# domainxz/top-k-rec

Hardware: AMD Instinct MI355X
Metric: BPR training triplets/sec (sampler + plan + step), MovieLens-10M shape (higher is better)
Workload: dtype f32

## Files before the change

include/tkr.h:

```cpp
#ifndef TKR_H
#define TKR_H
#include <stdint.h>

#ifdef __cplusplus
extern "C" {
#endif

#define TKR_VERSION 120
#define TKR_OK 0
#define TKR_E_INVAL (-1)
#define TKR_E_UNSUPPORTED (-2)
#define TKR_E_IO (-3)
#define TKR_E_PARSE (-4)
#define TKR_E_NOMEM (-5)

int tkr_version(void);
int tkr_lab_build(void);

int tkr_plan_team(int32_t batch_size);
int tkr_plan_max_blocks(int32_t batch_size);
int tkr_sample_plan(const int32_t* tr_users, int32_t n_tr, const int32_t* row_ptr, const int32_t* pos_cols,
                    const int32_t* cols_sorted, int32_t n_users, int32_t n_items, uint64_t seed,
                    uint64_t first_triplet, const int64_t* ctl, int32_t n_batches, int32_t batch_size,
                    int32_t* ucnt, int32_t* icnt, uint32_t* touch_u, uint32_t* touch_i, int32_t* out_u,
                    int32_t* out_i, int32_t* out_j, int32_t* task, int32_t* occ, int32_t* rec, int32_t* hdr,
                    int32_t* occt, int32_t* tpar, int32_t* prec, int32_t* pocc, void* workspace, int64_t workspace_bytes,
                    void* stream);
int64_t tkr_plan_workspace_bytes(int32_t batch_size, int32_t n_batches);

int tkr_plan_rollback(const int32_t* task, int32_t batch_size, int32_t first_batch, int32_t n_batches, int32_t* ucnt,
                      int32_t* icnt, void* stream);

typedef struct {
    float* U;
    float* msU;
    float* V;
    float* msV;
    float* b;
    float* msb;
    int32_t n_users, n_items, k;
    int32_t mode;
    float lu, li, lj, lb;
    float lr;
    float rho, eps;
    int32_t opt;
} tkr_bpr_state;

int tkr_bpr_run(const tkr_bpr_state* st, int32_t* rec, const int32_t* occ, const int32_t* hdr,
                int32_t batch_size, int32_t n_batches, float* loss_out, void* stream);

typedef struct {
    void* U;
    void* msU;
    void* tailU;
    uint32_t* rdU;
    void* V;
    void* msV;
    void* tailV;
    uint32_t* rdV;
    int32_t n_users, n_items, k;
    int32_t mode;
    float lu, li, lj, lb;
    float lr, rho, eps;
    int32_t opt;
    int32_t item_bufs;
} tkr_flow_state;
int32_t tkr_flow_row_granules(int32_t k);
int32_t tkr_flow_ctl_words(void);
#define TKR_FLOW_CTL_STATUS 1026
#define TKR_FLOW_CTL_SPINS 1027
int tkr_bpr_flow_run(const tkr_flow_state* st, const int32_t* prec, const int32_t* pocc, int32_t batch_size,
                     int32_t n_batches, uint32_t* ctl, float* loss_out, int32_t waves_per_cu, void* stream);

int32_t tkr_bpr_own_owners(int32_t n_items, int32_t k);
int32_t tkr_bpr_own_owners_shared(int32_t n_items, int32_t k, int32_t share);
int tkr_sample_plan_owned(const int32_t* tr_users, int32_t n_tr, const int32_t* row_ptr, const int32_t* pos_cols,
                          const int32_t* cols_sorted, int32_t n_users, int32_t n_items, uint64_t seed, uint64_t first_triplet,
                          int32_t n_batches, int32_t batch_size, int32_t* ucnt, int32_t* icnt, uint32_t* touch_u,
                          uint32_t* touch_i, int32_t* out_u, int32_t* out_i, int32_t* out_j, int32_t* task, int32_t* occ,
                          int32_t* occt, int32_t* prec, int32_t* pocc, int32_t n_owner, int32_t* ohdr, int32_t ohdr_stride,
                          void* stream);
int tkr_bpr_own_run(const tkr_flow_state* st, const int32_t* prec, const int32_t* pocc, const int32_t* occt, const int32_t* ohdr,
                    int32_t ohdr_stride, int32_t n_owner, int32_t batch_size, int32_t first_batch, int32_t n_batches, uint32_t* ctl, float* loss_out,
                    int32_t owner_waves, void* xch, uint32_t epoch, void* stream);
typedef struct tkr_plan_call {
    const int32_t *tr_users, *row_ptr, *pos_cols, *cols_sorted;
    int32_t *ucnt, *icnt;
    uint32_t *touch_u, *touch_i;
    int32_t *out_u, *out_i, *out_j, *task, *occ, *occt, *prec, *pocc, *ohdr;
    uint64_t seed, first_triplet;
    int32_t n_tr, n_users, n_items, n_batches, batch_size, n_owner, ohdr_stride, reserved;
} tkr_plan_call;
int tkr_bpr_own_plan_run(const tkr_plan_call* plan, const tkr_flow_state* st, int32_t first_batch, int32_t n_batches, uint32_t* ctl,
                         float* loss_out, int32_t owner_waves, void* xch, uint32_t epoch, void* ev_before, void* ev_after, void* stream);
int tkr_bpr_own_run_between(void* ev_before, void* ev_after, const tkr_flow_state* st, const int32_t* prec, const int32_t* pocc,
                            const int32_t* occt, const int32_t* ohdr, int32_t ohdr_stride, int32_t n_owner, int32_t batch_size,
                            int32_t first_batch, int32_t n_batches, uint32_t* ctl, float* loss_out, int32_t owner_waves, void* xch,
                            uint32_t epoch, void* stream);

typedef struct {
    float* U;
    float* msU;
    float* I;
    float* msI;
    float* irb;
    float* msirb;
    float* cem;
    float* mscem;
    float* icb;
    float* msicb;
    const float* feat;
    int32_t n_users, n_items, kh, d;
    int32_t mode;
    float lu, li, lj, lb, le;
    float lr, rho, eps;
    const int32_t* f_ptr;
    const int32_t* f_col;
    const float* f_val;
    const int32_t* c_ptr;
    const int32_t* c_item;
    const float* c_val;
    int64_t* item_tag;
} tkr_vbpr_state;

int64_t tkr_vbpr_workspace_floats(int32_t batch_size, int32_t kh, int32_t d);
int tkr_vbpr_set_pairs(int32_t mode);
int tkr_vbpr_run(const tkr_vbpr_state* st, const int32_t* tri_i, const int32_t* tri_j, const int32_t* rec,
                 const int32_t* occ, const int32_t* hdr, const int32_t* occt, const int32_t* tri_u ,
                 const int32_t* tpar , int32_t batch_size,
                 int32_t n_batches, float* workspace, float* loss_out, void* stream);

int64_t tkr_vbpr_colplan_lds_bytes(int32_t batch_size, int32_t d);
int tkr_vbpr_colplan(const int32_t* f_ptr, const int32_t* f_col, const float* f_val, int32_t d, const int32_t* tri_i,
                     const int32_t* tri_j, int32_t batch_size, int32_t n_batches, int32_t row_cap, int32_t* colh, int32_t* cent,
                     int32_t* tcnt, int32_t* tent, void* stream);
int tkr_vbpr_run_cols(const tkr_vbpr_state* st, const int32_t* tri_i, const int32_t* tri_j, const int32_t* rec, const int32_t* occ,
                      const int32_t* hdr, const int32_t* occt, const int32_t* tri_u, const int32_t* tpar, const int32_t* colh,
                      const int32_t* cent, const int32_t* tcnt, const int32_t* tent, int32_t row_cap, int32_t cols_per_block,
                      int32_t batch_size, int32_t n_batches, float* workspace, float* loss_out, void* stream);

int64_t tkr_topk_workspace_bytes(int32_t n_rows, int32_t K);
int64_t tkr_topk_workspace_bytes_for(int32_t n_rows, int32_t n_cols, int32_t k, int32_t K);
int tkr_topk_set_math(int32_t mode);
int tkr_build_rated_mask(const int64_t* rated_ptr, const int32_t* rated_cols, int32_t n_rows, int32_t n_cols,
                         uint32_t* mask, int32_t mask_pitch, void* stream);
int tkr_score_topk(const float* U, const int32_t* user_idx, int32_t n_rows, const float* Vt, const float* bias,
                   int32_t n_cols, int32_t k, const uint32_t* mask, int32_t mask_pitch, int32_t K,
                   int32_t* out_ids, float* out_scores, void* workspace, int64_t workspace_bytes, void* stream);

int tkr_count_hits(const int32_t* ids, int32_t n_rows, int32_t K, const int64_t* like_ptr, const int32_t* like_cols,
                   int32_t step, int32_t interval, uint64_t* first_bucket, void* stream);

int tkr_raw_ranks(const float* U, const int32_t* user_idx, int32_t n_rows, const float* Vt, const float* bias, int32_t k,
                  const int64_t* rated_ptr, const int32_t* rated_cols, const int32_t* ids, int32_t K, int32_t* raw_rank,
                  void* stream);
int tkr_count_hits_rr(const int32_t* ids, const int32_t* raw_rank, int32_t n_rows, int32_t K, const int64_t* like_ptr,
                      const int32_t* like_cols, int32_t step, int32_t interval, int32_t* hit_first, double* rr_first,
                      void* stream);

int64_t tkr_like_ranks_workspace_bytes(int32_t n_rows, int32_t n_cols, int32_t k, int64_t n_likes);
int tkr_like_ranks(const float* U, const int32_t* user_idx, int32_t n_rows, const float* Vt, const float* bias,
                   int32_t n_cols, int32_t k, const uint32_t* mask, int32_t mask_pitch, const int64_t* like_ptr,
                   const int32_t* like_cols, int32_t* rank_out, void* workspace, int64_t workspace_bytes, void* stream);

#define TKR_CANDIDATES_RESIDENT 2048
int tkr_rank_candidates(const float* U, const int32_t* user_idx, int32_t n_rows, const float* Vt, const float* bias,
                        int32_t n_cols, int32_t k, const int64_t* cand_ptr, const int32_t* cand_cols, const uint32_t* mask,
                        int32_t mask_pitch, float* score_out, int32_t* rank_out, void* stream);

int tkr_bpr_foldin(const float* V, const float* b, int32_t n_items, int32_t k, const int64_t* hist_ptr, const int32_t* hist_cols,
                   int32_t m, const float* U0, float lu, float lr, int32_t mode, int32_t steps, int32_t triplets, uint64_t seed,
                   uint64_t first_row, float* U, float* loss, int32_t* trip, void* stream);

int tkr_bpr_foldin_items(const float* U, const float* V, const float* b, int32_t n_users, int32_t n_items, int32_t k,
                         const int64_t* user_ptr, const int32_t* user_cols, const int64_t* liker_ptr, const int32_t* liker_rows,
                         const uint32_t* role_thresh, int32_t m, const float* V0, const float* b0, float li, float lj, float lb, float lr,
                         int32_t mode, int32_t steps, int32_t triplets, uint64_t seed, uint64_t first_row, float* Vn, float* bn,
                         float* loss, int32_t* trip, void* stream);

int tkr_sync_snapshot(const float* P, const int32_t* cnt, float* start, int64_t n, int32_t w, void* stream);
int tkr_sync_flow_snapshot(const void* V, const void* tailV, const int32_t* icnt, float* start, int32_t n, int32_t k, int32_t item_bufs,
                           void* stream);
int tkr_sync_flow_pack(const void* V, const void* msV, const void* tailV, const int32_t* icnt, const float* start, float* flat_delta,
                       float* flat_ms, int32_t n, int32_t k, float inv_world, int32_t item_bufs, void* stream);
int tkr_sync_flow_unpack(void* V, void* msV, void* tailV, uint32_t* rdV, int32_t* icnt, float* start ,
                         const float* flat_delta, const float* flat_ms, int32_t n, int32_t k, int32_t item_bufs, void* stream);
int tkr_sync_pack(const float* P, const float* ms, const int32_t* cnt, const float* start, float* flat_delta, float* flat_ms,
                  int64_t n, int32_t w, float inv_world, void* stream);
int tkr_sync_unpack(float* P, float* ms, const float* start, const float* flat_delta, const float* flat_ms, int64_t n, int32_t w,
                    void* stream);

int tkr_calib_rowcopy(const float* src, float* dst, const int32_t* rows, int32_t n, int32_t k, void* stream);

int tkr_idmap_create(const char* blob, int64_t blob_len, const int32_t* index, int64_t n, void** out_map);
int tkr_idmap_destroy(void* map);
int tkr_ratings_parse(const char* path, const void* user_map, const void* item_map, void** out_ratings);
int tkr_ratings_sizes(const void* ratings, int64_t* n_lines, int64_t* n_entries);
int tkr_ratings_copy(const void* ratings, int32_t* line_user, int64_t* line_ptr , int32_t* item,
                     int32_t* like);
int tkr_ratings_destroy(void* ratings);
int tkr_matrix_read(const char* path, void** out_matrix);
int tkr_matrix_sizes(const void* matrix, int64_t* rows, int64_t* cols);
int tkr_matrix_copy(const void* matrix, float* dst );
int tkr_matrix_destroy(void* matrix);
int tkr_matrix_write(const char* path, const float* data, int64_t rows, int64_t cols);

int64_t tkr_parse_dev_workspace_bytes(int64_t n_bytes, int64_t chunk_bytes);
int64_t tkr_idtable_slots(int64_t n);
int tkr_idtable_build(const char* blob, int64_t blob_len, const int32_t* index, int64_t n, int32_t* slots, int64_t n_slots);
int tkr_ratings_count_dev(const void* text, int64_t n_bytes, int64_t chunk_bytes, void* workspace, int64_t workspace_bytes,
                          int64_t* totals_out, void* stream);
int tkr_ratings_emit_dev(const void* text, int64_t n_bytes, int64_t chunk_bytes, void* workspace, int64_t workspace_bytes,
                         int64_t n_lines, int64_t n_entries, const int32_t* user_slots, int64_t user_n_slots,
                         const void* user_blob, int64_t user_blob_len, const int32_t* item_slots, int64_t item_n_slots,
                         const void* item_blob, int64_t item_blob_len, int64_t* line_start, int32_t* line_user,
                         int64_t* line_ptr, int32_t* item, int32_t* like, int64_t* status, void* stream);

int tkr_lists_format_sizes_dev(const int32_t* ids, const float* scores, const int32_t* row_user, int64_t n, int32_t K,
                               const void* user_blob, int64_t user_blob_len, const int64_t* user_start, const int32_t* user_len,
                               int64_t n_users, const void* item_blob, int64_t item_blob_len, const int64_t* item_start,
                               const int32_t* item_len, int64_t n_items, int64_t* line_ptr, int64_t* totals, void* stream);
int tkr_lists_format_emit_dev(const int32_t* ids, const float* scores, const int32_t* row_user, int64_t n, int32_t K,
                              const void* user_blob, int64_t user_blob_len, const int64_t* user_start, const int32_t* user_len,
                              int64_t n_users, const void* item_blob, int64_t item_blob_len, const int64_t* item_start,
                              const int32_t* item_len, int64_t n_items, const int64_t* line_ptr, int64_t first_row, int64_t n_rows,
                              void* out, int64_t out_bytes, int64_t* status, void* stream);
int tkr_matrix_format_sizes_dev(const float* data, int64_t rows, int64_t cols, int64_t* line_ptr, int64_t* totals, void* stream);
int tkr_matrix_format_emit_dev(const float* data, int64_t rows, int64_t cols, const int64_t* line_ptr, int64_t first_row,
                               int64_t n_rows, void* out, int64_t out_bytes, int64_t* status, void* stream);

int64_t tkr_scan_dev_workspace_bytes(int64_t n_bytes, int64_t chunk_bytes);
int tkr_matrix_count_dev(const void* text, int64_t n_bytes, int64_t chunk_bytes, void* workspace, int64_t workspace_bytes,
                         int64_t* totals_out, void* stream);
int tkr_matrix_emit_dev(const void* text, int64_t n_bytes, int64_t chunk_bytes, void* workspace, int64_t workspace_bytes,
                        int64_t n_lines, int64_t n_tokens, int64_t cols, int64_t* tok_start, float* data, uint64_t* hard,
                        int64_t* counts, void* stream);
int tkr_matrix_token_host(const char* tok, int64_t len, float* out);
int tkr_matrix_tokens_host(const char* text, int64_t n_bytes, const int64_t* start, int64_t n, float* out);

#ifdef __cplusplus
}
#endif
#endif
```

top-k-rec_amd/csrc/bpr_own.hip:

```cpp
#include "flow_task.h"
#ifndef TKR_TAG_NAP
#define TKR_TAG_NAP 4
#endif
#ifdef TKR_PLAN_STAMP
namespace tkr { __device__ unsigned long long own_k1_prof[32]; }
#define K1_STAMP(i) do { if (blockIdx.x == 0 && threadIdx.x == 0) tkr::own_k1_prof[i] = __builtin_amdgcn_s_memrealtime(); } while (0)
#define K1_STAMP_ITEMS(i) do { if (blockIdx.x == 0 && threadIdx.x == 256) tkr::own_k1_prof[i] = __builtin_amdgcn_s_memrealtime(); } while (0)
#endif
#include "plan_parts.h"

namespace tkr {

struct PlanArgs {
    const int32_t *tr_users, *row_ptr, *pos_cols, *cols_sorted;
    int32_t *ucnt, *icnt;
    uint32_t *touch_u, *touch_i;
    int32_t *out_u, *out_i, *out_j;
    int4* task;
    int2* occ;
    int32_t* occt;
    int4 *prec, *pocc;
    int32_t* ohdr;
    uint64_t seed, first_triplet;
    uint32_t n_tr, n_items;
    int n_plan, npad_items, own_words, reg_sort_ok;
};

template <int NAP>
__device__ __forceinline__ bool plan_rendezvous(uint32_t* counter, uint32_t n, bool arrive, uint32_t* ctl, volatile uint32_t* flag) {
    if (threadIdx.x == 0) {
        if (arrive) __hip_atomic_fetch_add(counter, 1u, __ATOMIC_RELAXED, __HIP_MEMORY_SCOPE_AGENT);
        uint32_t waited = 0, ok = 1u;
        while (ld_u32(counter) < n) {
            __builtin_amdgcn_s_sleep(NAP);
            if (spin_fail(waited, ctl, 0)) { ok = 0u; break; }
        }
        lds_poke(flag, ok);
    }
    __syncthreads();
    const bool ok = lds_peek(flag) != 0u;
    __syncthreads();
    return ok;
}

constexpr uint32_t kOwnInvalid = 0xffffffffu;

__host__ __device__ inline size_t plan_scratch_bytes(int B, int npad_items, int n_owner, int own_words) {
    size_t a = (size_t)npad_items * 8 + (kWideThreads / TKR_WAVE + 1) * 4;
    if (a < (size_t)(256 + 512) * 8 + 64) a = (size_t)(256 + 512) * 8 + 64;
    const size_t pb = (size_t)3 * B * 20 + (size_t)4 * n_owner * (own_words + 1) + (kWideThreads / TKR_WAVE + 1) * 4 + 16 + (size_t)3 * B * 32;
    return ((a > pb ? a : pb) + 15) & ~(size_t)15;
}

template <bool PLAN>
__device__ __forceinline__ int4 plan_ld(const int4* __restrict__ prec, const __amdgpu_buffer_rsrc_t& prec_r, size_t idx16) {
    if constexpr (PLAN) {
        const v4u x = __builtin_amdgcn_raw_buffer_load_b128(prec_r, (int)(idx16 * 16), 0, kAuxLoad);
        return make_int4((int)x.x, (int)x.y, (int)x.z, (int)x.w);
    } else {
        return prec[idx16];
    }
}
constexpr int kDotWin = 1024;

struct OwnQueue {
    uint32_t head;
    uint32_t total;
    uint32_t arrival;
    uint32_t head_batch;
};

struct QueueMap {
    const uint32_t* pre;
    const uint32_t* start;
    uint32_t slots_per_batch;
    __device__ __forceinline__ uint32_t locate(uint32_t pos, uint32_t& cur, int lane) const {
        uint32_t before;
        for (;;) {
            const uint32_t v = pre[cur + 1 + lane];
            const unsigned long long m = __ballot(v > pos);
            if (m) {
                const int f = __ffsll((long long)m) - 1;
                before = f ? (uint32_t)bcast_i((int)v, f - 1) : pre[cur];
                cur += f;
                break;
            }
            cur += TKR_WAVE;
        }
        return cur * slots_per_batch + start[cur] + (pos - before);
    }
};

template <bool PLAN>
struct UserTicketSrc {
    uint32_t ticket;
    int home, queues;
    uint32_t total;
    uint32_t B;
    const int4* __restrict__ prec;
    __amdgpu_buffer_rsrc_t prec_r;
    __device__ __forceinline__ void prefetch(NextTask& nx, int lane) {
        const u64 i64 = (u64)(uint32_t)bcast_i((int)ticket, 0) * (uint32_t)queues + (uint32_t)home;
        const uint32_t idx = i64 < total ? (uint32_t)i64 : 0xffffffffu;
        nx.have = true;
        nx.w = make_int4(0, 0, 0, 0);
        if (idx == 0xffffffffu) { nx.idx = idx; return; }
        nx.idx = idx + 2u * B * (idx / B);
        if (lane < 8) nx.w = plan_ld<PLAN>(prec, prec_r, (size_t)nx.idx * 8 + lane);
    }
};

template <int NP>
__device__ __forceinline__ void lds_row_read(const float* row, int lane, bool sgd, float (&own)[2 * NP], float (&ms)[2 * NP], Own& o) {
    constexpr int KP = NP * 128;
#pragma unroll
    for (int q = 0; q < NP; ++q) {
        const float2 a = *reinterpret_cast<const float2*>(row + q * 128 + 2 * lane);
        own[2 * q] = a.x; own[2 * q + 1] = a.y;
        if (!sgd) {
            const float2 m = *reinterpret_cast<const float2*>(row + KP + q * 128 + 2 * lane);
            ms[2 * q] = m.x; ms[2 * q + 1] = m.y;
        }
    }
    const float4 t = *reinterpret_cast<const float4*>(row + 2 * KP);
    const float2 t2 = *reinterpret_cast<const float2*>(row + 2 * KP + 4);
    o.b = t.x; o.msb = t.y;
    o.exp[0] = __float_as_uint(t.z); o.exp[1] = __float_as_uint(t.w);
    o.exp[2] = __float_as_uint(t2.x); o.exp[3] = __float_as_uint(t2.y);
}

struct ItemRow {
    const u64 *own_p, *own_ms, *own_tail;
    const uint32_t* own_rd;
    uint32_t ver;
    bool from_lds;
    const volatile uint32_t* tag;
    const float* row;
    int halves;
    bool rd_staged;
    uint32_t rd_val;
};

template <int NP>
__device__ __forceinline__ bool item_own_wait(const FlowTables& T, int lane, const ItemRow& r, bool sgd, float (&own)[2 * NP], float (&ms)[2 * NP],
                                              Own& o, uint32_t* ctl, uint32_t& spins) {
    if (r.from_lds) {
        uint32_t waited = 0;
        while (lds_peek(r.tag) != r.ver) {
#if TKR_TAG_NAP > 0
            __builtin_amdgcn_s_sleep(TKR_TAG_NAP);
#endif
            if (spin_fail(waited, ctl, 0)) {
                if (waited >= kSpinLimit && lane == 0 && atomicCAS(ctl + kCtlDebug, 0u, 4u) == 0u) {
                    ctl[kCtlDebug + 1] = lds_peek(r.tag); ctl[kCtlDebug + 3] = r.ver;
                }
                return false;
            }
        }
        spins += waited;
        asm volatile("" ::: "memory");
        lds_row_read<NP>(r.row, lane, sgd, own, ms, o);
        o.ok = true;
        if (r.rd_staged) {
            o.rd = r.rd_val;
            return true;
        }
    }
    return flow_own<NP>(T, lane, r.own_p, r.own_ms, r.own_tail, r.own_rd, r.ver, own, ms, o, sgd, ctl, spins, r.halves);
}

template <int NP>
struct LdsOwnStep {
    const FlowTables& T;
    int lane;
    const ItemRow& r;
    bool sgd;
    uint32_t* ctl;
    uint32_t& spins;
    __device__ __forceinline__ bool operator()(float (&own)[2 * NP], float (&ms)[2 * NP], Own& o) {
#ifdef TKR_OWN_PROF
        o.t_own0 = __builtin_amdgcn_s_memtime();
        const bool ok = item_own_wait<NP>(T, lane, r, sgd, own, ms, o, ctl, spins);
        o.t_own1 = __builtin_amdgcn_s_memtime();
        return ok;
#else
        return item_own_wait<NP>(T, lane, r, sgd, own, ms, o, ctl, spins);
#endif
    }
};
struct NoFeed {
    __device__ __forceinline__ void prefetch(NextTask& nx, int) { nx.have = true; }
};

template <int NP>
__device__ __forceinline__ void own_update(const tkr_flow_state& st, bool sgd, const float (&own)[2 * NP], const float (&ms)[2 * NP],
                                           const Own& o, const float (&g)[2 * NP], float gb, float (&pn)[2 * NP], float (&mn)[2 * NP],
                                           float& bn, float& mbn) {
    constexpr int NE = 2 * NP;
    if (sgd) {
#pragma unroll
        for (int e = 0; e < NE; ++e) { pn[e] = own[e] - st.lr * g[e]; mn[e] = 0.f; }
        bn = o.b - st.lr * gb;
        mbn = o.msb;
    } else {
#pragma unroll
        for (int e = 0; e < NE; ++e) {
            mn[e] = st.rho * ms[e] + (1.f - st.rho) * g[e] * g[e];
            pn[e] = own[e] - st.lr * g[e] * __builtin_amdgcn_rsqf(mn[e] + st.eps);
        }
        mbn = st.rho * o.msb + (1.f - st.rho) * gb * gb;
        bn = o.b - st.lr * gb * __builtin_amdgcn_rsqf(mbn + st.eps);
    }
}

template <int NP>
__device__ __forceinline__ bool own_publish(int lane, bool is_item, uint32_t bmask, bool sgd, u64* tabP, u64* tabM, u64* tabT, size_t woff,
                                            size_t n_rows, int row, int rowk, uint32_t ver, int n_occ, Own& o, const uint32_t* own_rd,
                                            const float (&pn)[2 * NP], const float (&mn)[2 * NP], float bn, float mbn, uint32_t* ctl,
                                            uint32_t& spins, uint32_t readers_per_occ) {
    const uint32_t nv = ver + 1u;
    const uint32_t expect = pick_exp(o, (ver + 1u) & bmask);
    uint32_t waited = 0;
    while ((int32_t)(o.rd - expect) < 0) {
        if (spin_fail(waited, ctl)) {
            if (waited >= kSpinLimit && lane == 0 && atomicCAS(ctl + kCtlDebug, 0u, 2u) == 0u) {
                ctl[kCtlDebug + 1] = o.rd; ctl[kCtlDebug + 2] = expect; ctl[kCtlDebug + 3] = ver; ctl[kCtlDebug + 4] = (uint32_t)rowk;
            }
            return false;
        }
        o.rd = ld_u32(own_rd);
    }
    spins += waited;
#ifdef TKR_OWN_PROF
    o.t_ack = __builtin_amdgcn_s_memtime();
#endif
    store_row<NP>(tabP + woff, lane, pn, nv);
    if (!sgd) store_row<NP>(tabM + woff, lane, mn, nv);
    store_tail(tabT, n_rows, row, bmask, lane, is_item, bn, mbn, o, ver, n_occ, readers_per_occ);
    return true;
}

constexpr int own_threads(int np) { return np == 1 ? 768 : 512; }

template <int NP, bool PLAN = false>
__global__ __launch_bounds__(own_threads(NP), own_threads(NP) / 256) void bpr_own_kernel(
    tkr_flow_state st, const int4* __restrict__ prec , const int4* __restrict__ pocc,
    const int32_t* __restrict__ occt, const int32_t* __restrict__ ohdr , int ohdr_stride,
    int first_batch, int nb, int B, int n_owner, int owner_waves, uint32_t tune, uint32_t* __restrict__ ctl, float* __restrict__ loss_out,
    u64* __restrict__ xch , uint32_t epoch, PlanArgs pa) {
    constexpr int TPB = own_threads(NP);
    constexpr int NE = 2 * NP;
    constexpr int KP = NP * 128;
    constexpr int ROWF = 2 * KP + 8;
    const int lane = threadIdx.x & (TKR_WAVE - 1), wave = threadIdx.x / TKR_WAVE;
    FlowTables T;
    T.tune = 0u;
    T.kp = KP;
    T.ustride = (size_t)st.n_users * T.kp;
    T.istride = (size_t)st.n_items * T.kp;
    T.imask = st.item_bufs == 4 ? 3u : 1u;
    const int item_halves = tail_halves(T.imask);
    T.U = reinterpret_cast<u64*>(st.U); T.msU = reinterpret_cast<u64*>(st.msU); T.tailU = reinterpret_cast<u64*>(st.tailU);
    T.V = reinterpret_cast<u64*>(st.V); T.msV = reinterpret_cast<u64*>(st.msV); T.tailV = reinterpret_cast<u64*>(st.tailV);
    T.rdU = st.rdU; T.rdV = st.rdV;
    const bool sgd = st.opt == 1;
    const bool want_loss = loss_out != nullptr;

    extern __shared__ __attribute__((aligned(16))) unsigned char smem[];
    OwnQueue* q = reinterpret_cast<OwnQueue*>(smem);
    uint32_t* pre = reinterpret_cast<uint32_t*>(smem + sizeof(OwnQueue));
    uint32_t* start = pre + nb + 1 + TKR_WAVE;
    const int rows_here = (st.n_items + n_owner - 1) / n_owner;
    uint32_t* tags = start + nb;
    uint32_t* dotmark = tags + rows_here;
    float* rows = reinterpret_cast<float*>(smem + ((sizeof(OwnQueue) + (size_t)4 * (2 * nb + 1 + TKR_WAVE + rows_here + kDotWin) + 15) & ~(size_t)15));

    const uint32_t me = blockIdx.x;
    bool alive = true;
    int commit_key = -1, commit_total = 0;
#ifdef TKR_PLAN_STAMP
#define PLAN_STAMP(i) do { if ((me == 0 || me == gridDim.x - 1) && threadIdx.x == 0) reinterpret_cast<u64*>(ctl + kCtlProf)[(me ? 16 : 0) + (i)] = __builtin_amdgcn_s_memrealtime(); } while (0)
#else
#define PLAN_STAMP(i) do { } while (0)
#endif
    PLAN_STAMP(0);
    for (int b = threadIdx.x; b < TKR_WAVE; b += TPB) pre[nb + 1 + b] = 0xffffffffu;
    for (int s = threadIdx.x; s < rows_here; s += TPB) tags[s] = kOwnInvalid;
    for (int s = threadIdx.x; s < kDotWin; s += TPB) dotmark[s] = 0u;
    if constexpr (PLAN) {
        static_assert(TPB == kWideThreads, "phase B of the planner is one thread per task slot");
        unsigned char* scratch = reinterpret_cast<unsigned char*>(rows);
        volatile uint32_t* flag = &q->arrival;
        const uint32_t n_plan = (uint32_t)pa.n_plan;
        int4 ct = make_int4(-1, 0, 0, 0);
        int cprev = 0, ctotal = 0;
        if (me < n_plan) {
            const int b = (int)me, n3 = 3 * B;
            int4* task_b = pa.task + (size_t)b * n3;
            int2* occ_b = pa.occ + (size_t)b * n3;
            int32_t* occt_b = pa.occt + (size_t)b * n3;
            const bool split = pa.reg_sort_ok != 0 && pa.npad_items == 512 && B > 128;
            const PlanMirror mir = plan_mirror(scratch + plan_scratch_bytes(B, pa.npad_items, n_owner, pa.own_words), B);
            if (split)
                plan_phase_a_split<TPB>(scratch, b, pa.tr_users, pa.n_tr, pa.row_ptr, pa.pos_cols, pa.cols_sorted, pa.n_items, pa.seed,
                                        pa.first_triplet + (uint64_t)b * (uint64_t)B, B, pa.out_u + (size_t)b * B, pa.out_i + (size_t)b * B,
                                        pa.out_j + (size_t)b * B, task_b, occ_b, occt_b, pa.touch_u, pa.touch_i, mir);
            else
                plan_phase_a<TPB, 256>(scratch, b, pa.tr_users, pa.n_tr, pa.row_ptr, pa.pos_cols, pa.cols_sorted, pa.n_items, pa.seed,
                                       pa.first_triplet + (uint64_t)b * (uint64_t)B, B, pa.npad_items, pa.out_u + (size_t)b * B, pa.out_i + (size_t)b * B,
                                       pa.out_j + (size_t)b * B, task_b, occ_b, occt_b, pa.touch_u, pa.touch_i, pa.reg_sort_ok != 0);
            PLAN_STAMP(1);
            asm volatile("s_waitcnt vmcnt(0)" ::: "memory");
            __syncthreads();
            PLAN_STAMP(2);
            alive = plan_rendezvous<4>(ctl + kCtlPlanA, n_plan, true, ctl, flag);
            PLAN_STAMP(3);
            if (alive) {
                if (split)
                    plan_phase_b_wide<true, true>(scratch, b, B, task_b, occ_b, occt_b, pa.ucnt, pa.icnt, pa.touch_u, pa.touch_i, pa.pocc + (size_t)b * n3,
                                                  pa.prec + (size_t)b * n3 * 8, n_owner, pa.ohdr, ohdr_stride, pa.own_words, ct, cprev, ctotal, mir);
                else
                    plan_phase_b_wide<true, false>(scratch, b, B, task_b, occ_b, occt_b, pa.ucnt, pa.icnt, pa.touch_u, pa.touch_i, pa.pocc + (size_t)b * n3,
                                                   pa.prec + (size_t)b * n3 * 8, n_owner, pa.ohdr, ohdr_stride, pa.own_words, ct, cprev, ctotal);
                PLAN_STAMP(4);
            }
            asm volatile("s_waitcnt vmcnt(0)" ::: "memory");
            __syncthreads();
            PLAN_STAMP(5);
        }
        alive = plan_rendezvous<12>(ctl + kCtlPlanC, n_plan, me < n_plan, ctl, flag) && alive;
        PLAN_STAMP(8);
        commit_key = (alive && me < n_plan && (int)threadIdx.x < 3 * B && ct.x != -1 && cprev == -1) ? ct.x : -1;
        commit_total = ctotal;
        PLAN_STAMP(9);
    }
    const bool ticket_wave = wave > owner_waves;
    const int tw = wave - owner_waves - 1, n_tw = TPB / TKR_WAVE - owner_waves - 1;
    const int queues = min(kQueues, max(n_tw, 1) * (int)gridDim.x);
    const int home = ticket_wave ? (int)((me * (uint32_t)n_tw + (uint32_t)tw) % (uint32_t)queues) : 0;
    uint32_t ticket = 0;
    if (ticket_wave) ticket = grab_issue(ctl, lane, home);
    for (int b = threadIdx.x; b < nb; b += TPB) {
        uint32_t h = 0u;
        if (me < (uint32_t)n_owner) {
            if constexpr (PLAN) h = (uint32_t)__hip_atomic_load(ohdr + (size_t)me * ohdr_stride + b, __ATOMIC_RELAXED, __HIP_MEMORY_SCOPE_AGENT);
            else h = (uint32_t)ohdr[(size_t)me * ohdr_stride + b];
        }
        start[b] = h & 0xffffu;
        pre[b + 1] = h >> 16;
    }
    __syncthreads();
    if (wave == 0) {
        const int per = (nb + TKR_WAVE - 1) / TKR_WAVE;
        const int b0 = min(lane * per, nb), b1 = min(b0 + per, nb);
        uint32_t mine = 0;
        for (int b = b0; b < b1; ++b) mine += pre[b + 1];
        uint32_t incl = mine;
#pragma unroll
        for (int d = 1; d < TKR_WAVE; d <<= 1) {
            const uint32_t up = (uint32_t)__shfl_up((int)incl, d);
            if (lane >= d) incl += up;
        }
        uint32_t run = incl - mine;
        for (int b = b0; b < b1; ++b) { run += pre[b + 1]; pre[b + 1] = run; }
        if (lane == TKR_WAVE - 1) { q->total = incl; q->head = 0u; q->head_batch = 0u; }
        if (lane == 0) pre[0] = 0u;
    }
    __syncthreads();

    PLAN_STAMP(10);
    uint32_t spins = 0;
#ifdef TKR_OWN_PROF
    u64 prof[16] = {0, 0, 0, 0, 0, 0, 0, 0, 0, 0, 0, 0, 0, 0, 0, 0};
    u64 tprev = __builtin_amdgcn_s_memtime();
#endif
    const QueueMap qm{pre, start, 3u * (uint32_t)B};
    const __amdgpu_buffer_rsrc_t prec_r = row_rsrc(prec, PLAN ? nb * 3 * B * 128 : 16);
    const uint32_t q_total = q->total;

    auto item_row = [&](const int4 w, ItemRow& r, int& row, int& slot) {
        const int rowk = bcast_i(w.x, 0);
        const uint32_t ver = (uint32_t)bcast_i(w.y, 0);
        const int prev = bcast_i(w.y, 1);
        row = rowk & 0x7fffffff;
        slot = row / n_owner;
        const size_t roff = (size_t)(ver & T.imask) * T.istride + (size_t)row * T.kp;
        r.own_p = T.V + roff; r.own_ms = T.msV + roff;
        r.own_tail = T.tailV + ((size_t)(ver & T.imask) * st.n_items + row) * (2 * item_halves);
        r.own_rd = T.rdV + (T.imask + 1u) * (size_t)row + ((ver + 1u) & T.imask);
        r.ver = ver;
        r.from_lds = prev >= first_batch;
        r.tag = tags + slot;
        r.row = rows + (size_t)slot * ROWF;
        r.halves = item_halves;
        r.rd_staged = false;
        r.rd_val = 0u;
    };

    constexpr uint32_t kItemReaders = 2u;
    if (wave <= owner_waves) {
        uint32_t cur = 0;
        while (alive) {
            uint32_t pos = 0;
            if (lane == 0) pos = atomicAdd(&q->head, 1u);
            pos = (uint32_t)bcast_i((int)pos, 0);
            if (pos >= q_total) break;
            const uint32_t idx = qm.locate(pos, cur, lane);
            if (lane == 0) atomicMax(&q->head_batch, cur);
            int4 w = make_int4(0, 0, 0, 0);
            if (lane < 8) w = plan_ld<PLAN>(prec, prec_r, (size_t)idx * 8 + lane);
#ifdef TKR_OWN_PROF
            asm volatile("" : "+v"(w.x) :: "memory");
            const u64 t0 = __builtin_amdgcn_s_memtime();
            prof[5] += t0 - tprev;
#endif
            ItemRow r;
            int row, slot;
            item_row(w, r, row, slot);
            const int rowk = bcast_i(w.x, 0);
            const uint32_t ver = r.ver;
            const int n_occ = bcast_i(w.z, 0), first = bcast_i(w.w, 0);
            const size_t woff = (size_t)((ver + 1u) & T.imask) * T.istride + (size_t)row * T.kp;
            float* lrow = rows + (size_t)slot * ROWF;

            float own[NE], ms[NE], g[NE];
#pragma unroll
            for (int e = 0; e < NE; ++e) { g[e] = 0.f; ms[e] = 0.f; }
            Own o = {};
            float gb = 0.f;
            o.ok = r.from_lds;
            NextTask nx;
            nx.idx = 0u; nx.w = make_int4(0, 0, 0, 0); nx.have = true;
            NoFeed feed;
            LdsOwnStep<NP> own_step{T, lane, r, sgd, ctl, spins};
            float loss_lane = 0.f;
            alive = run_task<NP, true, NoFeed, LdsOwnStep<NP>, 4>(st, T, lane, n_occ, first, w, pocc, r.own_p, r.own_ms, r.own_tail, ver, own, ms, o, g,
                                                                  gb, loss_lane, false, sgd, ctl, spins, nx, feed, own_step);
            if (!alive) break;
            if (lane == 0) dotmark[pos & (kDotWin - 1)] = pos + 1u;
#ifdef TKR_OWN_PROF
            const u64 t1 = __builtin_amdgcn_s_memtime();
#endif
            float pn[NE], mn[NE], bn, mbn;
            own_update<NP>(st, sgd, own, ms, o, g, gb, pn, mn, bn, mbn);

#pragma unroll
            for (int qq = 0; qq < NP; ++qq) {
                *reinterpret_cast<float2*>(lrow + qq * 128 + 2 * lane) = make_float2(pn[2 * qq], pn[2 * qq + 1]);
                if (!sgd) *reinterpret_cast<float2*>(lrow + KP + qq * 128 + 2 * lane) = make_float2(mn[2 * qq], mn[2 * qq + 1]);
            }
            if (lane == 0) {
                const uint32_t rb = ver & T.imask, add = kItemReaders * (uint32_t)n_occ;
                *reinterpret_cast<float4*>(lrow + 2 * KP) = make_float4(bn, mbn, __uint_as_float(o.exp[0] + (rb == 0u ? add : 0u)),
                                                                        __uint_as_float(o.exp[1] + (rb == 1u ? add : 0u)));
                *reinterpret_cast<float2*>(lrow + 2 * KP + 4) =
                    make_float2(__uint_as_float(o.exp[2] + (rb == 2u ? add : 0u)), __uint_as_float(o.exp[3] + (rb == 3u ? add : 0u)));
            }
            asm volatile("s_waitcnt lgkmcnt(0)" ::: "memory");
            if (lane == 0) lds_poke(tags + slot, ver + 1u);

            alive = own_publish<NP>(lane, true, T.imask, sgd, T.V, T.msV, T.tailV, woff, (size_t)st.n_items, row, rowk, ver, n_occ, o, r.own_rd, pn,
                                    mn, bn, mbn, ctl, spins, kItemReaders);
#ifdef TKR_OWN_PROF
            tprev = __builtin_amdgcn_s_memtime();
            prof[0] += o.t_own0 - t0; prof[1] += o.t_own1 - o.t_own0; prof[2] += t1 - o.t_own1;
            prof[3] += o.t_ack - t1; prof[4] += tprev - o.t_ack; prof[6] += 1; prof[7] += r.from_lds ? 1 : 0;
#endif
        }
    } else {
        const uint32_t total = (uint32_t)nb * (uint32_t)B;
        NextTask nx;
        nx.idx = 0u; nx.w = make_int4(0, 0, 0, 0); nx.have = false;
        while (alive) {
            if (!nx.have) {
                UserTicketSrc<PLAN> first_feed{ticket, home, queues, total, (uint32_t)B, prec, prec_r};
                first_feed.prefetch(nx, lane);
                asm volatile("" : "+v"(nx.w.x), "+v"(nx.w.y), "+v"(nx.w.z), "+v"(nx.w.w) :: "memory");
            }
            const uint32_t idx = nx.idx;
            const int4 w = nx.w;
            if (idx == 0xffffffffu) break;
            nx.have = false;
            ticket = grab_issue(ctl, lane, home);
            const int rowk = bcast_i(w.x, 0);
#ifdef TKR_OWN_PROF
            const u64 t0 = __builtin_amdgcn_s_memtime();
            prof[8] += t0 - tprev;
#endif
            if (rowk < 0) {
#ifdef TKR_OWN_PROF
                tprev = t0;
#endif
                continue;
            }
            const uint32_t ver = (uint32_t)bcast_i(w.y, 0);
            const int n_occ = bcast_i(w.z, 0);
            const int first = bcast_i(w.w, 0);
            const int batch = bcast_i(w.x, 1);
            const int row = rowk;

            const size_t roff = (size_t)(ver & 1u) * T.ustride + (size_t)row * T.kp;
            const size_t woff = (size_t)((ver + 1u) & 1u) * T.ustride + (size_t)row * T.kp;
            const uint32_t* own_rd = T.rdU + 2 * (size_t)row + ((ver + 1u) & 1u);
            const u64* own_tail = T.tailU + ((size_t)(ver & 1u) * st.n_users + row) * 4;

            float own[NE], ms[NE], g[NE];
#pragma unroll
            for (int e = 0; e < NE; ++e) { g[e] = 0.f; ms[e] = 0.f; }
            Own o = {};
            float gb = 0.f, loss_lane = 0.f;
            UserTicketSrc<PLAN> feed{ticket, home, queues, total, (uint32_t)B, prec, prec_r};
            GlobalOwn<NP> own_step{T, lane, T.U + roff, T.msU + roff, own_tail, own_rd, ver, sgd, ctl, spins, 2};
            alive = run_task<NP, false, UserTicketSrc<PLAN>, GlobalOwn<NP>, 4>(st, T, lane, n_occ, first, w, pocc, T.U + roff, T.msU + roff, own_tail, ver,
                                                                         own, ms, o, g, gb, loss_lane, want_loss, sgd, ctl, spins, nx, feed, own_step);
            if (!alive) break;
#ifdef TKR_OWN_PROF
            const u64 t1 = __builtin_amdgcn_s_memtime();
#endif
            if (want_loss) {
                const float tot = wave_sum(loss_lane);
                if (lane == 0) {
                    const uint32_t slot = idx - (uint32_t)(batch - first_batch) * 3u * (uint32_t)B;
                    __hip_atomic_store(xch + ((size_t)batch * B + slot) * 2, ((u64)epoch << 32) | (u64)__float_as_uint(tot), __ATOMIC_RELAXED,
                                       __HIP_MEMORY_SCOPE_AGENT);
                }
            }
            float pn[NE], mn[NE], bn, mbn;
            own_update<NP>(st, sgd, own, ms, o, g, gb, pn, mn, bn, mbn);
            asm volatile("" : "+v"(nx.w.x), "+v"(nx.w.y), "+v"(nx.w.z), "+v"(nx.w.w));
            alive = own_publish<NP>(lane, false, 1u, sgd, T.U, T.msU, T.tailU, woff, (size_t)st.n_users, row, rowk, ver, n_occ, o, own_rd, pn, mn,
                                    bn, mbn, ctl, spins, 2u);
#ifdef TKR_OWN_PROF
            tprev = __builtin_amdgcn_s_memtime();
            prof[9] += t1 - t0; prof[11] += o.t_ack - t1; prof[12] += tprev - o.t_ack; prof[13] += 1;
#endif
        }
    }

    if (lane == 0 && spins) atomicAdd(ctl + kCtlSpins, spins);
#ifdef TKR_OWN_PROF
    if (lane == 0)
        for (int qq = 0; qq < 16; ++qq) atomicAdd(reinterpret_cast<u64*>(ctl + kCtlProf) + qq, prof[qq]);
#endif
    asm volatile("s_waitcnt vmcnt(0)" ::: "memory");
    __syncthreads();
    PLAN_STAMP(11);
    if constexpr (PLAN) {
        if (commit_key != -1) plan_commit_first_touch(make_int4(commit_key, 0, 0, 0), -1, commit_total, pa.ucnt, pa.icnt, pa.touch_u, pa.touch_i);
    }
    const bool fold_loss = want_loss && (tune & 8u) != 0u;
    if (threadIdx.x == 0) {
        const bool last = __hip_atomic_fetch_add(ctl + kCtlLeave, 1u, __ATOMIC_RELAXED, __HIP_MEMORY_SCOPE_AGENT) == gridDim.x - 1u;
        if (last) {
            for (int qq = 0; qq < kQueues; ++qq) ctl[qq * kQueueStride] = 0u;
            ctl[kCtlArrive] = 0u;
            ctl[kCtlLeave] = 0u;
            if constexpr (PLAN) { ctl[kCtlPlanA] = 0u; ctl[kCtlPlanB] = 0u; ctl[kCtlPlanC] = 0u; }
        }
        q->arrival = last ? 1u : 0u;
    }
    if (!fold_loss) return;
    __syncthreads();
    if (q->arrival == 0u) return;
    for (int b = wave; b < nb; b += TPB / TKR_WAVE) {
        const int batch = first_batch + b;
        float part[4];
#pragma unroll
        for (int w = 0; w < 4; ++w) {
            float acc = 0.f;
            for (int t = w * TKR_WAVE + lane; t < B; t += 256) {
                const u64 g = __hip_atomic_load(xch + ((size_t)batch * B + t) * 2, __ATOMIC_RELAXED, __HIP_MEMORY_SCOPE_AGENT);
                if ((uint32_t)(g >> 32) == epoch) acc += __uint_as_float((uint32_t)g);
            }
            part[w] = wave_sum(acc);
        }
        if (lane == 0) loss_out[batch] = (part[0] + part[1]) + (part[2] + part[3]);
    }
}

__global__ __launch_bounds__(256) void own_loss_kernel(const u64* __restrict__ xch, int first_batch, int B, uint32_t epoch, float* __restrict__ loss_out) {
    __shared__ float part[4];
    const int b = first_batch + (int)blockIdx.x, lane = threadIdx.x & (TKR_WAVE - 1), wave = threadIdx.x / TKR_WAVE;
    float acc = 0.f;
    for (int s = threadIdx.x; s < B; s += 256) {
        const u64 g = xch[((size_t)b * B + s) * 2];
        if ((uint32_t)(g >> 32) == epoch) acc += __uint_as_float((uint32_t)g);
    }
    acc = wave_sum(acc);
    if (lane == TKR_WAVE - 1) part[wave] = acc;
    __syncthreads();
    if (threadIdx.x == 0) loss_out[b] = (part[0] + part[1]) + (part[2] + part[3]);
}

static size_t own_lds_bytes(int np, int nb, int n_items, int n_owner) {
    const int rows_here = (n_items + n_owner - 1) / n_owner;
    const size_t head = (sizeof(OwnQueue) + (size_t)4 * (2 * nb + 1 + TKR_WAVE + rows_here + kDotWin) + 15) & ~(size_t)15;
    return head + (size_t)rows_here * (2 * np * 128 + 8) * 4;
}

static size_t own_lds_bytes_planned(int np, int nb, int n_items, int n_owner, int B, int npad_items, int own_words) {
    const int rows_here = (n_items + n_owner - 1) / n_owner;
    const size_t head = (sizeof(OwnQueue) + (size_t)4 * (2 * nb + 1 + TKR_WAVE + rows_here + kDotWin) + 15) & ~(size_t)15;
    const size_t rows = (size_t)rows_here * (2 * np * 128 + 8) * 4;
    const size_t scratch = plan_scratch_bytes(B, npad_items, n_owner, own_words) + plan_mirror_lds(B);
    return head + (rows > scratch ? rows : scratch);
}

}

extern "C" int32_t tkr_bpr_own_owners_shared(int32_t n_items, int32_t k, int32_t share) {
    if (n_items <= 0 || k <= 0 || k > 256 || share <= 0) return 0;
    int dev = 0, cus = 0;
    if (hipGetDevice(&dev) != hipSuccess) return 0;
    if (hipDeviceGetAttribute(&cus, hipDeviceAttributeMultiprocessorCount, dev) != hipSuccess || cus <= 0) return 0;
    const int owners = cus / share;
    if (owners <= 0) return 0;
    const int np = (k + 127) / 128;
    if (tkr::own_lds_bytes(np, 512, n_items, owners) > 160 * 1024) return 0;
    return owners;
}
extern "C" int32_t tkr_bpr_own_owners(int32_t n_items, int32_t k) { return tkr_bpr_own_owners_shared(n_items, k, 1); }

static int own_launch(const tkr_flow_state* st, const int32_t* prec, const int32_t* pocc, const int32_t* occt, const int32_t* ohdr,
                      int32_t ohdr_stride, int32_t n_owner, int32_t batch_size, int32_t first_batch, int32_t n_batches, uint32_t* ctl,
                      float* loss_out, int32_t owner_waves, void* xch, uint32_t epoch, const tkr::PlanArgs* pa, void* stream) {
    if (!st || !st->U || !st->V || !st->tailU || !st->tailV || !st->rdU || !st->rdV) return TKR_EINVAL;
    if (st->opt != 0 && st->opt != 1) return TKR_EINVAL;
    if (st->opt == 0 && (!st->msU || !st->msV)) return TKR_EINVAL;
    if (st->n_users <= 0 || st->n_items <= 0 || st->k <= 0) return TKR_EINVAL;
    if (st->k > 256) return TKR_EUNSUPPORTED;
    if (st->item_bufs != 0 && st->item_bufs != 2 && st->item_bufs != 4) return TKR_EINVAL;
    if (!xch || epoch == 0u) return TKR_EINVAL;
    if (!prec || !pocc || !occt || !ohdr || !ctl || batch_size <= 0 || n_batches < 0 || first_batch < 0 || n_owner <= 0) return TKR_EINVAL;
    if (ohdr_stride < first_batch + n_batches || n_batches > 512) return TKR_EINVAL;
    if (n_batches == 0) return TKR_OK;
    if ((uint64_t)(first_batch + n_batches) * 3u * (uint64_t)batch_size >= 0xffffffffull / 8) return TKR_EUNSUPPORTED;
    const int np = (st->k + 127) / 128;
    int dev = 0;
    TKR_CHECK(hipGetDevice(&dev));
    static int cached_cus[64];
    static bool attr_set[64][3];
    int cus;
    if (dev >= 0 && dev < 64 && cached_cus[dev] > 0) cus = cached_cus[dev];
    else {
        TKR_CHECK(hipDeviceGetAttribute(&cus, hipDeviceAttributeMultiprocessorCount, dev));
        if (dev >= 0 && dev < 64) cached_cus[dev] = cus;
    }
    if (n_owner > cus) return TKR_EUNSUPPORTED;
    size_t lds = tkr::own_lds_bytes(np, n_batches, st->n_items, n_owner);
    if (pa) lds = tkr::own_lds_bytes_planned(np, n_batches, st->n_items, n_owner, batch_size, pa->npad_items, pa->own_words);
    if (lds > 160 * 1024) return TKR_EUNSUPPORTED;
    const uint32_t tune = ((uint32_t)owner_waves >> 8) & 0xffu;
    owner_waves &= 0xff;
    if ((tune & (1u | 128u)) || (np == 1 && (tune & (32u | 64u)))) return TKR_EUNSUPPORTED;
    if (pa && np != 1) return TKR_EINVAL;
    const int tpb = tkr::own_threads(np);
    const int waves = tpb / TKR_WAVE;
    int ow = owner_waves > 0 ? owner_waves : (waves == 12 ? 9 : 6);
    if (ow < 1) ow = 1;
    if (ow > waves - 2) ow = waves - 2;
    const bool fold = loss_out && n_batches <= 64 && !(tune & 2u);
    const uint32_t ktune = (tune & ~8u) | (fold ? 8u : 0u);
    const void* fn = pa ? (const void*)tkr::bpr_own_kernel<1, true>
                   : np == 1 ? (const void*)tkr::bpr_own_kernel<1, false> : (const void*)tkr::bpr_own_kernel<2, false>;
    const int form = pa ? 2 : np - 1;
    if (lds > 64 * 1024 && !(dev >= 0 && dev < 64 && attr_set[dev][form])) {
        TKR_CHECK(hipFuncSetAttribute(fn, hipFuncAttributeMaxDynamicSharedMemorySize, 160 * 1024));
        if (dev >= 0 && dev < 64) attr_set[dev][form] = true;
    }
    static signed char fits[64][3];
    if (dev >= 0 && dev < 64 && fits[dev][form] == 0) {
        int per_cu = 0;
        TKR_CHECK(hipOccupancyMaxActiveBlocksPerMultiprocessor(&per_cu, fn, tpb, 160 * 1024));
        fits[dev][form] = per_cu >= 1 ? 1 : -1;
    }
    if (dev >= 0 && dev < 64 && fits[dev][form] < 0) return TKR_EUNSUPPORTED;
    hipStream_t s = (hipStream_t)stream;
    const int4* r4 = reinterpret_cast<const int4*>(prec) + (size_t)first_batch * 3 * batch_size * 8;
    const int4* o4 = reinterpret_cast<const int4*>(pocc);
    ohdr += first_batch;
    const tkr::PlanArgs no_plan = {};
#define TKR_OWN_LAUNCH(NPV, PL)                                                                                                           \
    hipLaunchKernelGGL((tkr::bpr_own_kernel<NPV, PL>), dim3(n_owner), dim3(tkr::own_threads(NPV)), lds, s, *st, r4, o4, occt, ohdr, ohdr_stride,   \
                       first_batch, n_batches, batch_size, n_owner, ow, ktune, ctl, loss_out, static_cast<tkr::u64*>(xch), epoch, PL ? *pa : no_plan)
    if (pa) TKR_OWN_LAUNCH(1, true);
    else if (np == 1) TKR_OWN_LAUNCH(1, false);
    else TKR_OWN_LAUNCH(2, false);
#undef TKR_OWN_LAUNCH
    TKR_LAUNCH_CHECK();
    if (loss_out && !fold) {
        hipLaunchKernelGGL(tkr::own_loss_kernel, dim3(n_batches), dim3(256), 0, s, static_cast<const tkr::u64*>(xch), first_batch, batch_size, epoch,
                           loss_out);
        TKR_LAUNCH_CHECK();
    }
    return TKR_OK;
}

extern "C" int tkr_bpr_own_run(const tkr_flow_state* st, const int32_t* prec, const int32_t* pocc, const int32_t* occt, const int32_t* ohdr,
                               int32_t ohdr_stride, int32_t n_owner, int32_t batch_size, int32_t first_batch, int32_t n_batches,
                               uint32_t* ctl, float* loss_out, int32_t owner_waves, void* xch, uint32_t epoch, void* stream) {
    return own_launch(st, prec, pocc, occt, ohdr, ohdr_stride, n_owner, batch_size, first_batch, n_batches, ctl, loss_out, owner_waves, xch, epoch,
                      nullptr, stream);
}

extern "C" int tkr_bpr_own_run_between(void* ev_before, void* ev_after, const tkr_flow_state* st, const int32_t* prec, const int32_t* pocc,
                                       const int32_t* occt, const int32_t* ohdr, int32_t ohdr_stride, int32_t n_owner, int32_t batch_size,
                                       int32_t first_batch, int32_t n_batches, uint32_t* ctl, float* loss_out, int32_t owner_waves, void* xch,
                                       uint32_t epoch, void* stream) {
    if (ev_before) TKR_CHECK(hipEventRecord((hipEvent_t)ev_before, (hipStream_t)stream));
    const int rc = tkr_bpr_own_run(st, prec, pocc, occt, ohdr, ohdr_stride, n_owner, batch_size, first_batch, n_batches, ctl, loss_out, owner_waves,
                                   xch, epoch, stream);
    if (ev_after) TKR_CHECK(hipEventRecord((hipEvent_t)ev_after, (hipStream_t)stream));
    return rc;
}

extern "C" int tkr_bpr_own_plan_run(const tkr_plan_call* plan, const tkr_flow_state* st, int32_t first_batch, int32_t n_batches, uint32_t* ctl,
                                    float* loss_out, int32_t owner_waves, void* xch, uint32_t epoch, void* ev_before, void* ev_after,
                                    void* stream) {
    if (!plan || !st || first_batch < 0 || n_batches < 0 || first_batch + n_batches > plan->n_batches) return TKR_EINVAL;
    const uint32_t tune = ((uint32_t)owner_waves >> 8) & 0xffu;
    const int B = plan->batch_size, n_owner = plan->n_owner;
    const int np = (st->k + 127) / 128;
    int npad = 1, npad_bits = 0;
    while (npad < 2 * B) { npad <<= 1; ++npad_bits; }
    const int own_words = n_owner > 0 ? ((plan->n_items + n_owner - 1) / n_owner + 31) / 32 : 0;
    const bool fusable = !(tune & 16u) && np == 1 && !(tune & (32u | 64u | 128u)) && first_batch == 0 && n_batches == plan->n_batches && n_batches > 0 &&
                         n_batches <= 64 && n_batches <= n_owner && B > 0 && 3 * B <= tkr::kWideThreads && plan->n_tr > 0 && plan->n_users > 0 &&
                         plan->n_items > 0 && plan->n_users < (1 << 25) && plan->n_items < (1 << 25)  && plan->ohdr_stride >= n_batches &&
                         plan->n_users == st->n_users && plan->n_items == st->n_items &&
                         tkr::own_lds_bytes_planned(np, n_batches, st->n_items, n_owner, B, npad, own_words) <= 160 * 1024;
    if (fusable) {
        if (!plan->tr_users || !plan->row_ptr || !plan->pos_cols || !plan->cols_sorted || !plan->ucnt || !plan->icnt || !plan->touch_u ||
            !plan->touch_i || !plan->out_u || !plan->out_i || !plan->out_j || !plan->task || !plan->occ || !plan->occt || !plan->prec ||
            !plan->pocc || !plan->ohdr)
            return TKR_EINVAL;
        tkr::PlanArgs pa;
        pa.tr_users = plan->tr_users; pa.row_ptr = plan->row_ptr; pa.pos_cols = plan->pos_cols; pa.cols_sorted = plan->cols_sorted;
        pa.ucnt = plan->ucnt; pa.icnt = plan->icnt; pa.touch_u = plan->touch_u; pa.touch_i = plan->touch_i;
        pa.out_u = plan->out_u; pa.out_i = plan->out_i; pa.out_j = plan->out_j;
        pa.task = reinterpret_cast<int4*>(plan->task); pa.occ = reinterpret_cast<int2*>(plan->occ); pa.occt = plan->occt;
        pa.prec = reinterpret_cast<int4*>(plan->prec); pa.pocc = reinterpret_cast<int4*>(plan->pocc); pa.ohdr = plan->ohdr;
        pa.seed = plan->seed; pa.first_triplet = plan->first_triplet;
        pa.n_tr = (uint32_t)plan->n_tr; pa.n_items = (uint32_t)plan->n_items;
        pa.n_plan = n_batches; pa.npad_items = npad; pa.own_words = own_words;
        pa.reg_sort_ok = (npad_bits < 31 && (uint64_t)(plan->n_users > plan->n_items ? plan->n_users : plan->n_items) < (1ull << (32 - npad_bits)) - 1ull) ? 1 : 0;
        if (ev_before) TKR_CHECK(hipEventRecord((hipEvent_t)ev_before, (hipStream_t)stream));
        const int rc = own_launch(st, plan->prec, plan->pocc, plan->occt, plan->ohdr, plan->ohdr_stride, n_owner, B, 0, n_batches, ctl, loss_out,
                                  owner_waves, xch, epoch, &pa, stream);
        if (ev_after) TKR_CHECK(hipEventRecord((hipEvent_t)ev_after, (hipStream_t)stream));
        return rc;
    }
    const int rc = tkr_sample_plan_owned(plan->tr_users, plan->n_tr, plan->row_ptr, plan->pos_cols, plan->cols_sorted, plan->n_users,
                                         plan->n_items, plan->seed, plan->first_triplet, plan->n_batches, plan->batch_size, plan->ucnt,
                                         plan->icnt, plan->touch_u, plan->touch_i, plan->out_u, plan->out_i, plan->out_j, plan->task,
                                         plan->occ, plan->occt, plan->prec, plan->pocc, plan->n_owner, plan->ohdr, plan->ohdr_stride, stream);
    if (rc != TKR_OK) return rc;
    return tkr_bpr_own_run_between(ev_before, ev_after, st, plan->prec, plan->pocc, plan->occt, plan->ohdr, plan->ohdr_stride, plan->n_owner,
                                   plan->batch_size, first_batch, n_batches, ctl, loss_out, owner_waves, xch, epoch, stream);
}

#ifdef TKR_PLAN_STAMP
extern "C" int tkr_debug_own_k1_prof(unsigned long long* out ) {
    return hipMemcpyFromSymbol(out, HIP_SYMBOL(tkr::own_k1_prof), sizeof(unsigned long long) * 32) == hipSuccess ? 0 : -100;
}
#endif
```

top-k-rec_amd/csrc/sampler.hip:

```cpp
#include <stdlib.h>

#include "tkr_common.h"

#ifdef TKR_K1_PROF
namespace tkr { __device__ unsigned long long k1_prof[32]; }
#define K1_STAMP(i) do { if (blockIdx.x == 0 && threadIdx.x == 0) tkr::k1_prof[i] = __builtin_amdgcn_s_memrealtime(); } while (0)
#endif
#include "plan_parts.h"

namespace tkr {

template <int T>
__global__ __launch_bounds__(T) void sample_plan_kernel(
    const int32_t* __restrict__ tr_users, uint32_t n_tr, const int32_t* __restrict__ row_ptr,
    const int32_t* __restrict__ pos_cols, const int32_t* __restrict__ cols_sorted, uint32_t n_items,
    uint64_t seed, uint64_t first_triplet, const int64_t* __restrict__ ctl, int B, int npad_items,
    int32_t* __restrict__ out_u, int32_t* __restrict__ out_i, int32_t* __restrict__ out_j,
    int4* __restrict__ task_all, int2* __restrict__ occ_all, int32_t* __restrict__ occt_all,
    uint32_t* __restrict__ touch_u, uint32_t* __restrict__ touch_i, bool reg_sort_ok ) {
    extern __shared__ __attribute__((aligned(16))) unsigned char smem[];
    const int b = blockIdx.x;
    const uint64_t batch0 = ctl ? (uint64_t)ctl[0] : 0ull;
    const uint64_t g0 = first_triplet + (batch0 + (uint64_t)b) * (uint64_t)B;
    plan_phase_a<T, T>(smem, b, tr_users, n_tr, row_ptr, pos_cols, cols_sorted, n_items, seed, g0, B, npad_items, out_u + (size_t)b * B,
                       out_i + (size_t)b * B, out_j + (size_t)b * B, task_all + (size_t)b * 3 * B, occ_all + (size_t)b * 3 * B,
                       occt_all + (size_t)b * 3 * B, touch_u, touch_i, reg_sort_ok);
}

__device__ __forceinline__ int block_exclusive_scan2(int a, int b, int* scan , int& tot_a,
                                                      int& tot_b, int& ex_b) {
    const int lane = threadIdx.x & (TKR_WAVE - 1), wave = threadIdx.x / TKR_WAVE;
    int ia = a, ib = b;
#pragma unroll
    for (int d = 1; d < TKR_WAVE; d <<= 1) {
        const int ua = __shfl_up(ia, d), ub = __shfl_up(ib, d);
        if (lane >= d) { ia += ua; ib += ub; }
    }
    __syncthreads();
    if (lane == TKR_WAVE - 1) { scan[wave] = ia; scan[kPlanThreads / TKR_WAVE + wave] = ib; }
    __syncthreads();
    int ea = ia - a;
    ex_b = ib - b;
    tot_a = 0;
    tot_b = 0;
#pragma unroll
    for (int w = 0; w < kPlanThreads / TKR_WAVE; ++w) {
        const int ta = scan[w], tb = scan[kPlanThreads / TKR_WAVE + w];
        if (w < wave) { ea += ta; ex_b += tb; }
        tot_a += ta;
        tot_b += tb;
    }
    return ea;
}

__global__ __launch_bounds__(kPlanThreads) void resolve_kernel(
    int B, int rec_stride , int4* __restrict__ task_all, int2* __restrict__ occ_all,
    const int32_t* __restrict__ occt_all,
    const int32_t* __restrict__ ucnt, const int32_t* __restrict__ icnt, const uint32_t* __restrict__ touch_u,
    const uint32_t* __restrict__ touch_i, int32_t* __restrict__ rec_all, int4* __restrict__ hdr_all,
    const int32_t* __restrict__ out_u_all, int32_t* __restrict__ tpar_all ) {
    __shared__ int scan[2 * (kPlanThreads + 1)];
    const int kTeam = team_for(B);
    const int lmax = light_max(B);
    const int b = blockIdx.x;
    int4* task = task_all + (size_t)b * 3 * B;
    int2* occ = occ_all + (size_t)b * 3 * B;
    const int32_t* occt = occt_all + (size_t)b * 3 * B;
    int32_t* rec = rec_all + (size_t)b * rec_stride * 16;

    for (int s = threadIdx.x; s < 3 * B; s += kPlanThreads) {
        int4 t = task[s];
        if (t.x != -1) {
            const int row = t.x & 0x7fffffff;
            t.w = (t.x < 0) ? parity_of(icnt, touch_i, row, b) : parity_of(ucnt, touch_u, row, b);
            task[s] = t;
        }
    }
    for (int p = threadIdx.x; p < B; p += kPlanThreads) {
        int2 o = occ[p];
        const int pi = parity_of(icnt, touch_i, o.x, b), pj = parity_of(icnt, touch_i, o.y, b);
        o.x |= pi << 30;
        o.y |= pj << 30;
        occ[p] = o;
        if (tpar_all) {
            const int t = occt[p];
            const int u = out_u_all[(size_t)b * B + t];
            tpar_all[(size_t)b * B + t] = parity_of(ucnt, touch_u, u, b) | (pi << 1) | (pj << 2);
        }
    }
    for (int p = threadIdx.x; p < 2 * B; p += kPlanThreads) {
        int2 o = occ[B + p];
        o.x |= parity_of(ucnt, touch_u, o.x, b) << 30;
        o.y |= parity_of(icnt, touch_i, o.y & 0x3fffffff, b) << 30;
        occ[B + p] = o;
    }
    __threadfence_block();
    __syncthreads();

    const int per = (3 * B + kPlanThreads - 1) / kPlanThreads;
    const int beg = min((int)threadIdx.x * per, 3 * B), end = min(beg + per, 3 * B);
    int nl = 0, nh = 0;
    for (int s = beg; s < end; ++s) {
        const int4 t = task[s];
        if (t.x != -1) { if (t.z <= lmax) ++nl; else ++nh; }
    }
    int tot_l, tot_h, hi;
    int li = block_exclusive_scan2(nl, nh, scan, tot_l, tot_h, hi);
    const int lpb = light_per_block(B);
    const int nlb = (tot_l + lpb - 1) / lpb;
    for (int s = beg; s < end; ++s) {
        const int4 t = task[s];
        if (t.x == -1) continue;
        if (t.z <= lmax) {
            int32_t* r = rec + ((size_t)(li / lpb) * kTeam + li % lpb) * 16;
            r[0] = t.x; r[1] = t.w | (1 << 8); r[2] = t.z; r[3] = t.y;
            int tt[4];
            for (int q = 0; q < 4; ++q) {
                const int2 o = (q < t.z) ? occ[t.y + q] : make_int2(0, 0);
                r[4 + 2 * q] = o.x; r[5 + 2 * q] = o.y;
                tt[q] = (q < t.z) ? occt[t.y + q] : 0;
            }
            r[12] = t.z; r[13] = tt[0] | (tt[1] << 16); r[14] = tt[2] | (tt[3] << 16); r[15] = 0;
            ++li;
        } else {
            for (int w = 0; w < kTeam; ++w) {
                int32_t* r = rec + ((size_t)(nlb + hi) * kTeam + w) * 16;
                const int mine = (t.z > w) ? (t.z - w + kTeam - 1) / kTeam : 0;
                r[0] = t.x; r[1] = t.w | (kTeam << 8) | (w << 16); r[2] = mine; r[3] = t.y + w;
                int tt[4];
                for (int q = 0; q < 4; ++q) {
                    const int2 o = (q < mine) ? occ[t.y + w + q * kTeam] : make_int2(0, 0);
                    r[4 + 2 * q] = o.x; r[5 + 2 * q] = o.y;
                    tt[q] = (q < mine) ? occt[t.y + w + q * kTeam] : 0;
                }
                r[12] = t.z; r[13] = tt[0] | (tt[1] << 16); r[14] = tt[2] | (tt[3] << 16); r[15] = 0;
            }
            ++hi;
        }
    }
    for (int s = threadIdx.x; s < nlb * kTeam; s += kPlanThreads) {
        const int li_of = (s / kTeam) * lpb + (s % kTeam);
        if ((s % kTeam) >= lpb || li_of >= tot_l) {
            int32_t* r = rec + (size_t)s * 16;
            r[0] = -1;
            for (int q = 1; q < 16; ++q) r[q] = 0;
        }
    }
    if (threadIdx.x == 0) hdr_all[b] = make_int4(nlb + tot_h, nlb, tot_h, tot_l + tot_h);
}

template <int T>
__global__ __launch_bounds__(T) void resolve_flow_kernel(
    int B, const int4* __restrict__ task_all, const int2* __restrict__ occ_all, const int32_t* __restrict__ ucnt,
    const int32_t* __restrict__ icnt, const uint32_t* __restrict__ touch_u, const uint32_t* __restrict__ touch_i,
    int4* __restrict__ pocc_all, int4* __restrict__ prec_all, int n_owner, int32_t* __restrict__ ohdr, int ohdr_stride,
    const int32_t* __restrict__ occt_all, int own_words ) {
    extern __shared__ __attribute__((aligned(16))) unsigned char smem[];
    __shared__ int s_first_item, s_wave[T / TKR_WAVE];
    const int b = blockIdx.x;
    const int4* task = task_all + (size_t)b * 3 * B;
    const int2* occ = occ_all + (size_t)b * 3 * B;
    int4* pocc = pocc_all + (size_t)b * 3 * B;
    int4* prec = prec_all + (size_t)b * 3 * B * 8;
    K1_STAMP(8);

    for (int p = threadIdx.x; p < B; p += T) {
        const int2 o = occ[p];
        pocc[p] = make_int4(o.x, version_of(icnt, touch_i, o.x, b), o.y, version_of(icnt, touch_i, o.y, b));
    }
    for (int p = threadIdx.x; p < 2 * B; p += T) {
        const int2 o = occ[B + p];
        pocc[B + p] = make_int4(o.x, version_of(ucnt, touch_u, o.x, b), o.y,
                                version_of(icnt, touch_i, o.y & 0x3fffffff, b));
    }
    uint32_t* own_mask = reinterpret_cast<uint32_t*>(smem);
    uint32_t* own_start = own_mask + (size_t)n_owner * own_words;
    int first_item = 0;
#ifdef TKR_K1_PROF
    __syncthreads();
    K1_STAMP(9);
#endif
    if (n_owner > 0) {
        if (threadIdx.x == 0) s_first_item = 3 * B;
        for (int w = threadIdx.x; w < n_owner * own_words; w += T) own_mask[w] = 0u;
        __syncthreads();
        for (int s = threadIdx.x; s < 3 * B; s += T) {
            const int x = task[s].x;
            if (x < 0 && x != -1) {
                if (s == 0 || task[s - 1].x >= 0) s_first_item = s;
                const int row = x & 0x7fffffff, bit = row / n_owner;
                atomicOr(&own_mask[(size_t)(row % n_owner) * own_words + (bit >> 5)], 1u << (bit & 31));
            }
        }
        __syncthreads();
        first_item = s_first_item;
        const int per = (n_owner + T - 1) / T;
        const int w0 = min((int)threadIdx.x * per, n_owner), w1 = min(w0 + per, n_owner);
        int mine = 0;
        for (int w = w0; w < w1; ++w)
            for (int j = 0; j < own_words; ++j) mine += __popc(own_mask[(size_t)w * own_words + j]);
        const int lane = threadIdx.x & (TKR_WAVE - 1), wave = threadIdx.x / TKR_WAVE;
        int incl = mine;
#pragma unroll
        for (int d = 1; d < TKR_WAVE; d <<= 1) {
            const int up = __shfl_up(incl, d);
            if (lane >= d) incl += up;
        }
        if (lane == TKR_WAVE - 1) s_wave[wave] = incl;
        __syncthreads();
        int run = incl - mine;
        for (int w = 0; w < wave; ++w) run += s_wave[w];
        for (int w = w0; w < w1; ++w) {
            int c = 0;
            for (int j = 0; j < own_words; ++j) c += __popc(own_mask[(size_t)w * own_words + j]);
            ohdr[(size_t)w * ohdr_stride + b] = (first_item + run) | (c << 16);
            own_start[w] = (uint32_t)run;
            run += c;
        }
    }
    __threadfence_block();
    __syncthreads();
    K1_STAMP(10);
    for (int s = threadIdx.x; s < 3 * B; s += T) {
        const int4 t = task[s];
        int dst = s;
        if (n_owner > 0 && t.x < 0 && t.x != -1) {
            const int row = t.x & 0x7fffffff, w = row % n_owner, bit = row / n_owner;
            const uint32_t* m = own_mask + (size_t)w * own_words;
            int before = __popc(m[bit >> 5] & ((1u << (bit & 31)) - 1u));
            for (int j = 0; j < (bit >> 5); ++j) before += __popc(m[j]);
            dst = first_item + (int)own_start[w] + before;
        }
        int4* r = prec + (size_t)dst * 8;
        if (t.x == -1) {
            r[0] = make_int4(-1, 0, 0, 0);
#pragma unroll
            for (int q = 1; q < 8; ++q) r[q] = make_int4(0, 0, 0, 0);
            continue;
        }
        const int row = t.x & 0x7fffffff;
        int ver, prev;
        if (t.x < 0) row_history(icnt, touch_i, row, b, ver, prev);
        else row_history(ucnt, touch_u, row, b, ver, prev);
        r[0] = make_int4(t.x, ver, t.z, b * 3 * B + t.y);
        r[1] = make_int4(b, prev, 0, 0);
#pragma unroll
        for (int q = 0; q < 4; ++q) r[2 + q] = (q < t.z) ? pocc[t.y + q] : make_int4(0, 0, 0, 0);
        const int32_t* tt = occt_all + (size_t)b * 3 * B + t.y;
        r[6] = make_int4(tt[0], t.z > 1 ? tt[1] : 0, t.z > 2 ? tt[2] : 0, t.z > 3 ? tt[3] : 0);
        r[7] = make_int4(0, 0, 0, 0);
    }
#ifdef TKR_K1_PROF
    __syncthreads();
    K1_STAMP(11);
#endif
}

__global__ __launch_bounds__(kWideThreads) void resolve_flow_wide_kernel(
    int B, const int4* __restrict__ task_all, const int2* __restrict__ occ_all, const int32_t* __restrict__ ucnt,
    const int32_t* __restrict__ icnt, const uint32_t* __restrict__ touch_u, const uint32_t* __restrict__ touch_i,
    int4* __restrict__ pocc_all, int4* __restrict__ prec_all, int n_owner, int32_t* __restrict__ ohdr, int ohdr_stride,
    const int32_t* __restrict__ occt_all, int own_words) {
    extern __shared__ __attribute__((aligned(16))) unsigned char smem[];
    const int b = blockIdx.x, n = 3 * B;
    int4 t;
    int prev, total;
    plan_phase_b_wide<false>(smem, b, B, task_all + (size_t)b * n, occ_all + (size_t)b * n, occt_all + (size_t)b * n, ucnt, icnt, touch_u, touch_i,
                             pocc_all + (size_t)b * n, prec_all + (size_t)b * n * 8, n_owner, ohdr, ohdr_stride, own_words, t, prev, total);
#ifdef TKR_K1_PROF
    __syncthreads();
    K1_STAMP(11);
#endif
}

__global__ void commit_kernel(int n_users, int n_items, int32_t* __restrict__ ucnt, int32_t* __restrict__ icnt,
                              uint32_t* __restrict__ touch_u, uint32_t* __restrict__ touch_i) {
    const int r = blockIdx.x * blockDim.x + threadIdx.x;
    if (r >= n_users + n_items) return;
    int32_t* cnt = (r < n_users) ? ucnt + r : icnt + (r - n_users);
    uint4* w = reinterpret_cast<uint4*>((r < n_users) ? touch_u + (size_t)r * kTouchWords
                                                       : touch_i + (size_t)(r - n_users) * kTouchWords);
    int c = 0;
#pragma unroll
    for (int q = 0; q < kTouchWords / 4; ++q) {
        const uint4 v = w[q];
        c += __popc(v.x) + __popc(v.y) + __popc(v.z) + __popc(v.w);
    }
    if (c) {
        *cnt += c;
#pragma unroll
        for (int q = 0; q < kTouchWords / 4; ++q) w[q] = make_uint4(0, 0, 0, 0);
    }
}

__global__ void rollback_kernel(const int4* __restrict__ task, size_t n_slots, int32_t* __restrict__ ucnt,
                                int32_t* __restrict__ icnt) {
    const size_t s = (size_t)blockIdx.x * blockDim.x + threadIdx.x;
    if (s >= n_slots) return;
    const int rowk = task[s].x;
    if (rowk == -1) return;
    atomicSub((rowk < 0) ? icnt + (rowk & 0x7fffffff) : ucnt + rowk, 1);
}

}

extern "C" int tkr_plan_team(int32_t batch_size) { return tkr::team_for(batch_size); }

extern "C" __attribute__((visibility("hidden"))) int tkr_plan_commit(int32_t n_users, int32_t n_items, int32_t* ucnt, int32_t* icnt, uint32_t* touch_u,
                                                                     uint32_t* touch_i, void* stream) {
    const int rows = n_users + n_items;
    hipLaunchKernelGGL(tkr::commit_kernel, dim3((rows + 255) / 256), dim3(256), 0, (hipStream_t)stream, n_users, n_items, ucnt, icnt, touch_u, touch_i);
    TKR_LAUNCH_CHECK();
    return TKR_OK;
}

extern "C" int tkr_plan_max_blocks(int32_t batch_size) {
    const int lpb = tkr::light_per_block(batch_size);
    return (3 * batch_size + lpb - 1) / lpb + (3 * batch_size) / (tkr::light_max(batch_size) + 1);
}

extern "C" __attribute__((visibility("hidden"))) int64_t tkr_plan_workspace_bytes_for(int32_t batch_size, int32_t n_batches);
extern "C" __attribute__((visibility("hidden"))) int tkr_plan_mid_ok(int32_t n_users, int32_t n_items, int32_t B);
extern "C" __attribute__((visibility("hidden"))) int64_t tkr_plan_mid_workspace_bytes(int32_t batch_size, int32_t n_batches);
extern "C" __attribute__((visibility("hidden"))) int tkr_sample_plan_mid(
    const int32_t* tr_users, int32_t n_tr, const int32_t* row_ptr, const int32_t* pos_cols, const int32_t* cols_sorted, int32_t n_users,
    int32_t n_items, uint64_t seed, uint64_t first_triplet, const int64_t* ctl, int32_t n_batches, int32_t B, int32_t* ucnt, int32_t* icnt,
    uint32_t* touch_u, uint32_t* touch_i, int32_t* out_u, int32_t* out_i, int32_t* out_j, int32_t* task, int32_t* occ, int32_t* rec,
    int32_t* hdr, int32_t* occt, int32_t* tpar, void* workspace, int64_t workspace_bytes, void* stream);
extern "C" __attribute__((visibility("hidden"))) int tkr_sample_plan_big(const int32_t* tr_users, int32_t n_tr, const int32_t* row_ptr, const int32_t* pos_cols,
                                   const int32_t* cols_sorted, int32_t n_users, int32_t n_items, uint64_t seed,
                                   uint64_t first_triplet, const int64_t* ctl, int32_t n_batches, int32_t B, int32_t* ucnt,
                                   int32_t* icnt, uint32_t* touch_u, uint32_t* touch_i, int32_t* out_u, int32_t* out_i,
                                   int32_t* out_j, int32_t* task, int32_t* occ, int32_t* rec, int32_t* hdr, int32_t* occt,
                                   int32_t* tpar, void* workspace, int64_t workspace_bytes, void* stream);

static int sample_plan_impl(const int32_t* tr_users, int32_t n_tr, const int32_t* row_ptr,
                               const int32_t* pos_cols, const int32_t* cols_sorted, int32_t n_users,
                               int32_t n_items, uint64_t seed, uint64_t first_triplet, const int64_t* ctl,
                               int32_t n_batches, int32_t batch_size, int32_t* ucnt, int32_t* icnt,
                               uint32_t* touch_u, uint32_t* touch_i, int32_t* out_u, int32_t* out_i,
                               int32_t* out_j, int32_t* task, int32_t* occ, int32_t* rec, int32_t* hdr,
                               int32_t* occt, int32_t* tpar, int32_t* prec, int32_t* pocc, void* workspace,
                               int64_t workspace_bytes, int32_t n_owner, int32_t* ohdr, int32_t ohdr_stride, void* stream) {
    if (n_owner < 0 || n_owner > 65535 || (n_owner > 0 && (!prec || !ohdr || ohdr_stride < n_batches))) return TKR_EINVAL;
    const int own_words = n_owner > 0 ? ((n_items + n_owner - 1) / n_owner + 31) / 32 : 0;
    if (n_owner > 0 && (size_t)4 * n_owner * (own_words + 1) > 60 * 1024) return TKR_EUNSUPPORTED;
    if (n_tr <= 0 || n_items <= 0 || n_users <= 0 || batch_size <= 0 || n_batches < 0) return TKR_EINVAL;
    if (n_users >= (1 << 30) || n_items >= (1 << 30)) return TKR_EUNSUPPORTED;
    if (n_batches > 32 * tkr::kTouchWords) return TKR_EUNSUPPORTED;
    if (n_batches == 0) return TKR_OK;
    if (!ucnt || !icnt || !touch_u || !touch_i || !occt) return TKR_EINVAL;
    const bool flow = prec != nullptr;
    if (flow ? !pocc : (!rec || !hdr)) return TKR_EINVAL;
    if (!flow && tkr_plan_mid_ok(n_users, n_items, batch_size) && workspace &&
        workspace_bytes >= tkr_plan_mid_workspace_bytes(batch_size, n_batches)) {
        const int rc = tkr_sample_plan_mid(tr_users, n_tr, row_ptr, pos_cols, cols_sorted, n_users, n_items, seed, first_triplet, ctl,
                                           n_batches, batch_size, ucnt, icnt, touch_u, touch_i, out_u, out_i, out_j, task, occ, rec,
                                           hdr, occt, tpar, workspace, workspace_bytes, stream);
        return rc;
    }
    static const int big_from = [] { const char* e = getenv("TKR_PLAN_BIG_FROM"); const int v = e ? atoi(e) : 0; return v > 0 ? v : 4096; }();
    if (batch_size > 8192 || (batch_size >= big_from && !flow && workspace &&
                              workspace_bytes >= tkr_plan_workspace_bytes_for(batch_size, n_batches))) {
        if (flow) return TKR_EUNSUPPORTED;
        const int rc = tkr_sample_plan_big(tr_users, n_tr, row_ptr, pos_cols, cols_sorted, n_users, n_items, seed, first_triplet, ctl,
                                           n_batches, batch_size, ucnt, icnt, touch_u, touch_i, out_u, out_i, out_j, task, occ, rec,
                                           hdr, occt, tpar, workspace, workspace_bytes, stream);
        if (rc != TKR_OK) return rc;
        const int rows_ = n_users + n_items;
        hipLaunchKernelGGL(tkr::commit_kernel, dim3((rows_ + 255) / 256), dim3(256), 0, (hipStream_t)stream, n_users, n_items, ucnt,
                           icnt, touch_u, touch_i);
        TKR_LAUNCH_CHECK();
        return TKR_OK;
    }
    int npad = 1, npad_bits = 0;
    while (npad < 2 * batch_size) { npad <<= 1; ++npad_bits; }
    static const bool lds_sort = [] { const char* e = getenv("TKR_PLAN_LDS_SORT"); return e && atoi(e) != 0; }();
    const bool reg_sort_ok = !lds_sort && npad_bits < 31 && (uint64_t)(n_users > n_items ? n_users : n_items) < (1ull << (32 - npad_bits)) - 1ull;
    hipStream_t s = (hipStream_t)stream;
    if (batch_size <= 1024) {
        const size_t lds = (size_t)npad * 8 + (tkr::kPlanThreads + 1) * sizeof(int);
        hipLaunchKernelGGL(tkr::sample_plan_kernel<tkr::kPlanThreads>, dim3(n_batches), dim3(tkr::kPlanThreads), lds, s,
                           tr_users, (uint32_t)n_tr, row_ptr, pos_cols, cols_sorted, (uint32_t)n_items, seed,
                           first_triplet, ctl, batch_size, npad, out_u, out_i, out_j, reinterpret_cast<int4*>(task),
                           reinterpret_cast<int2*>(occ), occt, touch_u, touch_i, reg_sort_ok);
    } else {
        const size_t lds = (size_t)npad * 8 + (tkr::kPlanThreadsBig + 1) * sizeof(int);
        static bool attr_set[64] = {};
        int dev = 0;
        TKR_CHECK(hipGetDevice(&dev));
        if (lds > 64 * 1024 && !(dev >= 0 && dev < 64 && attr_set[dev])) {
            TKR_CHECK(hipFuncSetAttribute(reinterpret_cast<const void*>(tkr::sample_plan_kernel<tkr::kPlanThreadsBig>),
                                          hipFuncAttributeMaxDynamicSharedMemorySize, 160 * 1024));
            if (dev >= 0 && dev < 64) attr_set[dev] = true;
        }
        hipLaunchKernelGGL(tkr::sample_plan_kernel<tkr::kPlanThreadsBig>, dim3(n_batches), dim3(tkr::kPlanThreadsBig), lds,
                           s, tr_users, (uint32_t)n_tr, row_ptr, pos_cols, cols_sorted, (uint32_t)n_items, seed,
                           first_triplet, ctl, batch_size, npad, out_u, out_i, out_j, reinterpret_cast<int4*>(task),
                           reinterpret_cast<int2*>(occ), occt, touch_u, touch_i, reg_sort_ok);
    }
    TKR_LAUNCH_CHECK();
    if (flow) {
        static const int wide_upto = [] { const char* e = getenv("TKR_PLAN_WIDE_UPTO"); return e ? atoi(e) : 64; }();
        const size_t lds_r = n_owner > 0 ? (size_t)4 * n_owner * (own_words + 1) : 0;
        const size_t lds_w = tkr::plan_phase_b_wide_lds(batch_size, n_owner, own_words);
        if (n_batches <= wide_upto && 3 * batch_size <= tkr::kWideThreads && lds_w <= 64 * 1024)
            hipLaunchKernelGGL(tkr::resolve_flow_wide_kernel, dim3(n_batches), dim3(tkr::kWideThreads), lds_w, s,
                               batch_size, reinterpret_cast<const int4*>(task), reinterpret_cast<const int2*>(occ), ucnt, icnt, touch_u,
                               touch_i, reinterpret_cast<int4*>(pocc), reinterpret_cast<int4*>(prec), n_owner, ohdr, ohdr_stride, occt, own_words);
        else
            hipLaunchKernelGGL(tkr::resolve_flow_kernel<tkr::kPlanThreads>, dim3(n_batches), dim3(tkr::kPlanThreads), lds_r, s, batch_size,
                               reinterpret_cast<const int4*>(task), reinterpret_cast<const int2*>(occ), ucnt, icnt, touch_u,
                               touch_i, reinterpret_cast<int4*>(pocc), reinterpret_cast<int4*>(prec), n_owner, ohdr, ohdr_stride, occt, own_words);
    }
    else
        hipLaunchKernelGGL(tkr::resolve_kernel, dim3(n_batches), dim3(tkr::kPlanThreads), 0, s, batch_size,
                           tkr_plan_max_blocks(batch_size) * tkr::team_for(batch_size), reinterpret_cast<int4*>(task),
                           reinterpret_cast<int2*>(occ), occt, ucnt, icnt, touch_u, touch_i, rec,
                           reinterpret_cast<int4*>(hdr), out_u, tpar);
    TKR_LAUNCH_CHECK();
    const int rows = n_users + n_items;
    hipLaunchKernelGGL(tkr::commit_kernel, dim3((rows + 255) / 256), dim3(256), 0, s, n_users, n_items, ucnt, icnt,
                       touch_u, touch_i);
    TKR_LAUNCH_CHECK();
    return TKR_OK;
}

extern "C" int tkr_sample_plan(const int32_t* tr_users, int32_t n_tr, const int32_t* row_ptr,
                               const int32_t* pos_cols, const int32_t* cols_sorted, int32_t n_users,
                               int32_t n_items, uint64_t seed, uint64_t first_triplet, const int64_t* ctl,
                               int32_t n_batches, int32_t batch_size, int32_t* ucnt, int32_t* icnt,
                               uint32_t* touch_u, uint32_t* touch_i, int32_t* out_u, int32_t* out_i,
                               int32_t* out_j, int32_t* task, int32_t* occ, int32_t* rec, int32_t* hdr,
                               int32_t* occt, int32_t* tpar, int32_t* prec, int32_t* pocc, void* workspace,
                               int64_t workspace_bytes, void* stream) {
    return sample_plan_impl(tr_users, n_tr, row_ptr, pos_cols, cols_sorted, n_users, n_items, seed, first_triplet, ctl, n_batches,
                            batch_size, ucnt, icnt, touch_u, touch_i, out_u, out_i, out_j, task, occ, rec, hdr, occt, tpar, prec, pocc,
                            workspace, workspace_bytes, 0, nullptr, 0, stream);
}

extern "C" int tkr_sample_plan_owned(const int32_t* tr_users, int32_t n_tr, const int32_t* row_ptr,
                                     const int32_t* pos_cols, const int32_t* cols_sorted, int32_t n_users,
                                     int32_t n_items, uint64_t seed, uint64_t first_triplet, int32_t n_batches,
                                     int32_t batch_size, int32_t* ucnt, int32_t* icnt, uint32_t* touch_u, uint32_t* touch_i,
                                     int32_t* out_u, int32_t* out_i, int32_t* out_j, int32_t* task, int32_t* occ, int32_t* occt,
                                     int32_t* prec, int32_t* pocc, int32_t n_owner, int32_t* ohdr, int32_t ohdr_stride, void* stream) {
    if (n_owner <= 0) return TKR_EINVAL;
    return sample_plan_impl(tr_users, n_tr, row_ptr, pos_cols, cols_sorted, n_users, n_items, seed, first_triplet, nullptr, n_batches,
                            batch_size, ucnt, icnt, touch_u, touch_i, out_u, out_i, out_j, task, occ, nullptr, nullptr, occt, nullptr, prec,
                            pocc, nullptr, 0, n_owner, ohdr, ohdr_stride, stream);
}

extern "C" int tkr_plan_rollback(const int32_t* task, int32_t batch_size, int32_t first_batch, int32_t n_batches,
                                 int32_t* ucnt, int32_t* icnt, void* stream) {
    if (!task || !ucnt || !icnt || batch_size <= 0 || first_batch < 0 || n_batches < 0) return TKR_EINVAL;
    if (n_batches == 0) return TKR_OK;
    const size_t per = (size_t)3 * batch_size, n_slots = per * n_batches;
    hipLaunchKernelGGL(tkr::rollback_kernel, dim3((unsigned)((n_slots + 255) / 256)), dim3(256), 0, (hipStream_t)stream,
                       reinterpret_cast<const int4*>(task) + per * first_batch, n_slots, ucnt, icnt);
    TKR_LAUNCH_CHECK();
    return TKR_OK;
}

#ifdef TKR_K1_PROF
extern "C" int tkr_debug_k1_prof(unsigned long long* out ) {
    return hipMemcpyFromSymbol(out, HIP_SYMBOL(tkr::k1_prof), sizeof(unsigned long long) * 32) == hipSuccess ? 0 : -100;
}
#endif
```

top-k-rec_amd/single/_config.py:

```python
from __future__ import annotations

import os
from dataclasses import dataclass, fields


def _flag(name, raw):
    if raw in ('0', '1'):
        return raw == '1'
    raise ValueError('%s=%r: expected 0 or 1' % (name, raw))


def _int_in(lo, hi):
    def parse(name, raw):
        try:
            v = int(raw, 0)
        except ValueError:
            raise ValueError('%s=%r: expected an integer in [%d, %d]' % (name, raw, lo, hi)) from None
        if not lo <= v <= hi:
            raise ValueError('%s=%d: expected an integer in [%d, %d]' % (name, v, lo, hi))
        return v
    return parse


def _choice(*allowed):
    def parse(name, raw):
        if raw not in allowed:
            raise ValueError('%s=%r: expected one of %s' % (name, raw, ', '.join(allowed)))
        return raw
    return parse


@dataclass
class Tuning:
    flow: bool = True
    flow_max_batch: int = 512
    flow_waves_per_cu: int = 0
    flow_item_bufs: int = 4
    own: str = '1'
    own_max_batch: int = 256
    own_waves: int = 0
    fuse_short: bool = True
    fuse_plan: bool = True
    overlap_min_batch: int = 2048
    epoch_ahead: bool = True
    call_ahead: bool = False
    restart: bool = True
    vbpr_cols: bool = True
    vbpr_overlap: bool = True


    @classmethod
    def from_env(cls, environ=None):
        env = os.environ if environ is None else environ
        parsers = {
            'flow': _flag, 'flow_max_batch': _int_in(0, 1 << 20), 'flow_waves_per_cu': _int_in(0, 32),
            'flow_item_bufs': lambda n, r: int(_choice('2', '4')(n, r)), 'own': _choice('0', '1', '2'),
            'own_max_batch': _int_in(0, 1024), 'own_waves': _int_in(0, 0xffff), 'fuse_short': _flag, 'fuse_plan': _flag,
            'overlap_min_batch': _int_in(1, 1 << 30), 'epoch_ahead': _flag, 'call_ahead': _flag, 'restart': _flag, 'vbpr_cols': _flag, 'vbpr_overlap': _flag,
        }
        out = cls()
        for f in fields(cls):
            if f.name.startswith('_'):
                continue
            var = 'TKR_' + f.name.upper()
            raw = env.get(var)
            if raw is not None and raw != '':
                setattr(out, f.name, parsers[f.name](var, raw))
        return out
```

top-k-rec_amd/single/_engine.py:

```python
from __future__ import annotations

import numpy as np
import torch

import tkr_hip
from ._config import Tuning

RHO, EPS = 0.9, 1e-10
MAX_PLAN_BATCHES = tkr_hip.PLAN_MAX_BATCHES


def default_device():
    if not torch.cuda.is_available():
        raise tkr_hip.TkrError('no MI355X visible to PyTorch-ROCm: BPR/VBPR training runs only on the '
                               'HIP path (there is no CPU fallback)')
    return torch.device('cuda', torch.cuda.current_device())


class TrainingCSR:

    def __init__(self, tr_data: dict, tr_users, n_users: int, device):
        deg = np.zeros(n_users, dtype=np.int64)
        for u, items in tr_data.items():
            deg[u] = len(items)
        row_ptr = np.zeros(n_users + 1, dtype=np.int64)
        np.cumsum(deg, out=row_ptr[1:])
        order = sorted(tr_data.keys())
        pos = np.fromiter((it for u in order for it in tr_data[u]), dtype=np.int32, count=int(row_ptr[-1])) \
            if len(order) else np.zeros(0, np.int32)
        self._finish(row_ptr, pos, np.asarray(list(tr_users), dtype=np.int32), device)

    @classmethod
    def from_arrays(cls, row_ptr, pos_cols, tr_users, device):
        self = cls.__new__(cls)
        self._finish(np.asarray(row_ptr, dtype=np.int64), np.asarray(pos_cols, dtype=np.int32),
                     np.asarray(tr_users, dtype=np.int32), device)
        return self

    @classmethod
    def shard(cls, row_ptr, pos_cols, owned, device):
        row_ptr = np.asarray(row_ptr, dtype=np.int64)
        owned = np.asarray(owned, dtype=np.int64)
        deg = row_ptr[owned + 1] - row_ptr[owned]
        local_ptr = np.zeros(len(owned) + 1, dtype=np.int64)
        np.cumsum(deg, out=local_ptr[1:])
        take = np.repeat(row_ptr[owned] - local_ptr[:-1], deg) + np.arange(int(local_ptr[-1]), dtype=np.int64)
        self = cls.from_arrays(local_ptr, np.asarray(pos_cols)[take], np.flatnonzero(deg > 0).astype(np.int32), device)
        self.local = True
        return self

    def _finish(self, row_ptr, pos, tr_users, device):
        assert row_ptr[-1] < 2 ** 31
        owner = np.repeat(np.arange(len(row_ptr) - 1, dtype=np.int64), np.diff(row_ptr))
        big = int(pos.max()) + 1 if len(pos) else 1
        srt = (np.sort(owner * big + pos) % big).astype(np.int32)
        self.row_ptr = torch.from_numpy(row_ptr.astype(np.int32)).to(device)
        self.pos_cols = torch.from_numpy(pos).to(device)
        self.cols_sorted = torch.from_numpy(srt).to(device)
        self.tr_users = torch.from_numpy(tr_users).to(device)
        self.nnz = int(row_ptr[-1])


class PlanBuffers:

    def __init__(self, cap: int, B: int, device, flow: bool = False, cols=None, owners: int = 0):
        self.cap, self.B, self.flow, self.cols, self.owners = cap, B, flow, cols, (owners if flow else 0)
        i32 = dict(dtype=torch.int32, device=device)
        if cols is not None:
            d, row_cap = cols
            self.colh = torch.empty(cap * d * 8, **i32)
            self.cent = torch.empty(cap * B * 2 * row_cap * 2, **i32)
            self.tcnt = torch.empty(cap * B, **i32)
            self.tent = torch.empty(cap * B * 2 * row_cap * 2, **i32)
        self.u = torch.empty(cap * B, **i32)
        self.i = torch.empty(cap * B, **i32)
        self.j = torch.empty(cap * B, **i32)
        self.task = torch.empty(cap * 3 * B * 4, **i32)
        self.occ = torch.empty(cap * 3 * B * 2, **i32)
        self.occt = torch.empty(cap * 3 * B, **i32)
        if flow:
            self.prec = torch.empty(cap * 3 * B * 32, **i32)
            self.pocc = torch.empty(cap * 3 * B * 4, **i32)
            if self.owners:
                self.ohdr = torch.zeros(self.owners * cap, **i32)
                self.xch = torch.zeros(cap * B * 2 * 2, **i32)
                self.epoch = 0
        else:
            self.rec_stride = tkr_hip.plan_max_blocks(B) * tkr_hip.plan_team(B) * 16
            self.rec = torch.empty(cap * self.rec_stride, **i32)
            self.hdr = torch.empty(cap * 4, **i32)
            self.tpar = torch.empty(cap * B, **i32)
        self.loss = torch.zeros(cap, dtype=torch.float32, device=device)
        need = tkr_hip.plan_workspace_bytes(B, cap)
        self.ws = torch.empty(need, dtype=torch.uint8, device=device) if need else None


class UpdateCounters:

    def __init__(self, n_users, n_items, device):
        i32 = dict(dtype=torch.int32, device=device)
        self.ucnt = torch.zeros(n_users, **i32)
        self.icnt = torch.zeros(n_items, **i32)
        self.touch_u = torch.zeros(n_users * 16, **i32)
        self.touch_i = torch.zeros(n_items * 16, **i32)


class PlanPipeline:

    _side_streams = {}

    def __init__(self, device, private_side=False):
        self.device = device
        self._private = private_side
        self._side = None
        self.bufs = [None, None]
        self.planned = [None, None]

    @property
    def side(self):
        if self._side is None and self._private:
            self._side = torch.cuda.Stream(device=self.device)
        if self._side is None:
            key = (self.device.type, self.device.index)
            if key not in PlanPipeline._side_streams:
                PlanPipeline._side_streams[key] = torch.cuda.Stream(device=self.device)
            self._side = PlanPipeline._side_streams[key]
        return self._side

    def ensure(self, cap, B, flow=False, cols=None, owners=0):
        for i in range(2):
            b = self.bufs[i]
            if b is None or b.B != B or b.cap < cap or b.flow != flow or b.cols != cols or b.owners != (owners if flow else 0):
                self.bufs[i] = b = None
                self.bufs[i] = PlanBuffers(cap, B, self.device, flow, cols, owners)
                self.planned[i] = None

    def plan(self, i, fn, overlap=True):
        main = torch.cuda.current_stream(self.device)
        if not overlap:
            self.drain()
            fn(self.bufs[i])
            self.planned[i] = None
            return
        with torch.cuda.stream(self.side):
            self.side.wait_stream(main)
            fn(self.bufs[i])
            ev = torch.cuda.Event()
            ev.record(self.side)
            self.planned[i] = ev
        self._side_dirty = True

    def acquire(self, i):
        if self.planned[i] is not None:
            torch.cuda.current_stream(self.device).wait_event(self.planned[i])
            self.planned[i] = None
        return self.bufs[i]

    def drain(self):
        if self._side is not None and getattr(self, '_side_dirty', False):
            torch.cuda.current_stream(self.device).wait_stream(self._side)
            self._side_dirty = False




def _chunk_cap(B):
    if B > 8192:
        return max(2, (1 << 21) // B)
    return min(MAX_PLAN_BATCHES, max(8, (1 << 20) // B))


class _Chunk:
    __slots__ = ('idx', 'nb', 'used', 'B', 'first', 'csr', 'shadow', 'epoch_ahead', 'pending', 'loss_zeroed', 'fused')

    def __init__(self, idx, nb, B, first, csr, shadow=None):
        self.idx, self.nb, self.used, self.B, self.first, self.csr = idx, nb, 0, B, first, csr
        self.shadow, self.epoch_ahead = shadow, shadow is not None
        self.loss_zeroed = False
        self.pending = None
        self.fused = False


class _ShadowCounters:

    def __init__(self, cnt, icnt):
        self.ucnt, self.icnt, self.touch_u, self.touch_i = cnt.ucnt, icnt, cnt.touch_u, cnt.touch_i


def _event_pair():
    return torch.cuda.Event(enable_timing=True), torch.cuda.Event(enable_timing=True)


def _recorded_event_pair():
    pair = _event_pair()
    for e in pair:
        e.record()
    return pair


class PlanMixin:

    def _plan_flow(self):
        return False

    def _plan_owners(self, B):
        return 0

    def prepare(self, B, layout=None):
        """engines with more than one table layout pick the one batch size B runs on"""

    def check(self):
        """raise if the device reported a failed step (engines with a persistent kernel); synchronises"""

    def check_async(self):
        """queue a copy of the device's status word; the NEXT check_async / check / settle raises if it was set (no host wait
        now: the per-epoch exchange of a sharded run calls this instead of check)"""

    def _cap(self, B):
        return _chunk_cap(B)

    def _plan_overlap(self, B):
        if getattr(self, 'plan_in_order', False):
            return False
        return B >= self.cfg.overlap_min_batch or self._plan_flow()

    def _plan_cols(self, B):
        return None

    def _plan_extra(self, buf, nb, B):
        """more planner-side work for the nb batches K1 just wrote into buf (same stream, right behind K1)"""

    def _init_plans(self, tuning=None):
        self.cfg = tuning if tuning is not None else Tuning.from_env()
        self._cnt = UpdateCounters(self.n_users, self.n_items, self.device)
        self._drawn = 0
        self._cur = None
        self._ahead = None
        self.plan = None
        self.pipe = None
        self.step_events = None
        self._event_pool = []
        self._fused_calls = {}
        self._again_key = None
        self._again_buf = 0

    @property
    def cnt(self):
        self.settle()
        return self._cnt

    @property
    def triplets_drawn(self):
        return self._drawn

    @triplets_drawn.setter
    def triplets_drawn(self, value):
        self.settle()
        self._drawn = int(value)

    def reserve_events(self, n):
        while len(self._event_pool) < n:
            self._event_pool.append(_recorded_event_pair())

    def settle(self, check=True, keep_epoch_ahead=False):
        if check:
            self.check()
        if self._cur is None and self._ahead is None:
            return
        ah, cur = self._ahead, self._cur
        if keep_epoch_ahead and ah is not None and ah.epoch_ahead and ah.used == 0 and (cur is None or cur.used == cur.nb):
            return
        self.pipe.drain()
        for ch in (self._ahead, self._cur):
            if ch is not None and ch.used < ch.nb and ch.pending is None:
                buf = self.pipe.bufs[ch.idx]
                cnt = self._cnt if ch.shadow is None else _ShadowCounters(self._cnt, ch.shadow)
                tkr_hip.plan_rollback(buf, ch.B, ch.used, ch.nb - ch.used, cnt)
        self._cur = self._ahead = None

    def after_exchange(self):
        ah = self._ahead
        if ah is None or ah.shadow is None:
            return
        ev = self.pipe.planned[ah.idx]
        if ev is not None:
            torch.cuda.current_stream(self.device).wait_event(ev)
        self._cnt.icnt.copy_(ah.shadow)
        ah.shadow = None

    def _plan_chunk(self, idx, csr, B, first, overlap, want, shadow=None, fuse=False):
        nb = max(1, min(self._cap(B), want))
        cnt = self._cnt if shadow is None else _ShadowCounters(self._cnt, shadow)
        if fuse:
            self.pipe.drain()
            buf = self.pipe.bufs[idx]
            key = ('fused', id(csr), id(cnt.ucnt), id(cnt.icnt), self.seed)
            callers = buf.__dict__.setdefault('_callers', {})
            call = callers.get(key)
            if call is None:
                if len(callers) > 4:
                    callers.clear()
                call = callers[key] = tkr_hip.plan_call(csr, self.n_users, self.n_items, self.seed, B, cnt, buf)
            call.first_triplet, call.n_batches = first, nb
            self.pipe.planned[idx] = None
            ch = _Chunk(idx, nb, B, first, csr, shadow)
            ch.pending, ch.fused = call, shadow is None
            self._fused_calls[idx] = (call, csr, buf)
            return ch

        def fn(buf):
            if shadow is not None:
                shadow.zero_()
            key = (id(csr), id(cnt.ucnt), id(cnt.icnt), self.seed)
            callers = buf.__dict__.setdefault('_callers', {})
            call = callers.get(key)
            if call is None:
                if len(callers) > 4:
                    callers.clear()
                call = callers[key] = tkr_hip.plan_caller(csr, self.n_users, self.n_items, self.seed, B, cnt, buf)
            call(first, nb)
            self._plan_extra(buf, nb, B)
            buf.loss[:nb].zero_()
        self.pipe.plan(idx, fn, overlap)
        ch = _Chunk(idx, nb, B, first, csr, shadow)
        ch.loss_zeroed = True
        return ch

    def _epoch_ahead_ok(self, B):
        return self._plan_flow() and self.cfg.epoch_ahead and not getattr(self, 'plan_in_order', False)

    def _next_chunk(self, csr, B, want, then_exchange=0):
        cur = self._cur
        if cur is not None and (cur.B != B or cur.csr is not csr):
            self.settle(check=False)
            cur = None
        if cur is not None and cur.used < cur.nb:
            return cur
        if self._ahead is not None and self._ahead.shadow is not None:
            self.settle(check=False)
            cur = None
        if self.pipe is None:
            self.pipe = PlanPipeline(self.device, getattr(self, 'private_side_stream', False))
        self.pipe.ensure(self._cap(B), B, self._plan_flow(), self._plan_cols(B), self._plan_owners(B))
        overlap = self._plan_overlap(B)
        if overlap:
            self.pipe.side
        if cur is not None and self._ahead is not None:
            nxt, self._ahead = self._ahead, None
        else:
            fuse = (self.cfg.fuse_short and then_exchange == 0 and want <= self._cap(B) and
                    getattr(getattr(self, '_step', None), 'plan_and_run', None) is not None and self._plan_owners(B) > 0)
            nxt = self._plan_chunk(0 if cur is None else cur.idx ^ 1, csr, B, self._drawn, False, want, fuse=fuse)
        if overlap and want > nxt.nb:
            self._ahead = self._plan_chunk(nxt.idx ^ 1, csr, B, nxt.first + nxt.nb * B, True, want - nxt.nb)
        elif overlap and then_exchange == 0 and not self._plan_flow() and self.cfg.call_ahead and want == nxt.nb and want > 8:
            self._ahead = self._plan_chunk(nxt.idx ^ 1, csr, B, nxt.first + nxt.nb * B, True, nxt.nb)
        elif then_exchange > 0 and want <= nxt.nb and self._epoch_ahead_ok(B):
            if getattr(self, '_shadow_icnt', None) is None:
                self._shadow_icnt = torch.zeros_like(self._cnt.icnt)
            self.pipe.side
            self._ahead = self._plan_chunk(nxt.idx ^ 1, csr, B, nxt.first + nxt.nb * B, True, then_exchange, shadow=self._shadow_icnt)
        self._cur = nxt
        return nxt

    def _run(self, csr, n_batches, B, want_loss, step_fn, then_exchange=0):
        loss, left = None, n_batches
        while left > 0:
            ch = self._next_chunk(csr, B, left, then_exchange)
            plan = self.pipe.acquire(ch.idx)
            m = min(left, ch.nb - ch.used)
            lo = ch.used
            if want_loss and not ch.loss_zeroed and not getattr(step_fn, 'assigns_loss', False):
                plan.loss[lo:lo + m].zero_()
            if ch.pending is not None:
                call, ch.pending = ch.pending, None
                ev = None
                if self.step_events is not None:
                    ev = self._event_pool.pop() if self._event_pool else _recorded_event_pair()
                    self.step_events.append((ev[0], ev[1], m))
                step_fn.plan_and_run(plan, call, lo, m, plan.loss if want_loss else None, ev)
            elif self.step_events is not None:
                e0, e1 = self._event_pool.pop() if self._event_pool else _recorded_event_pair()
                if getattr(step_fn, 'takes_events', False):
                    step_fn(plan, lo, m, plan.loss if want_loss else None, (e0, e1))
                else:
                    e0.record()
                    step_fn(plan, lo, m, plan.loss if want_loss else None)
                    e1.record()
                self.step_events.append((e0, e1, m))
            else:
                step_fn(plan, lo, m, plan.loss if want_loss else None)
            ch.used += m
            left -= m
            self._drawn += m * B
            loss = plan.loss[lo:lo + m] if want_loss else None
            self.plan = plan
        return loss


class DoubleTable:

    def __init__(self, n, k, device, init=None, gen=None):
        shape = (2, n, k) if k else (2, n)
        self.p = torch.zeros(shape, dtype=torch.float32, device=device)
        self.ms = torch.ones(shape, dtype=torch.float32, device=device)
        if init is not None:
            self.p[0].normal_(0.0, init, generator=gen)

    def current(self, cnt):
        sel = (cnt & 1).long()
        idx = torch.arange(self.p.shape[1], device=self.p.device)
        return self.p[sel, idx], self.ms[sel, idx]

    def assign(self, values, ms=None):
        self.mutations = getattr(self, 'mutations', 0) + 1
        self.p[0].copy_(values)
        if ms is not None:
            self.ms[0].copy_(ms)


def _generators(device, seed, user_seed):
    gen = torch.Generator(device=device)
    if user_seed is None:
        gen.manual_seed(seed & 0x7FFFFFFFFFFFFFFF)
        return gen, gen
    gen.manual_seed((seed ^ 0x5BD1E9955BD1E995) & 0x7FFFFFFFFFFFFFFF)
    gen_u = torch.Generator(device=device)
    gen_u.manual_seed(int(user_seed) & 0x7FFFFFFFFFFFFFFF)
    return gen, gen_u


def _tags(t):
    return t.view(torch.int32)[..., 1]


class FlowTable:

    def __init__(self, n, k, device, bufs=2):
        assert bufs in (2, 4)
        self.n, self.k, self.kp, self.bufs = n, k, tkr_hip.flow_row_granules(k), bufs
        self.p = torch.zeros((bufs, n, self.kp, 2), dtype=torch.float32, device=device)
        self.ms = torch.zeros((bufs, n, self.kp, 2), dtype=torch.float32, device=device)

    def current(self, cnt):
        sel = (cnt & (self.bufs - 1)).long()
        idx = torch.arange(self.n, device=self.p.device)
        return self.p[sel, idx, :self.k, 0], self.ms[sel, idx, :self.k, 0]

    def assign(self, values, ms):
        self.mutations = getattr(self, 'mutations', 0) + 1
        for t, v, pad in ((self.p, values, 0.0), (self.ms, ms, 1.0)):
            t.zero_()
            t[0, :, :, 0] = pad
            t[0, :, :self.k, 0] = v
            _tags(t)[1:] = -1


class FlowTail:

    def __init__(self, n, device, bufs=2):
        assert bufs in (2, 4)
        self.n, self.bufs = n, bufs
        self.t = torch.zeros((bufs, n, 2 * bufs, 2), dtype=torch.float32, device=device)
        self.rd = torch.zeros(bufs * n, dtype=torch.int32, device=device)
        _tags(self.t)[1:] = -1

    def current(self, cnt):
        sel = (cnt & (self.bufs - 1)).long()
        idx = torch.arange(self.n, device=self.t.device)
        return self.t[sel, idx, 0, 0], self.t[sel, idx, 1, 0]

    def assign(self, b=None, msb=None):
        self.mutations = getattr(self, 'mutations', 0) + 1
        self.t.zero_()
        if b is not None:
            self.t[0, :, 0, 0] = b
            self.t[0, :, 1, 0] = msb
        _tags(self.t)[1:] = -1
        self.rd.zero_()


class BprEngine(PlanMixin):

    def __init__(self, n_users, n_items, k, hp, device=None, seed=None, user_seed=None, tuning=None):
        self.device = device or default_device()
        self.n_users, self.n_items, self.k = n_users, n_items, k
        self.hp = hp
        self.seed = int(seed if seed is not None else np.random.SeedSequence().entropy % (2 ** 63))
        gen, gen_u = _generators(self.device, self.seed, user_seed)
        self.layout = 'bulk'
        self.layout_epoch = 0
        self.U = DoubleTable(n_users, k, self.device, 0.01, gen_u)
        self.V = DoubleTable(n_items, k, self.device, 0.01, gen)
        self.b = DoubleTable(n_items, 0, self.device)
        self.tailU = self.tailV = self.ctl = None
        self._item_mutations = 0
        self._flow_ran = False
        self._status_host = self._status_event = None
        self._init_plans(tuning)

    @property
    def item_mutations(self):
        return self._item_mutations + sum(getattr(t, 'mutations', 0) for t in (self.V, self.b, self.tailV) if t is not None)

    @item_mutations.setter
    def item_mutations(self, value):
        self._item_mutations = value - sum(getattr(t, 'mutations', 0) for t in (self.V, self.b, self.tailV) if t is not None)

    def _plan_flow(self):
        return self.layout == 'flow'

    def _plan_owners(self, B):
        if self.layout != 'flow' or B > min(self.cfg.own_max_batch, 1024) or self.cfg.own == '0' or getattr(self, '_own_failed', False):
            return 0
        share = max(1, int(getattr(self, 'ranks_on_device', 1)))
        cache = self.__dict__.setdefault('_owners_by_share', {})
        if share not in cache:
            cache[share] = tkr_hip.bpr_own_owners(self.n_items, self.k, self.device, share)
            if cache[share] == 0 and share > 1:
                import warnings
                cus = torch.cuda.get_device_properties(self.device).multi_processor_count if self.device.type == 'cuda' else 0
                warnings.warn('K2o is off: %d ranks share this GPU and %d item rows of width %d do not fit %d owners\' LDS; the persistent '
                              'step without owned rows (K2f) runs instead' % (share, self.n_items, self.k, cus // share))
        if cache[share] < getattr(self, 'own_min_owners', 0):
            return 0
        return cache[share]

    def wants_flow(self, B):
        if B > self.cfg.flow_max_batch or not self.cfg.flow or self.k > tkr_hip.FLOW_MAX_K:
            return False
        if getattr(self, '_flow_disabled', False):
            return False
        if self.layout == 'flow':
            return True
        fits = getattr(self, '_flow_fits', None)
        if fits is None:
            rows = self.n_users + self.n_items
            need = (rows + (self.cfg.flow_item_bufs // 2 - 1) * self.n_items) * (tkr_hip.flow_row_granules(self.k) * 32 + 96 + 8 * self.k)
            free = torch.cuda.mem_get_info(self.device)[0] if self.device.type == 'cuda' else need
            fits = self._flow_fits = need <= 0.7 * free
        return fits

    def prepare(self, B, layout=None):
        layout = layout or ('flow' if self.wants_flow(B) else 'bulk')
        if layout == self.layout:
            return
        self.settle()
        (pu, mu), (pv, mv), (pb, mb) = (tuple(t.clone() for t in self.get(n)) for n in ('U', 'V', 'b'))
        self.U = self.V = self.b = self.tailU = self.tailV = None
        if layout == 'flow':
            self.U, self.V = FlowTable(self.n_users, self.k, self.device), FlowTable(self.n_items, self.k, self.device, self.cfg.flow_item_bufs)
            self.tailU, self.tailV = FlowTail(self.n_users, self.device), FlowTail(self.n_items, self.device, self.cfg.flow_item_bufs)
            if self.ctl is None:
                self.ctl = torch.zeros(tkr_hip.flow_ctl_words(), dtype=torch.int32, device=self.device)
        else:
            self.U, self.V = DoubleTable(self.n_users, self.k, self.device), DoubleTable(self.n_items, self.k, self.device)
            self.b = DoubleTable(self.n_items, 0, self.device)
        self.layout = layout
        self.layout_epoch += 1
        self.item_mutations += 1
        self.U.assign(pu, mu)
        self.V.assign(pv, mv)
        if layout == 'flow':
            self.tailU.assign()
            self.tailV.assign(pb, mb)
        else:
            self.b.assign(pb, mb)
        self._cnt.ucnt.zero_()
        self._cnt.icnt.zero_()

    def _failed(self, code):
        post = self.ctl[tkr_hip.FLOW_CTL_DEBUG:tkr_hip.FLOW_CTL_DEBUG + 16].cpu().tolist()
        self.ctl.zero_()
        self._flow_ran = False
        if getattr(self, '_last_step_kind', None) == 'own':
            self._own_failed = True
            nxt = 'the persistent step without owned rows (K2f)'
        else:
            self._flow_disabled = True
            nxt = 'the per-batch step (K2)'
        self.tables_invalid = True
        self._step_key = None
        raise tkr_hip.StepGaveUp('persistent BPR step gave up waiting for a row version (status %d): tables are invalid; this engine uses %s '
                               'from now on; post-mortem words (csrc/bpr_flow.hip kCtlDebug) %r' % (code, nxt, post))

    def step_down(self):
        if getattr(self, '_last_step_kind', None) == 'own':
            self._own_failed = True
        else:
            self._flow_disabled = True
        self._step_key = None
        self._again_key = None

    def _raise_pending(self):
        ev, self._status_event = self._status_event, None
        if ev is not None:
            ev.synchronize()
            if int(self._status_host[0]) != 0:
                self._failed(int(self._status_host[0]))

    def check(self):
        self._raise_pending()
        if self.ctl is None or not self._flow_ran:
            return
        self._flow_ran = False
        code = int(self.ctl[tkr_hip.FLOW_CTL_STATUS])
        if code != 0:
            self._failed(code)

    def check_async(self):
        self._raise_pending()
        if self.ctl is None or not self._flow_ran:
            return
        self._flow_ran = False
        if self._status_host is None:
            self._status_host = torch.zeros(1, dtype=torch.int32).pin_memory()
        self._status_host.copy_(self.ctl[tkr_hip.FLOW_CTL_STATUS:tkr_hip.FLOW_CTL_STATUS + 1], non_blocking=True)
        self._status_event = torch.cuda.Event()
        self._status_event.record()

    def _hyper_into(self, st):
        hp = self.hp
        st.n_users, st.n_items, st.k = self.n_users, self.n_items, self.k
        st.mode = 0 if hp['mode'] == 'l2' else 1
        st.lu, st.li, st.lj, st.lb, st.lr = hp['lu'], hp['li'], hp['lj'], hp['lb'], hp['lr']
        st.rho, st.eps = RHO, EPS
        st.opt = 1 if hp.get('opt', 'rmsprop') == 'sgd' else 0
        return st

    def state(self):
        if self.layout == 'flow':
            st = tkr_hip.FlowState()
            st.U, st.msU, st.tailU, st.rdU = self.U.p.data_ptr(), self.U.ms.data_ptr(), self.tailU.t.data_ptr(), self.tailU.rd.data_ptr()
            st.V, st.msV, st.tailV, st.rdV = self.V.p.data_ptr(), self.V.ms.data_ptr(), self.tailV.t.data_ptr(), self.tailV.rd.data_ptr()
            st.item_bufs = self.V.bufs
            return self._hyper_into(st)
        st = tkr_hip.BprState()
        st.U, st.msU = self.U.p.data_ptr(), self.U.ms.data_ptr()
        st.V, st.msV = self.V.p.data_ptr(), self.V.ms.data_ptr()
        st.b, st.msb = self.b.p.data_ptr(), self.b.ms.data_ptr()
        return self._hyper_into(st)

    def get(self, name):
        if name == 'U':
            return self.U.current(self.cnt.ucnt)
        if name == 'V':
            return self.V.current(self.cnt.icnt)
        return (self.tailV if self.layout == 'flow' else self.b).current(self.cnt.icnt)

    def set_users(self, U=None, msU=None):
        cur, ms = self.U.current(self.cnt.ucnt)
        self.U.assign(cur.clone() if U is None else self._dev(U), ms.clone() if msU is None else self._dev(msU))
        if self.layout == 'flow':
            self.tailU.assign()
        self._cnt.ucnt.zero_()

    def set_items(self, V=None, b=None, msV=None, msb=None):
        self.item_mutations += 1
        cv, mv = self.V.current(self.cnt.icnt)
        cb, mb = self.get('b')
        nb = cb.clone() if b is None else self._dev(b).reshape(-1)
        nmb = mb.clone() if msb is None else self._dev(msb).reshape(-1)
        self.V.assign(cv.clone() if V is None else self._dev(V), mv.clone() if msV is None else self._dev(msV))
        if self.layout == 'flow':
            self.tailV.assign(nb, nmb)
        else:
            self.b.assign(nb, nmb)
        self._cnt.icnt.zero_()

    replicated_names = ('V', 'b')

    def replicated_tables(self):
        if self.layout == 'flow':
            return []
        return [('V', self.V.p, self.V.ms, self.cnt.icnt), ('b', self.b.p, self.b.ms, self.cnt.icnt)]

    def flow_sync_tables(self):
        if self.layout != 'flow':
            return None
        return self.V.p, self.V.ms, self.tailV.t, self.tailV.rd, self._cnt.icnt, self.n_items, self.k, self.V.bufs

    def snapshot(self):
        snap = {n: tuple(t.clone() for t in self.get(n)) for n in ('U', 'V', 'b')}
        snap['drawn'] = self._drawn
        return snap

    def restore(self, snap):
        self.settle(check=False)
        self._cnt.touch_u.zero_()
        self._cnt.touch_i.zero_()
        self.set_users(U=snap['U'][0], msU=snap['U'][1])
        self.set_items(V=snap['V'][0], b=snap['b'][0], msV=snap['V'][1], msb=snap['b'][1])
        self._drawn = int(snap['drawn'])
        self.tables_invalid = False

    def copy_model_from(self, other):
        p, ms = other.get('U')
        self.set_users(U=p, msU=ms)
        self.set_replicated({n: other.get(n) for n in self.replicated_names})

    def set_replicated(self, new):
        self.set_items(V=new['V'][0], b=new['b'][0], msV=new['V'][1], msb=new['b'][1])

    def _dev(self, a):
        if isinstance(a, torch.Tensor):
            return a.to(self.device, torch.float32)
        return torch.from_numpy(np.ascontiguousarray(a, dtype=np.float32)).to(self.device)

    def run_batches(self, csr: TrainingCSR, n_batches: int, B: int, want_loss=True, then_exchange=0):
        if (self.k > 512 or (self.k > 256 and B > 1024)) and not getattr(self, '_warned_wide', False):
            self._warned_wide = True
            import warnings
            warnings.warn('BPR: k = %d at batch_size = %d is wider than a wave can hold a row in registers beside its partners (k <= 512, '
                          '<= 256 above batch 1024): the generic row form steps (csrc/bpr_step.hip bpr_wide_kernel: every occurrence in two '
                          'passes over k, the gradient sum through memory)' % (self.k, B))
        cfg = self.cfg
        again = (id(csr), 0, B, self.layout_epoch, cfg.own, cfg.own_waves, cfg.fuse_short, cfg.fuse_plan, cfg.own_max_batch, cfg.flow, cfg.flow_max_batch, getattr(self, '_flow_disabled', False),
                 getattr(self, '_own_failed', False), getattr(self, 'ranks_on_device', 1), self.seed)
        if again == getattr(self, '_again_key', None) and then_exchange == 0 and self.step_events is None:
            loss = self._run_again(csr, n_batches, B, want_loss)
            if loss is not False:
                return loss
        self.prepare(B)
        again = again[:3] + (self.layout_epoch,) + again[4:]
        key = (self.layout_epoch, B, self.cfg.flow_waves_per_cu, self._plan_owners(B), self.cfg.own_waves, self.cfg.fuse_plan)
        if getattr(self, '_step_key', None) != key:
            self._step_key, self._step = key, self.step_fn(B)
        self._flow_ran = self._flow_ran or self.layout == 'flow'
        if self.layout == 'flow':
            self._last_step_kind = 'own' if self._plan_owners(B) else 'flow'
        loss = self._run(csr, n_batches, B, want_loss, self._step, then_exchange)
        cur = self._cur
        fused = cur is not None and cur.fused and cur.used == cur.nb and self._ahead is None
        self._again_key, self._again_buf = (again, cur.idx) if fused else (None, 0)
        return loss

    def _run_again(self, csr, n_batches, B, want_loss):
        cur, pipe = self._cur, self.pipe
        if ((cur is not None and cur.used != cur.nb) or self._ahead is not None or getattr(pipe, '_side_dirty', False)
                or getattr(self, 'tables_invalid', False)):
            return False
        if n_batches > self._cap(B):
            return False
        if n_batches <= 0 or (want_loss and not getattr(self._step, 'assigns_loss', False)):
            return False
        idx = self._again_buf ^ 1
        call = self._fused_calls.get(idx)
        if call is None or call[1] is not csr or call[2] is not pipe.bufs[idx]:
            return False
        call, buf = call[0], call[2]
        call.first_triplet, call.n_batches = self._drawn, n_batches
        pipe.planned[idx] = None
        ch = _Chunk(idx, n_batches, B, self._drawn, csr)
        ch.fused = True
        self._step.plan_and_run(buf, call, 0, n_batches, buf.loss if want_loss else None, None)
        ch.used = n_batches
        self._cur, self.plan, self._again_buf = ch, buf, idx
        self._drawn += n_batches * B
        self._flow_ran, self._last_step_kind = True, 'own'
        return buf.loss[:n_batches] if want_loss else None

    def step_fn(self, B):
        state = self.state()
        if self.layout == 'flow':
            if self._plan_owners(B):
                return tkr_hip.own_stepper(state, B, self.ctl, self.cfg.own_waves | (0 if self.cfg.fuse_plan else 0x1000))
            return tkr_hip.flow_stepper(state, B, self.ctl, self.cfg.flow_waves_per_cu)
        return lambda plan, lo, nb, loss: tkr_hip.bpr_run(state, plan, B, nb, loss, first=lo)


class VbprEngine(PlanMixin):

    SPARSE_DENSITY = 0.25
    NARROW_D = 512
    COLS_MAX_BATCH = 1024
    PLAN_BYTES = 768 << 20

    def __init__(self, n_users, n_items, k, d, feat, hp, device=None, seed=None, sparse=None, user_seed=None, tuning=None):
        self.device = device or default_device()
        self.n_users, self.n_items, self.k, self.kh, self.d = n_users, n_items, k, k // 2, d
        self.hp = hp
        self.seed = int(seed if seed is not None else np.random.SeedSequence().entropy % (2 ** 63))
        gen, gen_u = _generators(self.device, self.seed, user_seed)
        kh = self.kh
        self.U = DoubleTable(n_users, 2 * kh, self.device, 0.01, gen_u)
        self.I = DoubleTable(n_items, kh, self.device, 0.01, gen)
        self.irb = DoubleTable(n_items, 0, self.device)
        f32 = dict(dtype=torch.float32, device=self.device)
        self.cem = torch.full((d, kh), 2.0 / (d * k), **f32)
        self.mscem = torch.ones((d, kh), **f32)
        self.icb = torch.zeros(d, **f32)
        self.msicb = torch.ones(d, **f32)
        self.feat = feat if isinstance(feat, torch.Tensor) else torch.from_numpy(np.ascontiguousarray(feat, dtype=np.float32))
        self.feat = self.feat.to(self.device).contiguous()
        assert self.feat.shape == (n_items, d)
        self._init_plans(tuning)
        self.ws = None
        self.sparse = None
        nnz = int(torch.count_nonzero(self.feat))
        if sparse or (sparse is None and (nnz <= self.SPARSE_DENSITY * n_items * d or d <= self.NARROW_D or self.kh > 128)):
            self.sparse = self._sparse_view(self.feat)
            per_row = (self.sparse['f_ptr'][1:] - self.sparse['f_ptr'][:-1])
            self.max_row_nnz, self.avg_row_nnz = int(per_row.max()), float(per_row.float().mean())

    @staticmethod
    def _sparse_view(feat):
        n_items, d = feat.shape
        i32 = torch.int32
        rc = (feat != 0).nonzero()
        f_ptr = torch.zeros(n_items + 1, dtype=torch.int64, device=feat.device)
        f_ptr[1:] = torch.cumsum(torch.bincount(rc[:, 0], minlength=n_items), 0)
        cr = (feat.t() != 0).nonzero()
        c_ptr = torch.zeros(d + 1, dtype=torch.int64, device=feat.device)
        c_ptr[1:] = torch.cumsum(torch.bincount(cr[:, 0], minlength=d), 0)
        assert int(f_ptr[-1]) < 2 ** 31
        return dict(f_ptr=f_ptr.to(i32), f_col=rc[:, 1].to(i32).contiguous(), f_val=feat[rc[:, 0], rc[:, 1]].contiguous(),
                    c_ptr=c_ptr.to(i32), c_item=cr[:, 1].to(i32).contiguous(), c_val=feat[cr[:, 1], cr[:, 0]].contiguous(),
                    item_tag=torch.zeros(n_items + 8, dtype=torch.int64, device=feat.device))

    def wants_cols(self, B):
        if self.sparse is None or not self.cfg.vbpr_cols:
            return False
        return (((self.kh % 4 == 0 and self.kh <= 128) or self.kh > 128) and B <= self.COLS_MAX_BATCH and 0 < self.max_row_nnz <= 1024 and
                tkr_hip.vbpr_colplan_lds_bytes(B, self.d) <= 160 * 1024)

    def _plan_cols(self, B):
        return (self.d, self.max_row_nnz) if self.wants_cols(B) else None

    def _cap(self, B):
        cap = _chunk_cap(B)
        if self.wants_cols(B):
            per_batch = 32 * self.d + 4 * B + 2 * 16 * B * self.max_row_nnz
            cap = max(4, min(cap, self.PLAN_BYTES // per_batch))
        return cap

    def _plan_overlap(self, B):
        return B >= self.cfg.overlap_min_batch or (self.wants_cols(B) and self.cfg.vbpr_overlap)

    def _plan_extra(self, buf, nb, B):
        if buf.cols is not None:
            tkr_hip.vbpr_colplan(self.sparse, self.d, buf, B, nb, buf.cols[1])

    def cols_per_block(self, B):
        lpc = 4 if self.kh <= 16 else 8 if self.kh <= 32 else 16 if self.kh <= 64 else 32
        groups = 256 // lpc
        run = 2.0 * B * self.avg_row_nnz / self.d
        return int(max(1, min(groups, groups * 8 // max(int(run), 1))))

    def state(self):
        hp = self.hp
        st = tkr_hip.VbprState()
        st.U, st.msU, st.I, st.msI = self.U.p.data_ptr(), self.U.ms.data_ptr(), self.I.p.data_ptr(), self.I.ms.data_ptr()
        st.irb, st.msirb = self.irb.p.data_ptr(), self.irb.ms.data_ptr()
        st.cem, st.mscem, st.icb, st.msicb = self.cem.data_ptr(), self.mscem.data_ptr(), self.icb.data_ptr(), self.msicb.data_ptr()
        st.feat = self.feat.data_ptr()
        st.n_users, st.n_items, st.kh, st.d = self.n_users, self.n_items, self.kh, self.d
        st.mode = 0 if hp['mode'] == 'l2' else 1
        st.lu, st.li, st.lj, st.lb, st.le, st.lr = hp['lu'], hp['li'], hp['lj'], hp['lb'], hp['le'], hp['lr']
        st.rho, st.eps = RHO, EPS
        if self.sparse is not None:
            for name, t in self.sparse.items():
                setattr(st, name, t.data_ptr())
        return st

    def get(self, name):
        if name == 'U':
            return self.U.current(self.cnt.ucnt)
        if name == 'I':
            return self.I.current(self.cnt.icnt)
        if name == 'irb':
            return self.irb.current(self.cnt.icnt)
        return {'cem': (self.cem, self.mscem), 'icb': (self.icb, self.msicb)}[name]

    _dev = BprEngine._dev

    def set_users(self, U=None, msU=None):
        cur, ms = self.U.current(self.cnt.ucnt)
        self.U.assign(cur if U is None else self._dev(U), ms if msU is None else self._dev(msU))
        self.cnt.ucnt.zero_()

    def set_items(self, I=None, irb=None, msI=None, msirb=None):
        ci, mi = self.I.current(self.cnt.icnt)
        cb, mb = self.irb.current(self.cnt.icnt)
        self.I.assign(ci if I is None else self._dev(I), mi if msI is None else self._dev(msI))
        self.irb.assign(cb if irb is None else self._dev(irb).reshape(-1), mb if msirb is None else self._dev(msirb).reshape(-1))
        self.cnt.icnt.zero_()

    def set_dense(self, cem=None, icb=None, mscem=None, msicb=None):
        for dst, src in ((self.cem, cem), (self.icb, icb), (self.mscem, mscem), (self.msicb, msicb)):
            if src is not None:
                dst.copy_(self._dev(src).reshape(dst.shape))

    def set_replicated(self, new):
        self.set_items(I=new['I'][0], irb=new['irb'][0], msI=new['I'][1], msirb=new['irb'][1])
        self.set_dense(cem=new['cem'][0], icb=new['icb'][0], mscem=new['cem'][1], msicb=new['icb'][1])

    replicated_names = ('I', 'irb', 'cem', 'icb')

    def replicated_tables(self):
        return [('I', self.I.p, self.I.ms, self.cnt.icnt), ('irb', self.irb.p, self.irb.ms, self.cnt.icnt),
                ('cem', self.cem, self.mscem, None), ('icb', self.icb, self.msicb, None)]
    copy_model_from = BprEngine.copy_model_from

    def run_batches(self, csr: TrainingCSR, n_batches: int, B: int, want_loss=True, then_exchange=0):
        if self.kh > 128 and self.sparse is None:
            raise ValueError('VBPR: k // 2 = %d takes the CSR view of feat (sparse=True or None): the dense fp32-MFMA view holds at most '
                             '128 factors' % self.kh)
        if B > 65536 and not getattr(self, '_warned_big', False):
            self._warned_big = True
            import warnings
            warnings.warn('VBPR: batch_size = %d: the objective sums over all B^2 = %.3g pairs of a batch (vbpr.py:61,64 broadcast to [B, B]), '
                          'so the pair sums of every batch are O(B^2) work' % (B, float(B) * B))
        if self.kh > 128 and not getattr(self, '_warned_wide', False):
            self._warned_wide = True
            import warnings
            warnings.warn('VBPR: k // 2 = %d is wider than the step\'s kernels hold a row in registers (128): the generic form steps '
                          '(csrc/vbpr_wide.hip: every kernel walks the factors in passes of its threads; the column plan where it applies, '
                          'the five-launch sparse view elsewhere)' % self.kh)
        if getattr(self, '_step_key', None) != B:
            self._step_key, self._step = B, self.step_fn(B)
        return self._run(csr, n_batches, B, want_loss, self._step)

    def step_fn(self, B):
        need = tkr_hip.vbpr_workspace_floats(B, self.kh, self.d)
        if self.ws is None or self.ws.numel() < need:
            self.ws = torch.empty(need, dtype=torch.float32, device=self.device)
        state = self.state()
        if self.wants_cols(B):
            d, row_cap, cpb = self.d, self.max_row_nnz, self.cols_per_block(B)
            return lambda plan, lo, nb, loss: tkr_hip.vbpr_run_cols(state, plan, B, nb, self.ws, d, row_cap, cpb, loss, first=lo)
        return lambda plan, lo, nb, loss: tkr_hip.vbpr_run(state, plan, B, nb, self.ws, loss, first=lo)
```

top-k-rec_amd/tkr_hip.py:

```python
from __future__ import annotations

import ctypes as C
import warnings
import os

import torch

_HERE = os.path.dirname(os.path.abspath(__file__))
LIB_PATH = os.environ.get('TKR_HIP_LIB') or os.path.join(_HERE, 'libtkr_hip.so')

_lib = None
VERSION = 120


class TkrError(RuntimeError):
    pass


class StepGaveUp(TkrError):
    """a bounded spin of a persistent step kernel ran out: the tables of the run are invalid, the engine has stepped down to the
    next kernel (K2o -> K2f -> K2) and works again once valid tables are put back (BPR.train does)"""


class BprState(C.Structure):
    _fields_ = [('U', C.c_void_p), ('msU', C.c_void_p),
                ('V', C.c_void_p), ('msV', C.c_void_p), ('b', C.c_void_p), ('msb', C.c_void_p),
                ('n_users', C.c_int32), ('n_items', C.c_int32), ('k', C.c_int32), ('mode', C.c_int32),
                ('lu', C.c_float), ('li', C.c_float), ('lj', C.c_float), ('lb', C.c_float),
                ('lr', C.c_float), ('rho', C.c_float), ('eps', C.c_float), ('opt', C.c_int32)]


class PlanCall(C.Structure):
    _fields_ = [(n, C.c_void_p) for n in ('tr_users', 'row_ptr', 'pos_cols', 'cols_sorted', 'ucnt', 'icnt', 'touch_u', 'touch_i', 'out_u', 'out_i',
                                           'out_j', 'task', 'occ', 'occt', 'prec', 'pocc', 'ohdr')] + \
               [('seed', C.c_uint64), ('first_triplet', C.c_uint64)] + \
               [(n, C.c_int32) for n in ('n_tr', 'n_users', 'n_items', 'n_batches', 'batch_size', 'n_owner', 'ohdr_stride', 'reserved')]


def plan_call(csr, n_users, n_items, seed, B, cnt, plan):
    assert plan.owners > 0
    for t in (csr.tr_users, csr.row_ptr, csr.pos_cols, csr.cols_sorted, cnt.ucnt, cnt.icnt, cnt.touch_u, cnt.touch_i, plan.u, plan.task):
        assert t.is_cuda and t.is_contiguous()
    assert cnt.ucnt.numel() == n_users and cnt.icnt.numel() == n_items
    pc = PlanCall()
    for name, t in (('tr_users', csr.tr_users), ('row_ptr', csr.row_ptr), ('pos_cols', csr.pos_cols), ('cols_sorted', csr.cols_sorted),
                    ('ucnt', cnt.ucnt), ('icnt', cnt.icnt), ('touch_u', cnt.touch_u), ('touch_i', cnt.touch_i), ('out_u', plan.u),
                    ('out_i', plan.i), ('out_j', plan.j), ('task', plan.task), ('occ', plan.occ), ('occt', plan.occt), ('prec', plan.prec),
                    ('pocc', plan.pocc), ('ohdr', plan.ohdr)):
        setattr(pc, name, t.data_ptr())
    pc.seed, pc.n_tr, pc.n_users, pc.n_items, pc.batch_size = seed, int(csr.tr_users.numel()), n_users, n_items, B
    pc.n_owner, pc.ohdr_stride = plan.owners, plan.cap
    pc.keep = (csr, cnt)
    return pc


class FlowState(C.Structure):
    _fields_ = [(n, C.c_void_p) for n in ('U', 'msU', 'tailU', 'rdU', 'V', 'msV', 'tailV', 'rdV')] + \
               [(n, C.c_int32) for n in ('n_users', 'n_items', 'k', 'mode')] + \
               [(n, C.c_float) for n in ('lu', 'li', 'lj', 'lb', 'lr', 'rho', 'eps')] + [('opt', C.c_int32), ('item_bufs', C.c_int32)]


class VbprState(C.Structure):
    _fields_ = [(n, C.c_void_p) for n in ('U', 'msU', 'I', 'msI', 'irb', 'msirb', 'cem', 'mscem', 'icb', 'msicb', 'feat')] + \
               [(n, C.c_int32) for n in ('n_users', 'n_items', 'kh', 'd', 'mode')] + \
               [(n, C.c_float) for n in ('lu', 'li', 'lj', 'lb', 'le', 'lr', 'rho', 'eps')] + \
               [(n, C.c_void_p) for n in ('f_ptr', 'f_col', 'f_val', 'c_ptr', 'c_item', 'c_val', 'item_tag')]


EXPORTS = ('tkr_version', 'tkr_plan_team', 'tkr_plan_max_blocks', 'tkr_sample_plan', 'tkr_sample_plan_owned', 'tkr_plan_rollback', 'tkr_bpr_run', 'tkr_bpr_flow_run', 'tkr_bpr_own_run', 'tkr_bpr_own_run_between', 'tkr_bpr_own_plan_run', 'tkr_bpr_own_owners', 'tkr_bpr_own_owners_shared', 'tkr_flow_row_granules', 'tkr_flow_ctl_words',
           'tkr_vbpr_run', 'tkr_vbpr_colplan', 'tkr_vbpr_run_cols', 'tkr_build_rated_mask', 'tkr_score_topk', 'tkr_count_hits', 'tkr_calib_rowcopy',
           'tkr_idmap_create', 'tkr_idmap_destroy', 'tkr_ratings_parse', 'tkr_ratings_sizes', 'tkr_ratings_copy',
           'tkr_ratings_destroy', 'tkr_matrix_read', 'tkr_matrix_sizes', 'tkr_matrix_copy', 'tkr_matrix_destroy',
           'tkr_matrix_write', 'tkr_raw_ranks', 'tkr_count_hits_rr', 'tkr_topk_set_math', 'tkr_vbpr_set_pairs', 'tkr_lab_build',
           'tkr_sync_snapshot', 'tkr_sync_pack', 'tkr_sync_unpack', 'tkr_sync_flow_snapshot', 'tkr_sync_flow_pack',
           'tkr_sync_flow_unpack', 'tkr_like_ranks', 'tkr_bpr_foldin', 'tkr_bpr_foldin_items', 'tkr_idtable_build', 'tkr_ratings_count_dev',
           'tkr_ratings_emit_dev', 'tkr_rank_candidates', 'tkr_lists_format_sizes_dev', 'tkr_lists_format_emit_dev',
           'tkr_matrix_format_sizes_dev', 'tkr_matrix_format_emit_dev', 'tkr_matrix_count_dev', 'tkr_matrix_emit_dev', 'tkr_matrix_token_host',
           'tkr_matrix_tokens_host')
EXPORTS_I64 = ('tkr_vbpr_workspace_floats', 'tkr_vbpr_colplan_lds_bytes', 'tkr_topk_workspace_bytes_for', 'tkr_topk_workspace_bytes', 'tkr_plan_workspace_bytes', 'tkr_like_ranks_workspace_bytes',
               'tkr_parse_dev_workspace_bytes', 'tkr_idtable_slots', 'tkr_scan_dev_workspace_bytes')


def lib():
    global _lib
    if _lib is None:
        if not os.path.exists(LIB_PATH):
            raise TkrError('%s not found: build it with `make -C top-k-rec_amd/csrc` '
                           '(or __graft_entry__.build()); there is no CPU fallback' % LIB_PATH)
        _lib = C.CDLL(LIB_PATH)
        for name in EXPORTS:
            getattr(_lib, name).restype = C.c_int
        for name in EXPORTS_I64:
            getattr(_lib, name).restype = C.c_int64
        if _lib.tkr_version() != VERSION:
            raise TkrError('%s is version %d, this binding expects %d: rebuild it (make -C top-k-rec_amd/csrc)'
                           % (LIB_PATH, _lib.tkr_version(), VERSION))
    return _lib


def _check(rc, what):
    if rc != 0:
        kind = 'hipError_t' if rc > 0 else 'tkr error'
        raise TkrError('%s failed: %s %d' % (what, kind, rc))


def _p(t):
    if t is None:
        return C.c_void_p(0)
    assert t.is_cuda and t.is_contiguous(), 'device-resident contiguous tensor required'
    return C.c_void_p(t.data_ptr())


def _call(name, anchor, *args):
    dev = anchor.device.index
    prev = torch.cuda.current_device()
    if prev != dev:
        torch.cuda.set_device(dev)
    try:
        _check(getattr(lib(), name)(*args, C.c_void_p(torch.cuda.current_stream(anchor.device).cuda_stream)), name)
    finally:
        if prev != dev:
            torch.cuda.set_device(prev)


def version():
    return lib().tkr_version()


PLAN_MAX_BATCHES = 512


def plan_team(B):
    return lib().tkr_plan_team(C.c_int32(B))


def plan_workspace_bytes(B, n_batches):
    return int(lib().tkr_plan_workspace_bytes(C.c_int32(B), C.c_int32(n_batches)))


def plan_max_blocks(B):
    return lib().tkr_plan_max_blocks(C.c_int32(B))


def sample_plan(csr, n_users, n_items, seed, first_triplet, n_batches, B, cnt, plan, ctl=None):
    assert n_batches <= PLAN_MAX_BATCHES
    assert plan.u.numel() >= n_batches * B and plan.task.numel() >= n_batches * 3 * B * 4
    prec, pocc = getattr(plan, 'prec', None), getattr(plan, 'pocc', None)
    if getattr(plan, 'owners', 0) > 0:
        assert ctl is None and prec.numel() >= n_batches * 3 * B * 32 and pocc.numel() >= n_batches * 3 * B * 4
        assert plan.ohdr.numel() >= plan.owners * plan.cap and plan.cap >= n_batches
        _call('tkr_sample_plan_owned', plan.u, _p(csr.tr_users), C.c_int32(csr.tr_users.numel()), _p(csr.row_ptr), _p(csr.pos_cols),
              _p(csr.cols_sorted), C.c_int32(n_users), C.c_int32(n_items), C.c_uint64(seed), C.c_uint64(first_triplet),
              C.c_int32(n_batches), C.c_int32(B), _p(cnt.ucnt), _p(cnt.icnt), _p(cnt.touch_u), _p(cnt.touch_i), _p(plan.u), _p(plan.i),
              _p(plan.j), _p(plan.task), _p(plan.occ), _p(plan.occt), _p(prec), _p(pocc), C.c_int32(plan.owners), _p(plan.ohdr),
              C.c_int32(plan.cap))
        return
    ws = getattr(plan, 'ws', None)
    assert ws is None or ws.numel() >= plan_workspace_bytes(B, n_batches)
    assert B <= 8192 or ws is not None
    if prec is not None:
        assert prec.numel() >= n_batches * 3 * B * 32 and pocc.numel() >= n_batches * 3 * B * 4
    else:
        assert plan.rec.numel() >= n_batches * plan_max_blocks(B) * plan_team(B) * 16 and plan.hdr.numel() >= n_batches * 4
    assert cnt.ucnt.numel() == n_users and cnt.touch_u.numel() == n_users * 16
    assert cnt.icnt.numel() == n_items and cnt.touch_i.numel() == n_items * 16
    _call('tkr_sample_plan', plan.u, _p(csr.tr_users), C.c_int32(csr.tr_users.numel()), _p(csr.row_ptr), _p(csr.pos_cols),
                                 _p(csr.cols_sorted), C.c_int32(n_users), C.c_int32(n_items), C.c_uint64(seed),
                                 C.c_uint64(first_triplet), _p(ctl), C.c_int32(n_batches), C.c_int32(B),
                                 _p(cnt.ucnt), _p(cnt.icnt), _p(cnt.touch_u), _p(cnt.touch_i),
                                 _p(plan.u), _p(plan.i), _p(plan.j), _p(plan.task), _p(plan.occ), _p(getattr(plan, 'rec', None)),
                                 _p(getattr(plan, 'hdr', None)), _p(plan.occt), _p(getattr(plan, 'tpar', None)), _p(prec), _p(pocc),
                                 _p(ws), C.c_int64(ws.numel() if ws is not None else 0))


_PLAN_ARGTYPES = [C.c_void_p, C.c_int32, C.c_void_p, C.c_void_p, C.c_void_p, C.c_int32, C.c_int32, C.c_uint64, C.c_uint64, C.c_void_p,
                  C.c_int32, C.c_int32] + [C.c_void_p] * 15 + [C.c_void_p, C.c_int64, C.c_void_p]


def plan_caller(csr, n_users, n_items, seed, B, cnt, plan):
    sample_plan.__doc__
    prec, pocc = getattr(plan, 'prec', None), getattr(plan, 'pocc', None)
    ws = getattr(plan, 'ws', None)
    assert B <= 8192 or ws is not None
    assert cnt.ucnt.numel() == n_users and cnt.touch_u.numel() == n_users * 16
    assert cnt.icnt.numel() == n_items and cnt.touch_i.numel() == n_items * 16
    cap = plan.u.numel() // B
    fn = lib().tkr_sample_plan
    fn.argtypes = _PLAN_ARGTYPES
    ptr = lambda t: None if t is None else t.data_ptr()
    for t in (csr.tr_users, csr.row_ptr, csr.pos_cols, csr.cols_sorted, cnt.ucnt, cnt.icnt, cnt.touch_u, cnt.touch_i, plan.u, plan.task):
        assert t.is_cuda and t.is_contiguous()
    fixed_a = (ptr(csr.tr_users), int(csr.tr_users.numel()), ptr(csr.row_ptr), ptr(csr.pos_cols), ptr(csr.cols_sorted), n_users, n_items, seed)
    fixed_b = (ptr(cnt.ucnt), ptr(cnt.icnt), ptr(cnt.touch_u), ptr(cnt.touch_i), ptr(plan.u), ptr(plan.i), ptr(plan.j), ptr(plan.task), ptr(plan.occ),
               ptr(getattr(plan, 'rec', None)), ptr(getattr(plan, 'hdr', None)), ptr(plan.occt), ptr(getattr(plan, 'tpar', None)), ptr(prec), ptr(pocc),
               ptr(ws), int(ws.numel()) if ws is not None else 0)
    device = plan.u.device
    keep = (csr, cnt)
    owners = getattr(plan, 'owners', 0)
    if owners > 0:
        fo = lib().tkr_sample_plan_owned
        fo.argtypes = [C.c_void_p, C.c_int32, C.c_void_p, C.c_void_p, C.c_void_p, C.c_int32, C.c_int32, C.c_uint64, C.c_uint64, C.c_int32,
                       C.c_int32] + [C.c_void_p] * 12 + [C.c_int32, C.c_void_p, C.c_int32, C.c_void_p]
        tail = (ptr(cnt.ucnt), ptr(cnt.icnt), ptr(cnt.touch_u), ptr(cnt.touch_i), ptr(plan.u), ptr(plan.i), ptr(plan.j), ptr(plan.task),
                ptr(plan.occ), ptr(plan.occt), ptr(prec), ptr(pocc), owners, ptr(plan.ohdr), plan.cap)

        def call_owned(first_triplet, n_batches):
            assert 0 < n_batches <= min(cap, PLAN_MAX_BATCHES) and keep
            prev = torch.cuda.current_device()
            if prev != device.index:
                torch.cuda.set_device(device.index)
            try:
                rc = fo(*fixed_a, first_triplet, n_batches, B, *tail, torch.cuda.current_stream(device).cuda_stream)
            finally:
                if prev != device.index:
                    torch.cuda.set_device(prev)
            if rc:
                _check(rc, 'tkr_sample_plan_owned')
        return call_owned

    def call(first_triplet, n_batches):
        assert 0 < n_batches <= min(cap, PLAN_MAX_BATCHES) and keep
        if torch.cuda.current_device() != device.index:
            prev = torch.cuda.current_device()
            torch.cuda.set_device(device.index)
            try:
                rc = fn(*fixed_a, first_triplet, None, n_batches, B, *fixed_b, torch.cuda.current_stream(device).cuda_stream)
            finally:
                torch.cuda.set_device(prev)
            if rc:
                _check(rc, 'tkr_sample_plan')
            return
        rc = fn(*fixed_a, first_triplet, None, n_batches, B, *fixed_b, torch.cuda.current_stream(device).cuda_stream)
        if rc:
            _check(rc, 'tkr_sample_plan')
    return call


def plan_rollback(plan, B, first_batch, n_batches, cnt):
    _call('tkr_plan_rollback', plan.task, _p(plan.task), C.c_int32(B), C.c_int32(first_batch), C.c_int32(n_batches),
                                   _p(cnt.ucnt), _p(cnt.icnt))


def _at(t, offset):
    if t is None:
        return C.c_void_p(0)
    assert t.is_cuda and t.is_contiguous() and 0 <= offset <= t.numel()
    return C.c_void_p(t.data_ptr() + offset * t.element_size())


def bpr_run(state, plan, B, n_batches, loss_out=None, first=0):
    rs = plan_max_blocks(B) * plan_team(B) * 16
    _call('tkr_bpr_run', plan.rec, C.byref(state), _at(plan.rec, first * rs), _at(plan.occ, first * 6 * B), _at(plan.hdr, first * 4),
                             C.c_int32(B), C.c_int32(n_batches), _at(loss_out, first))


FLOW_MAX_K = 256


def flow_row_granules(k):
    return int(lib().tkr_flow_row_granules(C.c_int32(k)))


def flow_ctl_words():
    return int(lib().tkr_flow_ctl_words())


FLOW_CTL_ARRIVE, FLOW_CTL_STATUS, FLOW_CTL_SPINS = 1024, 1026, 1027
FLOW_CTL_DEBUG, FLOW_CTL_PROF = 1032, 1056


def bpr_flow_run(state, plan, B, n_batches, ctl, loss_out=None, first=0, waves_per_cu=0):
    _call('tkr_bpr_flow_run', plan.prec, C.byref(state), _at(plan.prec, first * 3 * B * 32), _p(plan.pocc), C.c_int32(B),
          C.c_int32(n_batches), _p(ctl), _p(loss_out), C.c_int32(waves_per_cu))


def flow_stepper(state, B, ctl, waves_per_cu=0):
    fn = lib().tkr_bpr_flow_run
    fn.argtypes = [C.c_void_p, C.c_void_p, C.c_void_p, C.c_int32, C.c_int32, C.c_void_p, C.c_void_p, C.c_int32, C.c_void_p]
    device, st = ctl.device, C.addressof(state)
    ctl_ptr, rec_bytes = ctl.data_ptr(), 3 * B * 32 * 4

    def step(plan, first, n_batches, loss_out):
        if torch.cuda.current_device() != device.index:
            return bpr_flow_run(state, plan, B, n_batches, ctl, loss_out, first, waves_per_cu)
        rc = fn(st, plan.prec.data_ptr() + first * rec_bytes, plan.pocc.data_ptr(), B, n_batches, ctl_ptr,
                None if loss_out is None else loss_out.data_ptr(), waves_per_cu, torch.cuda.current_stream(device).cuda_stream)
        if rc:
            _check(rc, 'tkr_bpr_flow_run')
    step.state = state
    return step


def bpr_own_owners(n_items, k, device=None, share=1):
    if device is not None and torch.cuda.current_device() != device.index:
        with torch.cuda.device(device):
            return int(lib().tkr_bpr_own_owners_shared(C.c_int32(n_items), C.c_int32(k), C.c_int32(share)))
    return int(lib().tkr_bpr_own_owners_shared(C.c_int32(n_items), C.c_int32(k), C.c_int32(share)))


def bpr_own_run(state, plan, B, n_batches, ctl, loss_out=None, first=0, owner_waves=0):
    plan.epoch += 1
    _call('tkr_bpr_own_run', plan.prec, C.byref(state), _p(plan.prec), _p(plan.pocc), _p(plan.occt), _p(plan.ohdr), C.c_int32(plan.cap), C.c_int32(plan.owners),
          C.c_int32(B), C.c_int32(first), C.c_int32(n_batches), _p(ctl), _p(loss_out), C.c_int32(owner_waves), _p(plan.xch),
          C.c_uint32(plan.epoch & 0xffffffff or 1))


def own_stepper(state, B, ctl, owner_waves=0):
    fn = lib().tkr_bpr_own_run_between
    fn.argtypes = [C.c_void_p, C.c_void_p, C.c_void_p, C.c_void_p, C.c_void_p, C.c_void_p, C.c_void_p, C.c_int32, C.c_int32, C.c_int32, C.c_int32,
                   C.c_int32, C.c_void_p, C.c_void_p, C.c_int32, C.c_void_p, C.c_uint32, C.c_void_p]
    device, st, ctl_ptr = ctl.device, C.addressof(state), ctl.data_ptr()

    def step(plan, first, n_batches, loss_out, events=None):
        if torch.cuda.current_device() != device.index:
            assert events is None
            return bpr_own_run(state, plan, B, n_batches, ctl, loss_out, first, owner_waves)
        plan.epoch += 1
        rc = fn(None if events is None else events[0].cuda_event, None if events is None else events[1].cuda_event,
                st, plan.prec.data_ptr(), plan.pocc.data_ptr(), plan.occt.data_ptr(), plan.ohdr.data_ptr(), plan.cap, plan.owners, B, first, n_batches,
                ctl_ptr, None if loss_out is None else loss_out.data_ptr(), owner_waves, plan.xch.data_ptr(), plan.epoch & 0xffffffff or 1,
                torch.cuda.current_stream(device).cuda_stream)
        if rc:
            _check(rc, 'tkr_bpr_own_run_between')
    fused = lib().tkr_bpr_own_plan_run
    fused.argtypes = [C.c_void_p, C.c_void_p, C.c_int32, C.c_int32, C.c_void_p, C.c_void_p, C.c_int32, C.c_void_p, C.c_uint32, C.c_void_p,
                      C.c_void_p, C.c_void_p]

    raw_stream = getattr(torch._C, '_cuda_getCurrentRawStream', None)
    dev_index = device.index

    def plan_and_run(plan, call, first, n_batches, loss_out, events=None):
        assert torch.cuda.current_device() == dev_index and 0 < call.n_batches <= min(plan.cap, PLAN_MAX_BATCHES)
        plan.epoch += 1
        stream = raw_stream(dev_index) if raw_stream is not None else torch.cuda.current_stream(device).cuda_stream
        rc = fused(C.addressof(call), st, first, n_batches, ctl_ptr, None if loss_out is None else loss_out.data_ptr(), owner_waves,
                   plan.xch.data_ptr(), plan.epoch & 0xffffffff or 1, None if events is None else events[0].cuda_event,
                   None if events is None else events[1].cuda_event, stream)
        if rc:
            _check(rc, 'tkr_bpr_own_plan_run')
    step.state = state
    step.takes_events = True
    step.plan_and_run = plan_and_run
    step.assigns_loss = True
    return step


def set_vbpr_pairs(mode):
    _check(lib().tkr_vbpr_set_pairs(C.c_int32(int(mode))), 'tkr_vbpr_set_pairs')


def vbpr_workspace_floats(B, kh, d):
    return int(lib().tkr_vbpr_workspace_floats(C.c_int32(B), C.c_int32(kh), C.c_int32(d)))


def vbpr_run(state, plan, B, n_batches, workspace, loss_out=None, first=0):
    rs = plan_max_blocks(B) * plan_team(B) * 16
    _call('tkr_vbpr_run', plan.rec, C.byref(state), _at(plan.i, first * B), _at(plan.j, first * B), _at(plan.rec, first * rs),
                              _at(plan.occ, first * 6 * B), _at(plan.hdr, first * 4), _at(plan.occt, first * 3 * B),
                              _at(plan.u, first * B), _at(getattr(plan, 'tpar', None), first * B), C.c_int32(B),
                              C.c_int32(n_batches), _p(workspace), _at(loss_out, first))


def vbpr_colplan_lds_bytes(B, d):
    return int(lib().tkr_vbpr_colplan_lds_bytes(C.c_int32(B), C.c_int32(d)))


def vbpr_colplan(sparse, d, plan, B, n_batches, row_cap):
    tcap = 2 * row_cap
    assert plan.colh.numel() >= n_batches * d * 8 and plan.cent.numel() >= n_batches * B * tcap * 2
    assert plan.tcnt.numel() >= n_batches * B and plan.tent.numel() >= n_batches * B * tcap * 2
    _call('tkr_vbpr_colplan', plan.i, _p(sparse['f_ptr']), _p(sparse['f_col']), _p(sparse['f_val']), C.c_int32(d), _p(plan.i), _p(plan.j),
          C.c_int32(B), C.c_int32(n_batches), C.c_int32(row_cap), _p(plan.colh), _p(plan.cent), _p(plan.tcnt), _p(plan.tent))


def vbpr_run_cols(state, plan, B, n_batches, workspace, d, row_cap, cols_per_block=0, loss_out=None, first=0):
    rs = plan_max_blocks(B) * plan_team(B) * 16
    ent = B * 2 * row_cap * 2
    _call('tkr_vbpr_run_cols', plan.rec, C.byref(state), _at(plan.i, first * B), _at(plan.j, first * B), _at(plan.rec, first * rs),
          _at(plan.occ, first * 6 * B), _at(plan.hdr, first * 4), _at(plan.occt, first * 3 * B), _at(plan.u, first * B),
          _at(plan.tpar, first * B), _at(plan.colh, first * d * 8), _at(plan.cent, first * ent), _at(plan.tcnt, first * B),
          _at(plan.tent, first * ent), C.c_int32(row_cap), C.c_int32(cols_per_block), C.c_int32(B), C.c_int32(n_batches), _p(workspace),
          _at(loss_out, first))


def build_rated_mask(rated_ptr, rated_cols, n_rows, n_cols):
    assert rated_ptr.dtype == torch.int64 and rated_cols.dtype == torch.int32
    pitch = (n_rows + 31) // 32 * 32
    mask = torch.zeros(((n_cols + 31) // 32) * pitch, dtype=torch.int32, device=rated_ptr.device)
    if rated_cols.numel() == 0:
        rated_cols = torch.zeros(1, dtype=torch.int32, device=rated_ptr.device)
    _call('tkr_build_rated_mask', mask, _p(rated_ptr), _p(rated_cols), C.c_int32(n_rows), C.c_int32(n_cols), _p(mask), C.c_int32(pitch))
    return mask, pitch


_topk_ws = {}


def _topk_workspace(n_rows, K, device, n_cols=0, k=0):
    need = int(lib().tkr_topk_workspace_bytes_for(C.c_int32(n_rows), C.c_int32(n_cols), C.c_int32(k), C.c_int32(K)))
    ws = _topk_ws.get(device)
    if ws is None or ws.numel() < need:
        ws = _topk_ws[device] = torch.empty(need, dtype=torch.uint8, device=device)
    return ws


TOPK_MAX_K = 32


def _score_topk_once(U, Vt, K, bias, user_idx, mask, mask_pitch, want_scores, split):
    n_rows = int(user_idx.numel()) if user_idx is not None else int(U.shape[0])
    ids = torch.empty((n_rows, K), dtype=torch.int32, device=U.device)
    scores = torch.empty((n_rows, K), dtype=torch.float32, device=U.device) if want_scores else None
    ws = _topk_workspace(n_rows, K, U.device, int(Vt.shape[0]), int(U.shape[1])) if split else None
    _call('tkr_score_topk', U, _p(U), _p(user_idx), C.c_int32(n_rows), _p(Vt), _p(bias), C.c_int32(Vt.shape[0]),
                                C.c_int32(U.shape[1]), _p(mask), C.c_int32(mask_pitch), C.c_int32(K), _p(ids),
                                _p(scores), _p(ws), C.c_int64(ws.numel() if ws is not None else 0))
    return ids, scores


TOPK_MATH_DEFAULT = 'refine'


def set_topk_math(mode):
    _check(lib().tkr_topk_set_math(C.c_int32({'bf16x3': 0, 'fp32': 1, 'refine': 2}[mode])), 'tkr_topk_set_math')


def lab():
    return bool(lib().tkr_lab_build())


def score_topk(U, Vt, K, bias=None, user_idx=None, mask=None, mask_pitch=0, want_scores=False, split=True):
    assert U.dtype == torch.float32 and Vt.dtype == torch.float32 and U.shape[1] == Vt.shape[1]
    if U.shape[1] > 768 and not getattr(score_topk, '_warned_wide', False):
        score_topk._warned_wide = True
        warnings.warn('K4: factor width %d is above 768, where a workgroup\'s users no longer stay resident as MFMA operands: the generic '
                      'form runs (one wave per row, every lane gathers its own item row: csrc/topk.hip score_topk_wide_kernel)' % U.shape[1])
    if K <= TOPK_MAX_K:
        ids, scores = _score_topk_once(U, Vt, K, bias, user_idx, mask, mask_pitch, want_scores, split)
        return (ids, scores) if want_scores else ids
    n_rows = int(user_idx.numel()) if user_idx is not None else int(U.shape[0])
    n_cols = int(Vt.shape[0])
    pitch = mask_pitch if mask is not None else (n_rows + 31) // 32 * 32
    work = mask.clone() if mask is not None else torch.zeros(((n_cols + 31) // 32) * pitch, dtype=torch.int32, device=U.device)
    ptr = torch.arange(0, (n_rows + 1) * TOPK_MAX_K, TOPK_MAX_K, dtype=torch.int64, device=U.device)
    parts_i, parts_s, left = [], [], K
    while left > 0:
        ids, scores = _score_topk_once(U, Vt, TOPK_MAX_K, bias, user_idx, work, pitch, want_scores, split)
        take = min(left, TOPK_MAX_K)
        parts_i.append(ids[:, :take])
        if want_scores:
            parts_s.append(scores[:, :take])
        left -= take
        if left > 0:
            _call('tkr_build_rated_mask', work, _p(ptr), _p(ids.reshape(-1)), C.c_int32(n_rows), C.c_int32(n_cols), _p(work), C.c_int32(pitch))
    ids = torch.cat(parts_i, dim=1).contiguous()
    return (ids, torch.cat(parts_s, dim=1).contiguous()) if want_scores else ids


def count_hits(ids, like_ptr, like_cols, step, interval):
    assert ids.dtype == torch.int32 and like_ptr.dtype == torch.int64 and like_cols.dtype == torch.int32
    first = torch.zeros(max(interval, 1), dtype=torch.int64, device=ids.device)
    if like_cols.numel() == 0:
        like_cols = torch.zeros(1, dtype=torch.int32, device=ids.device)
    _call('tkr_count_hits', ids, _p(ids), C.c_int32(ids.shape[0]), C.c_int32(ids.shape[1]), _p(like_ptr), _p(like_cols),
                                C.c_int32(step), C.c_int32(interval), _p(first))
    return torch.cumsum(first[:interval], 0)


def raw_ranks(U, Vt, ids, rated_ptr, rated_cols, bias=None, user_idx=None):
    assert ids.dtype == torch.int32 and rated_ptr.dtype == torch.int64 and rated_cols.dtype == torch.int32
    n_rows, K = int(ids.shape[0]), int(ids.shape[1])
    out = torch.empty((n_rows, K), dtype=torch.int32, device=ids.device)
    if rated_cols.numel() == 0:
        rated_cols = torch.zeros(1, dtype=torch.int32, device=ids.device)
    _call('tkr_raw_ranks', ids, _p(U), _p(user_idx), C.c_int32(n_rows), _p(Vt), _p(bias), C.c_int32(U.shape[1]), _p(rated_ptr),
                               _p(rated_cols), _p(ids), C.c_int32(K), _p(out))
    return out


def count_hits_rr(ids, raw_rank, like_ptr, like_cols, step, interval):
    n_rows = int(ids.shape[0])
    hit = torch.zeros((n_rows, max(interval, 1)), dtype=torch.int32, device=ids.device)
    rr = torch.zeros((n_rows, max(interval, 1)), dtype=torch.float64, device=ids.device)
    if like_cols.numel() == 0:
        like_cols = torch.zeros(1, dtype=torch.int32, device=ids.device)
    if interval > 0:
        _call('tkr_count_hits_rr', ids, _p(ids), _p(raw_rank), C.c_int32(n_rows), C.c_int32(ids.shape[1]), _p(like_ptr),
                                       _p(like_cols), C.c_int32(step), C.c_int32(interval), _p(hit), _p(rr))
    return torch.cumsum(hit.sum(0, dtype=torch.int64)[:interval], 0), torch.cumsum(rr.sum(0)[:interval], 0)


def like_ranks(U, Vt, like_ptr, like_cols, bias=None, user_idx=None, mask=None, mask_pitch=0):
    assert U.dtype == torch.float32 and Vt.dtype == torch.float32 and U.shape[1] == Vt.shape[1]
    assert like_ptr.dtype == torch.int64 and like_cols.dtype == torch.int32
    n_rows = int(user_idx.numel()) if user_idx is not None else int(U.shape[0])
    assert like_ptr.numel() == n_rows + 1
    n_likes, n_cols, k = int(like_cols.numel()), int(Vt.shape[0]), int(U.shape[1])
    out = torch.empty(n_likes, dtype=torch.int32, device=U.device)
    if n_likes == 0:
        return out
    need = int(lib().tkr_like_ranks_workspace_bytes(C.c_int32(n_rows), C.c_int32(n_cols), C.c_int32(k), C.c_int64(n_likes)))
    ws = torch.empty(need, dtype=torch.uint8, device=U.device)
    _call('tkr_like_ranks', U, _p(U), _p(user_idx), C.c_int32(n_rows), _p(Vt), _p(bias), C.c_int32(n_cols), C.c_int32(k), _p(mask),
          C.c_int32(mask_pitch), _p(like_ptr), _p(like_cols), _p(out), _p(ws), C.c_int64(need))
    return out


CANDIDATES_RESIDENT = 2048


def _cand_args(U, Vt, cand_ptr, cand_cols, bias, user_idx, mask, mask_pitch):
    named = dict(U=(U, torch.float32), Vt=(Vt, torch.float32), cand_ptr=(cand_ptr, torch.int64), cand_cols=(cand_cols, torch.int32),
                 bias=(bias, torch.float32), user_idx=(user_idx, torch.int32), mask=(mask, torch.int32))
    for name, (t, dtype) in named.items():
        if t is None and name in ('bias', 'user_idx', 'mask'):
            continue
        if not isinstance(t, torch.Tensor):
            raise TypeError('rank_candidates: %s must be a tensor' % name)
        if t.dtype != dtype:
            raise TypeError('rank_candidates: %s must be %s, not %s' % (name, dtype, t.dtype))
        if not t.is_contiguous():
            raise ValueError('rank_candidates: %s must be contiguous' % name)
    for name, (t, _) in named.items():
        if t is not None and (not t.is_cuda or t.device != U.device):
            raise ValueError('rank_candidates: %s must live on the GPU that holds U, not on %s' % (name, t.device))
    if U.dim() != 2 or Vt.dim() != 2 or U.shape[1] != Vt.shape[1] or U.shape[1] < 1 or Vt.shape[0] < 1:
        raise ValueError('rank_candidates: U [*, k] and Vt [n_cols, k] must share k >= 1')
    n_rows = int(user_idx.numel()) if user_idx is not None else int(U.shape[0])
    n_cols, k, nnz = int(Vt.shape[0]), int(U.shape[1]), int(cand_cols.numel())
    if cand_ptr.dim() != 1 or cand_cols.dim() != 1 or cand_ptr.numel() != n_rows + 1:
        raise ValueError('rank_candidates: cand_ptr must hold n_rows + 1 = %d entries' % (n_rows + 1))
    if bias is not None and bias.numel() != n_cols:
        raise ValueError('rank_candidates: bias must hold one value per column')
    if mask is not None and (mask_pitch < n_rows or mask.numel() < ((n_cols + 31) // 32) * mask_pitch):
        raise ValueError('rank_candidates: the mask is not the bitmap of build_rated_mask for %d rows and %d columns' % (n_rows, n_cols))
    if n_rows and not (int(cand_ptr[0]) == 0 and int(cand_ptr[-1]) == nnz and bool((cand_ptr[1:] >= cand_ptr[:-1]).all())):
        raise ValueError('rank_candidates: cand_ptr must run from 0 to len(cand_cols) = %d and never decrease' % nnz)
    return n_rows, n_cols, k, nnz


def rank_candidates(U, Vt, cand_ptr, cand_cols, bias=None, user_idx=None, mask=None, mask_pitch=0):
    n_rows, n_cols, k, nnz = _cand_args(U, Vt, cand_ptr, cand_cols, bias, user_idx, mask, mask_pitch)
    scores = torch.empty(nnz, dtype=torch.float32, device=U.device)
    ranks = torch.empty(nnz, dtype=torch.int32, device=U.device)
    if nnz == 0 or n_rows == 0:
        return scores, ranks
    _call('tkr_rank_candidates', U, _p(U), _p(user_idx), C.c_int32(n_rows), _p(Vt), _p(bias), C.c_int32(n_cols), C.c_int32(k),
          _p(cand_ptr), _p(cand_cols), _p(mask), C.c_int32(mask_pitch), _p(scores), _p(ranks))
    return scores, ranks


def topk_from_ranks(cand_ptr, cand_cols, scores, ranks, K):
    n_rows = int(cand_ptr.numel()) - 1
    dev = cand_cols.device
    ids = torch.full((n_rows, K), -1, dtype=torch.int32, device=dev)
    out = torch.full((n_rows, K), float('-inf'), dtype=torch.float32, device=dev)
    keep = (ranks >= 0) & (ranks < K)
    row = torch.repeat_interleave(torch.arange(n_rows, device=dev), cand_ptr[1:] - cand_ptr[:-1])[keep]
    at = row * K + ranks[keep].long()
    ids.view(-1)[at] = cand_cols[keep]
    out.view(-1)[at] = scores[keep]
    return ids, out


FOLDIN_MAX_TRIPLETS = 64
FOLDIN_REG_MAX_K = 512
ROLE_ALWAYS_POSITIVE = 0xffffffff


def _fold_csr(ptr, idx, bound, what):
    assert ptr.dtype == torch.int64 and idx.dtype == torch.int32
    assert int(ptr[0]) == 0 and int(ptr[-1]) == idx.numel() and bool((ptr[1:] >= ptr[:-1]).all()), 'the row pointer does not describe %s' % what
    assert idx.numel() == 0 or (0 <= int(idx.min()) and int(idx.max()) < bound), '%s holds an index outside [0, %d)' % (what, bound)
    return idx if idx.numel() else torch.zeros(1, dtype=torch.int32, device=idx.device)


def _fold_warn_wide(name, row, k):
    if k > FOLDIN_REG_MAX_K and name not in _fold_warn_wide.seen:
        _fold_warn_wide.seen.add(name)
        warnings.warn('%s: factor width %d is above %d, where a wave no longer holds its %s row in registers: the generic form runs '
                      '(row, slot and gradient sum in LDS, two passes over the gathered rows per triplet: csrc/fold_rows.h fold_wide_kernel)'
                      % (name, k, FOLDIN_REG_MAX_K, row))


_fold_warn_wide.seen = set()


def _fold_outputs(m, steps, triplets, width, want_loss, want_triplets, device):
    loss = torch.zeros(m, dtype=torch.float32, device=device) if want_loss else None
    trip = torch.full((m, steps, triplets, width), -1, dtype=torch.int32, device=device) if want_triplets else None
    return loss, trip


def fold_in(V, b, hist_ptr, hist_cols, *, lu, lr, mode='l2', steps, triplets, seed, first_row=0, U0=None, want_loss=False,
            want_triplets=False):
    assert V.dtype == torch.float32 and V.dim() == 2
    m, (n_items, k) = int(hist_ptr.numel()) - 1, V.shape
    if not 1 <= triplets <= FOLDIN_MAX_TRIPLETS or steps < 1 or m < 0:
        raise ValueError('fold_in: 1 <= triplets <= %d and steps >= 1 required' % FOLDIN_MAX_TRIPLETS)
    assert b is None or (b.dtype == torch.float32 and b.numel() == n_items)
    assert U0 is None or (U0.dtype == torch.float32 and tuple(U0.shape) == (m, k))
    hist_cols = _fold_csr(hist_ptr, hist_cols, n_items, 'hist_cols')
    _fold_warn_wide('K9', 'user', k)
    U = torch.empty((m, k), dtype=torch.float32, device=V.device)
    loss, trip = _fold_outputs(m, steps, triplets, 2, want_loss, want_triplets, V.device)
    if m:
        _call('tkr_bpr_foldin', V, _p(V), _p(b), C.c_int32(n_items), C.c_int32(k), _p(hist_ptr), _p(hist_cols), C.c_int32(m), _p(U0),
              C.c_float(lu), C.c_float(lr), C.c_int32({'l2': 0, 'l1': 1}[mode]), C.c_int32(steps), C.c_int32(triplets),
              C.c_uint64(seed & 0xffffffffffffffff), C.c_uint64(first_row), _p(U), _p(loss), _p(trip))
    out = (U,) + ((loss,) if want_loss else ()) + ((trip,) if want_triplets else ())
    return out[0] if len(out) == 1 else out


def fold_in_items(U, V, b, user_ptr, user_cols, liker_ptr, liker_rows, role_thresh, *, li, lj, lb, lr, mode='l2', steps, triplets, seed,
                  first_row=0, V0=None, b0=None, want_loss=False, want_triplets=False):
    assert U.dtype == torch.float32 and V.dtype == torch.float32 and U.dim() == 2 and V.dim() == 2 and U.shape[1] == V.shape[1]
    (n_users, k), n_items, m = U.shape, int(V.shape[0]), int(liker_ptr.numel()) - 1
    if not 1 <= triplets <= FOLDIN_MAX_TRIPLETS or steps < 1 or m < 0:
        raise ValueError('fold_in_items: 1 <= triplets <= %d and steps >= 1 required' % FOLDIN_MAX_TRIPLETS)
    assert int(user_ptr.numel()) == n_users + 1
    assert b is None or (b.dtype == torch.float32 and b.numel() == n_items)
    assert V0 is None or (V0.dtype == torch.float32 and tuple(V0.shape) == (m, k))
    assert b0 is None or (b0.dtype == torch.float32 and b0.numel() == m)
    user_cols = _fold_csr(user_ptr, user_cols, n_items, 'user_cols')
    liker_rows = _fold_csr(liker_ptr, liker_rows, n_users, 'liker_rows')
    thresh = torch.as_tensor(role_thresh, dtype=torch.int64).reshape(-1)
    assert thresh.numel() == m and (m == 0 or (0 <= int(thresh.min()) and int(thresh.max()) <= ROLE_ALWAYS_POSITIVE))
    thresh = torch.where(thresh >= 2 ** 31, thresh - 2 ** 32, thresh).to(torch.int32).to(V.device)
    _fold_warn_wide('K10', 'item', k)
    Vn = torch.empty((m, k), dtype=torch.float32, device=V.device)
    bn = torch.empty(m, dtype=torch.float32, device=V.device)
    loss, trip = _fold_outputs(m, steps, triplets, 3, want_loss, want_triplets, V.device)
    if m:
        _call('tkr_bpr_foldin_items', V, _p(U), _p(V), _p(b), C.c_int32(n_users), C.c_int32(n_items), C.c_int32(k), _p(user_ptr), _p(user_cols),
              _p(liker_ptr), _p(liker_rows), _p(thresh), C.c_int32(m), _p(V0), _p(b0), C.c_float(li), C.c_float(lj), C.c_float(lb),
              C.c_float(lr), C.c_int32({'l2': 0, 'l1': 1}[mode]), C.c_int32(steps), C.c_int32(triplets), C.c_uint64(seed & 0xffffffffffffffff),
              C.c_uint64(first_row), _p(Vn), _p(bn), _p(loss), _p(trip))
    return (Vn, bn) + ((loss,) if want_loss else ()) + ((trip,) if want_triplets else ())


PARSE_CHUNK_MIN, PARSE_CHUNK_MAX = 64, 1 << 20


def idtable_build(blob, index):
    import numpy as np
    n = int(index.shape[0])
    n_slots = int(lib().tkr_idtable_slots(C.c_int64(n)))
    if n_slots < 0:
        raise TkrError('tkr_idtable_slots failed: tkr error %d' % n_slots)
    slots = np.empty((n_slots, 4), dtype=np.int32)
    _check(lib().tkr_idtable_build(blob, C.c_int64(len(blob)), index.ctypes.data_as(C.c_void_p), C.c_int64(n),
                                   slots.ctypes.data_as(C.c_void_p), C.c_int64(n_slots)), 'tkr_idtable_build')
    return slots


def parse_dev_workspace_bytes(n_bytes, chunk_bytes):
    need = int(lib().tkr_parse_dev_workspace_bytes(C.c_int64(n_bytes), C.c_int64(chunk_bytes)))
    if need < 0:
        raise ValueError('parse on the device: chunk_bytes must be a power of two in [%d, %d], got %r' % (PARSE_CHUNK_MIN, PARSE_CHUNK_MAX, chunk_bytes))
    return need


def ratings_count_dev(text, chunk_bytes, workspace, totals):
    assert text.dtype == torch.uint8 and totals.dtype == torch.int64 and totals.numel() == 2 and workspace.dtype == torch.uint8
    _call('tkr_ratings_count_dev', workspace, _p(text), C.c_int64(text.numel()), C.c_int64(chunk_bytes), _p(workspace), C.c_int64(workspace.numel()),
          _p(totals))


def ratings_emit_dev(text, chunk_bytes, workspace, n_lines, n_entries, user_table, item_table, status):
    dev = workspace.device
    line_start = torch.empty(n_lines, dtype=torch.int64, device=dev)
    line_user = torch.empty(n_lines, dtype=torch.int32, device=dev)
    line_ptr = torch.empty(n_lines + 1, dtype=torch.int64, device=dev)
    item = torch.empty(n_entries, dtype=torch.int32, device=dev)
    like = torch.empty(n_entries, dtype=torch.int32, device=dev)
    (us, ub, ul), (vs, vb, vl) = user_table, item_table
    assert us.dtype == torch.int32 and vs.dtype == torch.int32 and ub.dtype == torch.uint8 and vb.dtype == torch.uint8 and status.dtype == torch.int64
    _call('tkr_ratings_emit_dev', workspace, _p(text), C.c_int64(text.numel()), C.c_int64(chunk_bytes), _p(workspace), C.c_int64(workspace.numel()),
          C.c_int64(n_lines), C.c_int64(n_entries), _p(us), C.c_int64(us.shape[0]), _p(ub), C.c_int64(ul), _p(vs), C.c_int64(vs.shape[0]), _p(vb),
          C.c_int64(vl), _p(line_start), _p(line_user), _p(line_ptr), _p(item), _p(like), _p(status))
    return line_user, line_ptr, item, like


def format_totals(totals, what):
    size, bad = (int(v) for v in totals)
    if bad != -1:
        raise TkrError('%s: row %d holds an index that names no token of its table' % (what, bad))
    return size


def _list_args(ids, scores, row_user, user_tokens, item_tokens):
    assert ids.dtype == torch.int32 and scores.dtype == torch.float32 and row_user.dtype == torch.int32
    assert ids.dim() == 2 and ids.shape == scores.shape and row_user.numel() == ids.shape[0]
    args = [_p(ids), _p(scores), _p(row_user), C.c_int64(ids.shape[0]), C.c_int32(ids.shape[1])]
    for blob, blob_len, start, length in (user_tokens, item_tokens):
        assert blob.dtype == torch.uint8 and start.dtype == torch.int64 and length.dtype == torch.int32 and start.numel() == length.numel()
        assert blob_len <= blob.numel()
        args += [_p(blob), C.c_int64(blob_len), _p(start), _p(length), C.c_int64(length.numel())]
    return args


def lists_format_sizes(ids, scores, row_user, user_tokens, item_tokens):
    n = int(ids.shape[0])
    line_ptr = torch.empty(n + 1, dtype=torch.int64, device=ids.device)
    totals = torch.empty(2, dtype=torch.int64, device=ids.device)
    _call('tkr_lists_format_sizes_dev', line_ptr, *_list_args(ids, scores, row_user, user_tokens, item_tokens), _p(line_ptr), _p(totals))
    return line_ptr, totals


def format_emit_check(status, what):
    bad = int(status.item())
    if bad != -1:
        raise TkrError('%s: line_ptr does not describe the text of row %d' % (what, bad))


def lists_format_emit(ids, scores, row_user, user_tokens, item_tokens, line_ptr, first_row, n_rows, out):
    assert out.dtype == torch.uint8 and line_ptr.dtype == torch.int64 and line_ptr.numel() == ids.shape[0] + 1
    status = torch.empty(1, dtype=torch.int64, device=ids.device)
    _call('tkr_lists_format_emit_dev', line_ptr, *_list_args(ids, scores, row_user, user_tokens, item_tokens), _p(line_ptr),
          C.c_int64(first_row), C.c_int64(n_rows), _p(out), C.c_int64(out.numel()), _p(status))
    return status


def matrix_format_sizes(data):
    assert data.dtype == torch.float32 and data.dim() == 2
    line_ptr = torch.empty(data.shape[0] + 1, dtype=torch.int64, device=data.device)
    totals = torch.empty(2, dtype=torch.int64, device=data.device)
    _call('tkr_matrix_format_sizes_dev', line_ptr, _p(data) if data.numel() else C.c_void_p(0), C.c_int64(data.shape[0]), C.c_int64(data.shape[1]),
          _p(line_ptr), _p(totals))
    return line_ptr, totals


def matrix_format_emit(data, line_ptr, first_row, n_rows, out):
    assert out.dtype == torch.uint8 and line_ptr.dtype == torch.int64 and line_ptr.numel() == data.shape[0] + 1
    status = torch.empty(1, dtype=torch.int64, device=data.device)
    _call('tkr_matrix_format_emit_dev', line_ptr, _p(data) if data.numel() else C.c_void_p(0), C.c_int64(data.shape[0]), C.c_int64(data.shape[1]),
          _p(line_ptr), C.c_int64(first_row), C.c_int64(n_rows), _p(out), C.c_int64(out.numel()), _p(status))
    return status


def scan_dev_workspace_bytes(n_bytes, chunk_bytes):
    need = int(lib().tkr_scan_dev_workspace_bytes(C.c_int64(n_bytes), C.c_int64(chunk_bytes)))
    if need < 0:
        raise ValueError('read on the device: chunk_bytes must be a power of two in [%d, %d], got %r' % (PARSE_CHUNK_MIN, PARSE_CHUNK_MAX, chunk_bytes))
    return need


def matrix_count_dev(text, chunk_bytes, workspace, totals):
    assert text.dtype == torch.uint8 and totals.dtype == torch.int64 and totals.numel() == 3 and workspace.dtype == torch.uint8
    _call('tkr_matrix_count_dev', workspace, _p(text), C.c_int64(text.numel()), C.c_int64(chunk_bytes), _p(workspace), C.c_int64(workspace.numel()),
          _p(totals))


def matrix_emit_dev(text, chunk_bytes, workspace, n_lines, n_tokens, cols):
    dev = workspace.device
    tok_start = torch.empty(n_tokens, dtype=torch.int64, device=dev)
    data = torch.empty(n_tokens, dtype=torch.float32, device=dev)
    hard = torch.empty((n_tokens + 63) // 64, dtype=torch.int64, device=dev)
    counts = torch.empty(2, dtype=torch.int64, device=dev)
    _call('tkr_matrix_emit_dev', workspace, _p(text), C.c_int64(text.numel()), C.c_int64(chunk_bytes), _p(workspace), C.c_int64(workspace.numel()),
          C.c_int64(n_lines), C.c_int64(n_tokens), C.c_int64(cols), _p(tok_start), _p(data), _p(hard), _p(counts))
    return tok_start, data, hard, counts


def matrix_token_host(token: bytes):
    out = C.c_float()
    rc = lib().tkr_matrix_token_host(token, C.c_int64(len(token)), C.byref(out))
    if rc < 0:
        raise TkrError('tkr_matrix_token_host failed: tkr error %d' % rc)
    return bytes(memoryview(out).cast('B')) if rc == 1 else None


def matrix_tokens_host(text, start):
    import numpy as np
    out = np.empty(len(start), dtype=np.float32)
    rc = lib().tkr_matrix_tokens_host(C.c_void_p(text.ctypes.data), C.c_int64(text.size), C.c_void_p(start.ctypes.data), C.c_int64(len(start)),
                                      C.c_void_p(out.ctypes.data))
    return rc, out


def sync_snapshot(P, cnt, start, n, w):
    _call('tkr_sync_snapshot', P, _p(P), _p(cnt), _p(start), C.c_int64(n), C.c_int32(w))


def sync_pack(P, ms, cnt, start, flat_delta, flat_ms, n, w, inv_world):
    _call('tkr_sync_pack', P, _p(P), _p(ms), _p(cnt), _p(start), _p(flat_delta), _p(flat_ms), C.c_int64(n), C.c_int32(w),
                               C.c_float(inv_world))


def sync_flow_snapshot(V, tailV, icnt, start, n, k, item_bufs=2):
    _call('tkr_sync_flow_snapshot', V, _p(V), _p(tailV), _p(icnt), _p(start), C.c_int32(n), C.c_int32(k), C.c_int32(item_bufs))


def sync_flow_pack(V, msV, tailV, icnt, start, flat_delta, flat_ms, n, k, inv_world, item_bufs=2):
    _call('tkr_sync_flow_pack', V, _p(V), _p(msV), _p(tailV), _p(icnt), _p(start), _p(flat_delta), _p(flat_ms), C.c_int32(n),
          C.c_int32(k), C.c_float(inv_world), C.c_int32(item_bufs))


def sync_flow_unpack(V, msV, tailV, rdV, icnt, start, flat_delta, flat_ms, n, k, item_bufs=2):
    _call('tkr_sync_flow_unpack', V, _p(V), _p(msV), _p(tailV), _p(rdV), _p(icnt), _p(start), _p(flat_delta), _p(flat_ms),
          C.c_int32(n), C.c_int32(k), C.c_int32(item_bufs))


def sync_unpack(P, ms, start, flat_delta, flat_ms, n, w):
    _call('tkr_sync_unpack', P, _p(P), _p(ms), _p(start), _p(flat_delta), _p(flat_ms), C.c_int64(n), C.c_int32(w))
```

Before: 42.32 million.

## Let owner kernel span multiple plan sub-blocks per launch and drop dot-mark tracking

Adds a span mode where one owner-kernel launch can process more batches than the planner's per-call limit. Plan records are rebased per sub-block of PLAN_MAX_BATCHES using a base offset, and the LDS-residency test is adjusted to match. The per-task dotmark window and the head_batch atomic are removed, which frees LDS and an atomic per task. A new helper computes the largest batch count that fits in LDS. The aim is fewer launches and less per-launch sync overhead, at the cost of added complexity in the index mapping and a risk of LDS overflow when the batch count is large.

```diff
diff --git a/include/tkr.h b/include/tkr.h
--- a/include/tkr.h
+++ b/include/tkr.h
@@ -80,6 +80,17 @@
                           uint32_t* touch_i, int32_t* out_u, int32_t* out_i, int32_t* out_j, int32_t* task, int32_t* occ,
                           int32_t* occt, int32_t* prec, int32_t* pocc, int32_t n_owner, int32_t* ohdr, int32_t ohdr_stride,
                           void* stream);
+int32_t tkr_bpr_own_max_batches(int32_t n_items, int32_t k, int32_t n_owner);
+int tkr_sample_plan_owned_span(const int32_t* tr_users, int32_t n_tr, const int32_t* row_ptr, const int32_t* pos_cols,
+                               const int32_t* cols_sorted, int32_t n_users, int32_t n_items, uint64_t seed, uint64_t first_triplet,
+                               int32_t n_batches, int32_t batch_size, int32_t* ucnt, int32_t* icnt, uint32_t* touch_u,
+                               uint32_t* touch_i, int32_t* out_u, int32_t* out_i, int32_t* out_j, int32_t* task, int32_t* occ,
+                               int32_t* occt, int32_t* prec, int32_t* pocc, int32_t n_owner, int32_t* ohdr, int32_t ohdr_stride,
+                               void* stream);
+int tkr_bpr_own_run_span(void* ev_before, void* ev_after, const tkr_flow_state* st, const int32_t* prec, const int32_t* pocc,
+                         const int32_t* occt, const int32_t* ohdr, int32_t ohdr_stride, int32_t n_owner, int32_t batch_size,
+                         int32_t first_batch, int32_t n_batches, int32_t sub_batches, uint32_t* ctl, float* loss_out, int32_t owner_waves,
+                         void* xch, uint32_t epoch, void* stream);
 int tkr_bpr_own_run(const tkr_flow_state* st, const int32_t* prec, const int32_t* pocc, const int32_t* occt, const int32_t* ohdr,
                     int32_t ohdr_stride, int32_t n_owner, int32_t batch_size, int32_t first_batch, int32_t n_batches, uint32_t* ctl, float* loss_out,
                     int32_t owner_waves, void* xch, uint32_t epoch, void* stream);
diff --git a/top-k-rec_amd/csrc/bpr_own.hip b/top-k-rec_amd/csrc/bpr_own.hip
--- a/top-k-rec_amd/csrc/bpr_own.hip
+++ b/top-k-rec_amd/csrc/bpr_own.hip
@@ -61,14 +61,17 @@
         return prec[idx16];
     }
 }
-constexpr int kDotWin = 1024;
 
 struct OwnQueue {
     uint32_t head;
     uint32_t total;
     uint32_t arrival;
-    uint32_t head_batch;
+    uint32_t pad;
 };
+
+__host__ __device__ inline size_t own_head_bytes(int nb, int rows_here) {
+    return (sizeof(OwnQueue) + (size_t)4 * (2 * nb + 1 + TKR_WAVE + rows_here) + 15) & ~(size_t)15;
+}
 
 struct QueueMap {
     const uint32_t* pre;
@@ -99,13 +102,15 @@
     uint32_t B;
     const int4* __restrict__ prec;
     __amdgpu_buffer_rsrc_t prec_r;
+    uint32_t lb = 0;
     __device__ __forceinline__ void prefetch(NextTask& nx, int lane) {
         const u64 i64 = (u64)(uint32_t)bcast_i((int)ticket, 0) * (uint32_t)queues + (uint32_t)home;
         const uint32_t idx = i64 < total ? (uint32_t)i64 : 0xffffffffu;
         nx.have = true;
         nx.w = make_int4(0, 0, 0, 0);
         if (idx == 0xffffffffu) { nx.idx = idx; return; }
-        nx.idx = idx + 2u * B * (idx / B);
+        lb = idx / B;
+        nx.idx = idx + 2u * B * lb;
         if (lane < 8) nx.w = plan_ld<PLAN>(prec, prec_r, (size_t)nx.idx * 8 + lane);
     }
 };
@@ -246,7 +251,8 @@
 __global__ __launch_bounds__(own_threads(NP), own_threads(NP) / 256) void bpr_own_kernel(
     tkr_flow_state st, const int4* __restrict__ prec , const int4* __restrict__ pocc,
     const int32_t* __restrict__ occt, const int32_t* __restrict__ ohdr , int ohdr_stride,
-    int first_batch, int nb, int B, int n_owner, int owner_waves, uint32_t tune, uint32_t* __restrict__ ctl, float* __restrict__ loss_out,
+    int first_batch, int nb, int sub ,
+    int B, int n_owner, int owner_waves, uint32_t tune, uint32_t* __restrict__ ctl, float* __restrict__ loss_out,
     u64* __restrict__ xch , uint32_t epoch, PlanArgs pa) {
     constexpr int TPB = own_threads(NP);
     constexpr int NE = 2 * NP;
@@ -272,8 +278,7 @@
     uint32_t* start = pre + nb + 1 + TKR_WAVE;
     const int rows_here = (st.n_items + n_owner - 1) / n_owner;
     uint32_t* tags = start + nb;
-    uint32_t* dotmark = tags + rows_here;
-    float* rows = reinterpret_cast<float*>(smem + ((sizeof(OwnQueue) + (size_t)4 * (2 * nb + 1 + TKR_WAVE + rows_here + kDotWin) + 15) & ~(size_t)15));
+    float* rows = reinterpret_cast<float*>(smem + own_head_bytes(nb, rows_here));
 
     const uint32_t me = blockIdx.x;
     bool alive = true;
@@ -286,7 +291,6 @@
     PLAN_STAMP(0);
     for (int b = threadIdx.x; b < TKR_WAVE; b += TPB) pre[nb + 1 + b] = 0xffffffffu;
     for (int s = threadIdx.x; s < rows_here; s += TPB) tags[s] = kOwnInvalid;
-    for (int s = threadIdx.x; s < kDotWin; s += TPB) dotmark[s] = 0u;
     if constexpr (PLAN) {
         static_assert(TPB == kWideThreads, "phase B of the planner is one thread per task slot");
         unsigned char* scratch = reinterpret_cast<unsigned char*>(rows);
@@ -363,7 +367,7 @@
         }
         uint32_t run = incl - mine;
         for (int b = b0; b < b1; ++b) { run += pre[b + 1]; pre[b + 1] = run; }
-        if (lane == TKR_WAVE - 1) { q->total = incl; q->head = 0u; q->head_batch = 0u; }
+        if (lane == TKR_WAVE - 1) { q->total = incl; q->head = 0u; }
         if (lane == 0) pre[0] = 0u;
     }
     __syncthreads();
@@ -378,7 +382,7 @@
     const __amdgpu_buffer_rsrc_t prec_r = row_rsrc(prec, PLAN ? nb * 3 * B * 128 : 16);
     const uint32_t q_total = q->total;
 
-    auto item_row = [&](const int4 w, ItemRow& r, int& row, int& slot) {
+    auto item_row = [&](const int4 w, int base, ItemRow& r, int& row, int& slot) {
         const int rowk = bcast_i(w.x, 0);
         const uint32_t ver = (uint32_t)bcast_i(w.y, 0);
         const int prev = bcast_i(w.y, 1);
@@ -389,8 +393,8 @@
         r.own_tail = T.tailV + ((size_t)(ver & T.imask) * st.n_items + row) * (2 * item_halves);
         r.own_rd = T.rdV + (T.imask + 1u) * (size_t)row + ((ver + 1u) & T.imask);
         r.ver = ver;
-        r.from_lds = prev >= first_batch;
         r.tag = tags + slot;
+        r.from_lds = prev >= 0 ? prev + base >= first_batch : (base > first_batch && lds_peek(r.tag) != kOwnInvalid);
         r.row = rows + (size_t)slot * ROWF;
         r.halves = item_halves;
         r.rd_staged = false;
@@ -400,13 +404,14 @@
     constexpr uint32_t kItemReaders = 2u;
     if (wave <= owner_waves) {
         uint32_t cur = 0;
+        int base = first_batch - first_batch % sub;
         while (alive) {
             uint32_t pos = 0;
             if (lane == 0) pos = atomicAdd(&q->head, 1u);
             pos = (uint32_t)bcast_i((int)pos, 0);
             if (pos >= q_total) break;
             const uint32_t idx = qm.locate(pos, cur, lane);
-            if (lane == 0) atomicMax(&q->head_batch, cur);
+            while (first_batch + (int)cur - base >= sub) base += sub;
             int4 w = make_int4(0, 0, 0, 0);
             if (lane < 8) w = plan_ld<PLAN>(prec, prec_r, (size_t)idx * 8 + lane);
 #ifdef TKR_OWN_PROF
@@ -416,10 +421,10 @@
 #endif
             ItemRow r;
             int row, slot;
-            item_row(w, r, row, slot);
+            item_row(w, base, r, row, slot);
             const int rowk = bcast_i(w.x, 0);
             const uint32_t ver = r.ver;
-            const int n_occ = bcast_i(w.z, 0), first = bcast_i(w.w, 0);
+            const int n_occ = bcast_i(w.z, 0), first = bcast_i(w.w, 0) + base * 3 * B;
             const size_t woff = (size_t)((ver + 1u) & T.imask) * T.istride + (size_t)row * T.kp;
             float* lrow = rows + (size_t)slot * ROWF;
 
@@ -437,7 +442,6 @@
             alive = run_task<NP, true, NoFeed, LdsOwnStep<NP>, 4>(st, T, lane, n_occ, first, w, pocc, r.own_p, r.own_ms, r.own_tail, ver, own, ms, o, g,
                                                                   gb, loss_lane, false, sgd, ctl, spins, nx, feed, own_step);
             if (!alive) break;
-            if (lane == 0) dotmark[pos & (kDotWin - 1)] = pos + 1u;
 #ifdef TKR_OWN_PROF
             const u64 t1 = __builtin_amdgcn_s_memtime();
 #endif
@@ -471,15 +475,18 @@
         const uint32_t total = (uint32_t)nb * (uint32_t)B;
         NextTask nx;
         nx.idx = 0u; nx.w = make_int4(0, 0, 0, 0); nx.have = false;
+        uint32_t nx_lb = 0;
         while (alive) {
             if (!nx.have) {
                 UserTicketSrc<PLAN> first_feed{ticket, home, queues, total, (uint32_t)B, prec, prec_r};
                 first_feed.prefetch(nx, lane);
+                nx_lb = first_feed.lb;
                 asm volatile("" : "+v"(nx.w.x), "+v"(nx.w.y), "+v"(nx.w.z), "+v"(nx.w.w) :: "memory");
             }
             const uint32_t idx = nx.idx;
             const int4 w = nx.w;
             if (idx == 0xffffffffu) break;
+            const int batch = first_batch + (int)nx_lb;
             nx.have = false;
             ticket = grab_issue(ctl, lane, home);
             const int rowk = bcast_i(w.x, 0);
@@ -495,8 +502,8 @@
             }
             const uint32_t ver = (uint32_t)bcast_i(w.y, 0);
             const int n_occ = bcast_i(w.z, 0);
-            const int first = bcast_i(w.w, 0);
-            const int batch = bcast_i(w.x, 1);
+            int first = bcast_i(w.w, 0);
+            if (n_occ > 4) first += (batch - batch % sub) * 3 * B;
             const int row = rowk;
 
             const size_t roff = (size_t)(ver & 1u) * T.ustride + (size_t)row * T.kp;
@@ -513,6 +520,7 @@
             GlobalOwn<NP> own_step{T, lane, T.U + roff, T.msU + roff, own_tail, own_rd, ver, sgd, ctl, spins, 2};
             alive = run_task<NP, false, UserTicketSrc<PLAN>, GlobalOwn<NP>, 4>(st, T, lane, n_occ, first, w, pocc, T.U + roff, T.msU + roff, own_tail, ver,
                                                                          own, ms, o, g, gb, loss_lane, want_loss, sgd, ctl, spins, nx, feed, own_step);
+            nx_lb = feed.lb;
             if (!alive) break;
 #ifdef TKR_OWN_PROF
             const u64 t1 = __builtin_amdgcn_s_memtime();
@@ -594,13 +602,12 @@
 
 static size_t own_lds_bytes(int np, int nb, int n_items, int n_owner) {
     const int rows_here = (n_items + n_owner - 1) / n_owner;
-    const size_t head = (sizeof(OwnQueue) + (size_t)4 * (2 * nb + 1 + TKR_WAVE + rows_here + kDotWin) + 15) & ~(size_t)15;
-    return head + (size_t)rows_here * (2 * np * 128 + 8) * 4;
+    return own_head_bytes(nb, rows_here) + (size_t)rows_here * (2 * np * 128 + 8) * 4;
 }
 
 static size_t own_lds_bytes_planned(int np, int nb, int n_items, int n_owner, int B, int npad_items, int own_words) {
     const int rows_here = (n_items + n_owner - 1) / n_owner;
-    const size_t head = (sizeof(OwnQueue) + (size_t)4 * (2 * nb + 1 + TKR_WAVE + rows_here + kDotWin) + 15) & ~(size_t)15;
+    const size_t head = own_head_bytes(nb, rows_here);
     const size_t rows = (size_t)rows_here * (2 * np * 128 + 8) * 4;
     const size_t scratch = plan_scratch_bytes(B, npad_items, n_owner, own_words) + plan_mirror_lds(B);
     return head + (rows > scratch ? rows : scratch);
@@ -616,13 +623,24 @@
     const int owners = cus / share;
     if (owners <= 0) return 0;
     const int np = (k + 127) / 128;
-    if (tkr::own_lds_bytes(np, 512, n_items, owners) > 160 * 1024) return 0;
+    if (tkr::own_lds_bytes(np, 512, n_items, owners) + 4096 > 160 * 1024) return 0;
     return owners;
 }
 extern "C" int32_t tkr_bpr_own_owners(int32_t n_items, int32_t k) { return tkr_bpr_own_owners_shared(n_items, k, 1); }
 
+extern "C" int32_t tkr_bpr_own_max_batches(int32_t n_items, int32_t k, int32_t n_owner) {
+    if (n_items <= 0 || k <= 0 || k > 256 || n_owner <= 0) return 0;
+    const int np = (k + 127) / 128;
+    const size_t budget = 160 * 1024, fixed = tkr::own_lds_bytes(np, 0, n_items, n_owner);
+    if (fixed > budget) return 0;
+    int64_t nb = (int64_t)((budget - fixed) / 8);
+    while (nb > 0 && tkr::own_lds_bytes(np, (int)nb, n_items, n_owner) > budget) --nb;
+    while (nb < (1 << 20) && tkr::own_lds_bytes(np, (int)nb + 1, n_items, n_owner) <= budget) ++nb;
+    return (int32_t)(nb < (1 << 20) ? nb : (1 << 20));
+}
+
 static int own_launch(const tkr_flow_state* st, const int32_t* prec, const int32_t* pocc, const int32_t* occt, const int32_t* ohdr,
-                      int32_t ohdr_stride, int32_t n_owner, int32_t batch_size, int32_t first_batch, int32_t n_batches, uint32_t* ctl,
+                      int32_t ohdr_stride, int32_t n_owner, int32_t batch_size, int32_t first_batch, int32_t n_batches, int32_t sub, uint32_t* ctl,
                       float* loss_out, int32_t owner_waves, void* xch, uint32_t epoch, const tkr::PlanArgs* pa, void* stream) {
     if (!st || !st->U || !st->V || !st->tailU || !st->tailV || !st->rdU || !st->rdV) return TKR_EINVAL;
     if (st->opt != 0 && st->opt != 1) return TKR_EINVAL;
@@ -632,7 +650,7 @@
     if (st->item_bufs != 0 && st->item_bufs != 2 && st->item_bufs != 4) return TKR_EINVAL;
     if (!xch || epoch == 0u) return TKR_EINVAL;
     if (!prec || !pocc || !occt || !ohdr || !ctl || batch_size <= 0 || n_batches < 0 || first_batch < 0 || n_owner <= 0) return TKR_EINVAL;
-    if (ohdr_stride < first_batch + n_batches || n_batches > 512) return TKR_EINVAL;
+    if (ohdr_stride < first_batch + n_batches || sub <= 0) return TKR_EINVAL;
     if (n_batches == 0) return TKR_OK;
     if ((uint64_t)(first_batch + n_batches) * 3u * (uint64_t)batch_size >= 0xffffffffull / 8) return TKR_EUNSUPPORTED;
     const int np = (st->k + 127) / 128;
@@ -682,7 +700,7 @@
     const tkr::PlanArgs no_plan = {};
 #define TKR_OWN_LAUNCH(NPV, PL)                                                                                                           \
     hipLaunchKernelGGL((tkr::bpr_own_kernel<NPV, PL>), dim3(n_owner), dim3(tkr::own_threads(NPV)), lds, s, *st, r4, o4, occt, ohdr, ohdr_stride,   \
-                       first_batch, n_batches, batch_size, n_owner, ow, ktune, ctl, loss_out, static_cast<tkr::u64*>(xch), epoch, PL ? *pa : no_plan)
+                       first_batch, n_batches, sub, batch_size, n_owner, ow, ktune, ctl, loss_out, static_cast<tkr::u64*>(xch), epoch, PL ? *pa : no_plan)
     if (pa) TKR_OWN_LAUNCH(1, true);
     else if (np == 1) TKR_OWN_LAUNCH(1, false);
     else TKR_OWN_LAUNCH(2, false);
@@ -699,8 +717,20 @@
 extern "C" int tkr_bpr_own_run(const tkr_flow_state* st, const int32_t* prec, const int32_t* pocc, const int32_t* occt, const int32_t* ohdr,
                                int32_t ohdr_stride, int32_t n_owner, int32_t batch_size, int32_t first_batch, int32_t n_batches,
                                uint32_t* ctl, float* loss_out, int32_t owner_waves, void* xch, uint32_t epoch, void* stream) {
-    return own_launch(st, prec, pocc, occt, ohdr, ohdr_stride, n_owner, batch_size, first_batch, n_batches, ctl, loss_out, owner_waves, xch, epoch,
-                      nullptr, stream);
+    return own_launch(st, prec, pocc, occt, ohdr, ohdr_stride, n_owner, batch_size, first_batch, n_batches, 0x7fffffff, ctl, loss_out, owner_waves,
+                      xch, epoch, nullptr, stream);
+}
+
+extern "C" int tkr_bpr_own_run_span(void* ev_before, void* ev_after, const tkr_flow_state* st, const int32_t* prec, const int32_t* pocc,
+                                    const int32_t* occt, const int32_t* ohdr, int32_t ohdr_stride, int32_t n_owner, int32_t batch_size,
+                                    int32_t first_batch, int32_t n_batches, int32_t sub_batches, uint32_t* ctl, float* loss_out,
+                                    int32_t owner_waves, void* xch, uint32_t epoch, void* stream) {
+    if (sub_batches <= 0) return TKR_EINVAL;
+    if (ev_before) TKR_CHECK(hipEventRecord((hipEvent_t)ev_before, (hipStream_t)stream));
+    const int rc = own_launch(st, prec, pocc, occt, ohdr, ohdr_stride, n_owner, batch_size, first_batch, n_batches, sub_batches, ctl, loss_out,
+                              owner_waves, xch, epoch, nullptr, stream);
+    if (ev_after) TKR_CHECK(hipEventRecord((hipEvent_t)ev_after, (hipStream_t)stream));
+    return rc;
 }
 
 extern "C" int tkr_bpr_own_run_between(void* ev_before, void* ev_after, const tkr_flow_state* st, const int32_t* prec, const int32_t* pocc,
@@ -745,8 +775,8 @@
         pa.n_plan = n_batches; pa.npad_items = npad; pa.own_words = own_words;
         pa.reg_sort_ok = (npad_bits < 31 && (uint64_t)(plan->n_users > plan->n_items ? plan->n_users : plan->n_items) < (1ull << (32 - npad_bits)) - 1ull) ? 1 : 0;
         if (ev_before) TKR_CHECK(hipEventRecord((hipEvent_t)ev_before, (hipStream_t)stream));
-        const int rc = own_launch(st, plan->prec, plan->pocc, plan->occt, plan->ohdr, plan->ohdr_stride, n_owner, B, 0, n_batches, ctl, loss_out,
-                                  owner_waves, xch, epoch, &pa, stream);
+        const int rc = own_launch(st, plan->prec, plan->pocc, plan->occt, plan->ohdr, plan->ohdr_stride, n_owner, B, 0, n_batches, 0x7fffffff, ctl,
+                                  loss_out, owner_waves, xch, epoch, &pa, stream);
         if (ev_after) TKR_CHECK(hipEventRecord((hipEvent_t)ev_after, (hipStream_t)stream));
         return rc;
     }
diff --git a/top-k-rec_amd/csrc/sampler.hip b/top-k-rec_amd/csrc/sampler.hip
--- a/top-k-rec_amd/csrc/sampler.hip
+++ b/top-k-rec_amd/csrc/sampler.hip
@@ -451,6 +451,26 @@
                             pocc, nullptr, 0, n_owner, ohdr, ohdr_stride, stream);
 }
 
+extern "C" int tkr_sample_plan_owned_span(const int32_t* tr_users, int32_t n_tr, const int32_t* row_ptr,
+                                          const int32_t* pos_cols, const int32_t* cols_sorted, int32_t n_users,
+                                          int32_t n_items, uint64_t seed, uint64_t first_triplet, int32_t n_batches,
+                                          int32_t batch_size, int32_t* ucnt, int32_t* icnt, uint32_t* touch_u, uint32_t* touch_i,
+                                          int32_t* out_u, int32_t* out_i, int32_t* out_j, int32_t* task, int32_t* occ, int32_t* occt,
+                                          int32_t* prec, int32_t* pocc, int32_t n_owner, int32_t* ohdr, int32_t ohdr_stride, void* stream) {
+    if (n_owner <= 0 || n_batches < 0 || batch_size <= 0 || ohdr_stride < n_batches) return TKR_EINVAL;
+    if (!out_u || !out_i || !out_j || !task || !occ || !occt || !prec || !pocc || !ohdr) return TKR_EINVAL;
+    constexpr int sub = 32 * tkr::kTouchWords;
+    for (int32_t done = 0; done < n_batches; done += sub) {
+        const int32_t m = n_batches - done < sub ? n_batches - done : sub;
+        const size_t t = (size_t)done * batch_size, s = 3 * t;
+        const int rc = tkr_sample_plan_owned(tr_users, n_tr, row_ptr, pos_cols, cols_sorted, n_users, n_items, seed, first_triplet + t, m, batch_size,
+                                             ucnt, icnt, touch_u, touch_i, out_u + t, out_i + t, out_j + t, task + s * 4, occ + s * 2, occt + s,
+                                             prec + s * 32, pocc + s * 4, n_owner, ohdr + done, ohdr_stride, stream);
+        if (rc != TKR_OK) return rc;
+    }
+    return TKR_OK;
+}
+
 extern "C" int tkr_plan_rollback(const int32_t* task, int32_t batch_size, int32_t first_batch, int32_t n_batches,
                                  int32_t* ucnt, int32_t* icnt, void* stream) {
     if (!task || !ucnt || !icnt || batch_size <= 0 || first_batch < 0 || n_batches < 0) return TKR_EINVAL;
diff --git a/top-k-rec_amd/single/_config.py b/top-k-rec_amd/single/_config.py
--- a/top-k-rec_amd/single/_config.py
+++ b/top-k-rec_amd/single/_config.py
@@ -38,6 +38,7 @@
     flow_item_bufs: int = 4
     own: str = '1'
     own_max_batch: int = 256
+    own_span: int = 2048
     own_waves: int = 0
     fuse_short: bool = True
     fuse_plan: bool = True
@@ -55,7 +56,7 @@
         parsers = {
             'flow': _flag, 'flow_max_batch': _int_in(0, 1 << 20), 'flow_waves_per_cu': _int_in(0, 32),
             'flow_item_bufs': lambda n, r: int(_choice('2', '4')(n, r)), 'own': _choice('0', '1', '2'),
-            'own_max_batch': _int_in(0, 1024), 'own_waves': _int_in(0, 0xffff), 'fuse_short': _flag, 'fuse_plan': _flag,
+            'own_max_batch': _int_in(0, 1024), 'own_span': _int_in(512, 1 << 16), 'own_waves': _int_in(0, 0xffff), 'fuse_short': _flag, 'fuse_plan': _flag,
             'overlap_min_batch': _int_in(1, 1 << 30), 'epoch_ahead': _flag, 'call_ahead': _flag, 'restart': _flag, 'vbpr_cols': _flag, 'vbpr_overlap': _flag,
         }
         out = cls()
diff --git a/top-k-rec_amd/single/_engine.py b/top-k-rec_amd/single/_engine.py
--- a/top-k-rec_amd/single/_engine.py
+++ b/top-k-rec_amd/single/_engine.py
@@ -95,6 +95,17 @@
         self.ws = torch.empty(need, dtype=torch.uint8, device=device) if need else None
 
 
+class _PlanWindow:
+
+    def __init__(self, buf, lo, hi):
+        B = buf.B
+        self.cap, self.B, self.flow, self.cols, self.owners, self.buffer = hi - lo, B, buf.flow, buf.cols, buf.owners, buf
+        for name, words in (('u', 1), ('i', 1), ('j', 1), ('task', 12), ('occ', 6), ('occt', 3), ('prec', 96), ('pocc', 12)):
+            if hasattr(buf, name):
+                setattr(self, name, getattr(buf, name)[lo * B * words:hi * B * words])
+        self.loss = buf.loss[lo:hi]
+
+
 class UpdateCounters:
 
     def __init__(self, n_users, n_items, device):
@@ -218,6 +229,9 @@
 
     def _cap(self, B):
         return _chunk_cap(B)
+
+    def _first_cap(self, B):
+        return self._cap(B)
 
     def _plan_overlap(self, B):
         if getattr(self, 'plan_in_order', False):
@@ -288,8 +302,8 @@
         self._cnt.icnt.copy_(ah.shadow)
         ah.shadow = None
 
-    def _plan_chunk(self, idx, csr, B, first, overlap, want, shadow=None, fuse=False):
-        nb = max(1, min(self._cap(B), want))
+    def _plan_chunk(self, idx, csr, B, first, overlap, want, shadow=None, fuse=False, cap=None):
+        nb = max(1, min(self._cap(B) if cap is None else cap, want))
         cnt = self._cnt if shadow is None else _ShadowCounters(self._cnt, shadow)
         if fuse:
             self.pipe.drain()
@@ -348,9 +362,9 @@
         if cur is not None and self._ahead is not None:
             nxt, self._ahead = self._ahead, None
         else:
-            fuse = (self.cfg.fuse_short and then_exchange == 0 and want <= self._cap(B) and
+            fuse = (self.cfg.fuse_short and then_exchange == 0 and want <= self._first_cap(B) and
                     getattr(getattr(self, '_step', None), 'plan_and_run', None) is not None and self._plan_owners(B) > 0)
-            nxt = self._plan_chunk(0 if cur is None else cur.idx ^ 1, csr, B, self._drawn, False, want, fuse=fuse)
+            nxt = self._plan_chunk(0 if cur is None else cur.idx ^ 1, csr, B, self._drawn, False, want, fuse=fuse, cap=self._first_cap(B))
         if overlap and want > nxt.nb:
             self._ahead = self._plan_chunk(nxt.idx ^ 1, csr, B, nxt.first + nxt.nb * B, True, want - nxt.nb)
         elif overlap and then_exchange == 0 and not self._plan_flow() and self.cfg.call_ahead and want == nxt.nb and want > 8:
@@ -359,7 +373,8 @@
             if getattr(self, '_shadow_icnt', None) is None:
                 self._shadow_icnt = torch.zeros_like(self._cnt.icnt)
             self.pipe.side
-            self._ahead = self._plan_chunk(nxt.idx ^ 1, csr, B, nxt.first + nxt.nb * B, True, then_exchange, shadow=self._shadow_icnt)
+            self._ahead = self._plan_chunk(nxt.idx ^ 1, csr, B, nxt.first + nxt.nb * B, True, then_exchange, shadow=self._shadow_icnt,
+                                           cap=self._first_cap(B))
         self._cur = nxt
         return nxt
 
@@ -393,8 +408,9 @@
             ch.used += m
             left -= m
             self._drawn += m * B
-            loss = plan.loss[lo:lo + m] if want_loss else None
-            self.plan = plan
+            call0 = (lo + m - 1) // MAX_PLAN_BATCHES * MAX_PLAN_BATCHES
+            loss = plan.loss[max(lo, call0):lo + m] if want_loss else None
+            self.plan = plan if call0 == 0 else _PlanWindow(plan, call0, lo + m)
         return loss
 
 
@@ -525,6 +541,20 @@
         if cache[share] < getattr(self, 'own_min_owners', 0):
             return 0
         return cache[share]
+
+    def _first_cap(self, B):
+        return _chunk_cap(B)
+
+    def _cap(self, B):
+        cap = _chunk_cap(B)
+        owners = self._plan_owners(B)
+        if not owners or not self._plan_overlap(B):
+            return cap
+        key = (B, owners)
+        spans = self.__dict__.setdefault('_span_by_shape', {})
+        if key not in spans:
+            spans[key] = max(cap, min(self.cfg.own_span, tkr_hip.bpr_own_max_batches(self.n_items, self.k, owners), (1 << 19) // B))
+        return spans[key]
 
     def wants_flow(self, B):
         if B > self.cfg.flow_max_batch or not self.cfg.flow or self.k > tkr_hip.FLOW_MAX_K:
@@ -715,7 +745,7 @@
                           '<= 256 above batch 1024): the generic row form steps (csrc/bpr_step.hip bpr_wide_kernel: every occurrence in two '
                           'passes over k, the gradient sum through memory)' % (self.k, B))
         cfg = self.cfg
-        again = (id(csr), 0, B, self.layout_epoch, cfg.own, cfg.own_waves, cfg.fuse_short, cfg.fuse_plan, cfg.own_max_batch, cfg.flow, cfg.flow_max_batch, getattr(self, '_flow_disabled', False),
+        again = (id(csr), 0, B, self.layout_epoch, cfg.own, cfg.own_span, cfg.own_waves, cfg.fuse_short, cfg.fuse_plan, cfg.own_max_batch, cfg.flow, cfg.flow_max_batch, getattr(self, '_flow_disabled', False),
                  getattr(self, '_own_failed', False), getattr(self, 'ranks_on_device', 1), self.seed)
         if again == getattr(self, '_again_key', None) and then_exchange == 0 and self.step_events is None:
             loss = self._run_again(csr, n_batches, B, want_loss)
@@ -740,7 +770,7 @@
         if ((cur is not None and cur.used != cur.nb) or self._ahead is not None or getattr(pipe, '_side_dirty', False)
                 or getattr(self, 'tables_invalid', False)):
             return False
-        if n_batches > self._cap(B):
+        if n_batches > self._first_cap(B):
             return False
         if n_batches <= 0 or (want_loss and not getattr(self._step, 'assigns_loss', False)):
             return False
diff --git a/top-k-rec_amd/tkr_hip.py b/top-k-rec_amd/tkr_hip.py
--- a/top-k-rec_amd/tkr_hip.py
+++ b/top-k-rec_amd/tkr_hip.py
@@ -67,7 +67,7 @@
                [(n, C.c_void_p) for n in ('f_ptr', 'f_col', 'f_val', 'c_ptr', 'c_item', 'c_val', 'item_tag')]
 
 
-EXPORTS = ('tkr_version', 'tkr_plan_team', 'tkr_plan_max_blocks', 'tkr_sample_plan', 'tkr_sample_plan_owned', 'tkr_plan_rollback', 'tkr_bpr_run', 'tkr_bpr_flow_run', 'tkr_bpr_own_run', 'tkr_bpr_own_run_between', 'tkr_bpr_own_plan_run', 'tkr_bpr_own_owners', 'tkr_bpr_own_owners_shared', 'tkr_flow_row_granules', 'tkr_flow_ctl_words',
+EXPORTS = ('tkr_version', 'tkr_plan_team', 'tkr_plan_max_blocks', 'tkr_sample_plan', 'tkr_sample_plan_owned', 'tkr_sample_plan_owned_span', 'tkr_plan_rollback', 'tkr_bpr_run', 'tkr_bpr_flow_run', 'tkr_bpr_own_run', 'tkr_bpr_own_run_between', 'tkr_bpr_own_run_span', 'tkr_bpr_own_plan_run', 'tkr_bpr_own_owners', 'tkr_bpr_own_owners_shared', 'tkr_bpr_own_max_batches', 'tkr_flow_row_granules', 'tkr_flow_ctl_words',
            'tkr_vbpr_run', 'tkr_vbpr_colplan', 'tkr_vbpr_run_cols', 'tkr_build_rated_mask', 'tkr_score_topk', 'tkr_count_hits', 'tkr_calib_rowcopy',
            'tkr_idmap_create', 'tkr_idmap_destroy', 'tkr_ratings_parse', 'tkr_ratings_sizes', 'tkr_ratings_copy',
            'tkr_ratings_destroy', 'tkr_matrix_read', 'tkr_matrix_sizes', 'tkr_matrix_copy', 'tkr_matrix_destroy',
@@ -173,6 +173,19 @@
                                  _p(ws), C.c_int64(ws.numel() if ws is not None else 0))
 
 
+def sample_plan_span(csr, n_users, n_items, seed, first_triplet, n_batches, B, cnt, plan):
+    assert plan.owners > 0 and 0 <= n_batches <= plan.cap
+    assert plan.u.numel() >= n_batches * B and plan.task.numel() >= n_batches * 3 * B * 4
+    assert plan.prec.numel() >= n_batches * 3 * B * 32 and plan.pocc.numel() >= n_batches * 3 * B * 4 and plan.ohdr.numel() >= plan.owners * plan.cap
+    assert cnt.ucnt.numel() == n_users and cnt.touch_u.numel() == n_users * 16
+    assert cnt.icnt.numel() == n_items and cnt.touch_i.numel() == n_items * 16
+    _call('tkr_sample_plan_owned_span', plan.u, _p(csr.tr_users), C.c_int32(csr.tr_users.numel()), _p(csr.row_ptr), _p(csr.pos_cols),
+          _p(csr.cols_sorted), C.c_int32(n_users), C.c_int32(n_items), C.c_uint64(seed), C.c_uint64(first_triplet),
+          C.c_int32(n_batches), C.c_int32(B), _p(cnt.ucnt), _p(cnt.icnt), _p(cnt.touch_u), _p(cnt.touch_i), _p(plan.u), _p(plan.i),
+          _p(plan.j), _p(plan.task), _p(plan.occ), _p(plan.occt), _p(plan.prec), _p(plan.pocc), C.c_int32(plan.owners), _p(plan.ohdr),
+          C.c_int32(plan.cap))
+
+
 _PLAN_ARGTYPES = [C.c_void_p, C.c_int32, C.c_void_p, C.c_void_p, C.c_void_p, C.c_int32, C.c_int32, C.c_uint64, C.c_uint64, C.c_void_p,
                   C.c_int32, C.c_int32] + [C.c_void_p] * 15 + [C.c_void_p, C.c_int64, C.c_void_p]
 
@@ -198,19 +211,19 @@
     keep = (csr, cnt)
     owners = getattr(plan, 'owners', 0)
     if owners > 0:
-        fo = lib().tkr_sample_plan_owned
-        fo.argtypes = [C.c_void_p, C.c_int32, C.c_void_p, C.c_void_p, C.c_void_p, C.c_int32, C.c_int32, C.c_uint64, C.c_uint64, C.c_int32,
-                       C.c_int32] + [C.c_void_p] * 12 + [C.c_int32, C.c_void_p, C.c_int32, C.c_void_p]
+        fo, fspan = lib().tkr_sample_plan_owned, lib().tkr_sample_plan_owned_span
+        fo.argtypes = fspan.argtypes = [C.c_void_p, C.c_int32, C.c_void_p, C.c_void_p, C.c_void_p, C.c_int32, C.c_int32, C.c_uint64, C.c_uint64,
+                                        C.c_int32, C.c_int32] + [C.c_void_p] * 12 + [C.c_int32, C.c_void_p, C.c_int32, C.c_void_p]
         tail = (ptr(cnt.ucnt), ptr(cnt.icnt), ptr(cnt.touch_u), ptr(cnt.touch_i), ptr(plan.u), ptr(plan.i), ptr(plan.j), ptr(plan.task),
                 ptr(plan.occ), ptr(plan.occt), ptr(prec), ptr(pocc), owners, ptr(plan.ohdr), plan.cap)
 
         def call_owned(first_triplet, n_batches):
-            assert 0 < n_batches <= min(cap, PLAN_MAX_BATCHES) and keep
+            assert 0 < n_batches <= cap and keep
             prev = torch.cuda.current_device()
             if prev != device.index:
                 torch.cuda.set_device(device.index)
             try:
-                rc = fo(*fixed_a, first_triplet, n_batches, B, *tail, torch.cuda.current_stream(device).cuda_stream)
+                rc = (fo if n_batches <= PLAN_MAX_BATCHES else fspan)(*fixed_a, first_triplet, n_batches, B, *tail, torch.cuda.current_stream(device).cuda_stream)
             finally:
                 if prev != device.index:
                     torch.cuda.set_device(prev)
@@ -298,30 +311,39 @@
     return int(lib().tkr_bpr_own_owners_shared(C.c_int32(n_items), C.c_int32(k), C.c_int32(share)))
 
 
-def bpr_own_run(state, plan, B, n_batches, ctl, loss_out=None, first=0, owner_waves=0):
+def bpr_own_max_batches(n_items, k, owners):
+    return int(lib().tkr_bpr_own_max_batches(C.c_int32(n_items), C.c_int32(k), C.c_int32(owners)))
+
+
+def bpr_own_run(state, plan, B, n_batches, ctl, loss_out=None, first=0, owner_waves=0, sub=0):
     plan.epoch += 1
+    if sub > 0:
+        _call('tkr_bpr_own_run_span', plan.prec, None, None, C.c_void_p(C.addressof(state)), _p(plan.prec), _p(plan.pocc), _p(plan.occt), _p(plan.ohdr),
+              C.c_int32(plan.cap), C.c_int32(plan.owners), C.c_int32(B), C.c_int32(first), C.c_int32(n_batches), C.c_int32(sub), _p(ctl),
+              _p(loss_out), C.c_int32(owner_waves), _p(plan.xch), C.c_uint32(plan.epoch & 0xffffffff or 1))
+        return
     _call('tkr_bpr_own_run', plan.prec, C.byref(state), _p(plan.prec), _p(plan.pocc), _p(plan.occt), _p(plan.ohdr), C.c_int32(plan.cap), C.c_int32(plan.owners),
           C.c_int32(B), C.c_int32(first), C.c_int32(n_batches), _p(ctl), _p(loss_out), C.c_int32(owner_waves), _p(plan.xch),
           C.c_uint32(plan.epoch & 0xffffffff or 1))
 
 
 def own_stepper(state, B, ctl, owner_waves=0):
-    fn = lib().tkr_bpr_own_run_between
+    fn = lib().tkr_bpr_own_run_span
     fn.argtypes = [C.c_void_p, C.c_void_p, C.c_void_p, C.c_void_p, C.c_void_p, C.c_void_p, C.c_void_p, C.c_int32, C.c_int32, C.c_int32, C.c_int32,
-                   C.c_int32, C.c_void_p, C.c_void_p, C.c_int32, C.c_void_p, C.c_uint32, C.c_void_p]
+                   C.c_int32, C.c_int32, C.c_void_p, C.c_void_p, C.c_int32, C.c_void_p, C.c_uint32, C.c_void_p]
     device, st, ctl_ptr = ctl.device, C.addressof(state), ctl.data_ptr()
 
     def step(plan, first, n_batches, loss_out, events=None):
         if torch.cuda.current_device() != device.index:
             assert events is None
-            return bpr_own_run(state, plan, B, n_batches, ctl, loss_out, first, owner_waves)
+            return bpr_own_run(state, plan, B, n_batches, ctl, loss_out, first, owner_waves, sub=PLAN_MAX_BATCHES)
         plan.epoch += 1
         rc = fn(None if events is None else events[0].cuda_event, None if events is None else events[1].cuda_event,
                 st, plan.prec.data_ptr(), plan.pocc.data_ptr(), plan.occt.data_ptr(), plan.ohdr.data_ptr(), plan.cap, plan.owners, B, first, n_batches,
-                ctl_ptr, None if loss_out is None else loss_out.data_ptr(), owner_waves, plan.xch.data_ptr(), plan.epoch & 0xffffffff or 1,
+                PLAN_MAX_BATCHES, ctl_ptr, None if loss_out is None else loss_out.data_ptr(), owner_waves, plan.xch.data_ptr(), plan.epoch & 0xffffffff or 1,
                 torch.cuda.current_stream(device).cuda_stream)
         if rc:
-            _check(rc, 'tkr_bpr_own_run_between')
+            _check(rc, 'tkr_bpr_own_run_span')
     fused = lib().tkr_bpr_own_plan_run
     fused.argtypes = [C.c_void_p, C.c_void_p, C.c_int32, C.c_int32, C.c_void_p, C.c_void_p, C.c_int32, C.c_void_p, C.c_uint32, C.c_void_p,
                       C.c_void_p, C.c_void_p]
```

Result: no change. 42.63 million, median of 4 (+0.7%).
